# DmitryUlyanov/deep-image-prior

Measured on AMD Instinct MI355X. Metric: optimisation iters/sec per image (skip-net 512x512 denoising), higher is better.
Workload: dtype f32

## Files before the change

deep-image-prior_amd/csrc/bn_kernels.hip:

```cpp
#include "dip_common.h"
#include "bn_ticket.h"
#include "dip_group.h"
#include "dip_gradsrc.h"
#include <stdlib.h>

namespace {

template <bool GRP = false>
__global__ __launch_bounds__(256) void bn_finalize_kernel(const float* __restrict__ partials_, int ntiles,
                                                          int Cstride, int C, const float* __restrict__ gamma_,
                                                          const float* __restrict__ beta_, float eps, float momentum,
                                                          float* state_, int Cs, float* running_mean_,
                                                          float* running_var_, const DipGrpArg<GRP> grp) {
    DIP_GRP_PTR(const float*, partials);
    DIP_GRP_PTR(const float*, gamma);
    DIP_GRP_PTR(const float*, beta);
    DIP_GRP_PTR(float*, state);
    DIP_GRP_PTR(float*, running_mean);
    DIP_GRP_PTR(float*, running_var);
    __shared__ double sh[256][12];
    const int row = threadIdx.x;
    const int c0 = blockIdx.x * 4;
    double acc[12];
#pragma unroll
// ... 82 lines not shown

__device__ __forceinline__ void block_reduce_2(const RowLayout& L, f32x4 s1, f32x4 s2, float* partials, int Cs,
                                               float* sh ) {
    dip_tree_sum8(sh, L.nc4, L.rpi, L.prow, L.cg, L.active, s1, s2);
    if (L.active && L.prow == 0) {
        float* o = partials + (size_t)blockIdx.x * 2 * Cs + L.cg * 4;
        st4(o, s1);
        st4(o + Cs, s2);
    }
}

template <bool GRP = false>
__global__ __launch_bounds__(256) void bn_bwd_stats_kernel(const DipGradSrc src_, const float* __restrict__ y_, int H,
                                                           int W, int Cy, int C, const float* __restrict__ state_,
                                                           int Cs, float slope, float* dz_, int Cdz, float* partials_,
                                                           int ppb , const DipBnbFin fin_, const DipGrpArg<GRP> grp) {
    DIP_GRP_DESC(DipGradSrc, src);
    DIP_GRP_PTR(const float*, y);
    DIP_GRP_PTR(const float*, state);
    DIP_GRP_PTR(float*, dz);
    DIP_GRP_PTR(float*, partials);
    DIP_GRP_DESC(DipBnbFin, fin);
    __shared__ __attribute__((aligned(16))) double shd[256 * 8];
    __shared__ unsigned flag;
    float* sh = reinterpret_cast<float*>(shd);
    const RowLayout L = row_layout(C);
    f32x4 s1 = f32x4{0.f, 0.f, 0.f, 0.f}, s2 = s1;
    if (L.active) {
        const int ch = L.cg * 4;
        const f32x4 mean = ld4(state + ch), rstd = ld4(state + Cs + ch), a = ld4(state + 2 * Cs + ch),
                    b = ld4(state + 3 * Cs + ch);
        const int npix = H * W;
        const int p0 = blockIdx.x * ppb;
        const int p1 = min(p0 + ppb, npix);
        const GradSrcThin tw = grad_src_thin(src, ch);
        auto one = [&](int p, const f32x4& du, const f32x4& yv) {
            f32x4 g;
#pragma unroll
            for (int e = 0; e < 4; ++e) {
                const float z = fmaf(a[e], yv[e], b[e]);
                g[e] = dip_mul_rn(du[e], dip_act_grad(z, slope));
                const float xh = (yv[e] - mean[e]) * rstd[e];
                s1[e] += g[e];
                s2[e] += g[e] * xh;
            }
            if (dz != nullptr) st4(dz + (size_t)p * Cdz + ch, g);
        };
        int p = p0 + L.prow;
        for (; p + L.rpi < p1; p += 2 * L.rpi) {
            const int q = p + L.rpi;
            const int r0 = p / W, c0 = p - r0 * W, r1 = q / W, c1 = q - r1 * W;
            const f32x4 du0 = grad_src4(src, tw, r0, c0, H, W, ch);
            const f32x4 du1 = grad_src4(src, tw, r1, c1, H, W, ch);
            const f32x4 y0 = ld4(y + (size_t)p * Cy + ch);
            const f32x4 y1 = ld4(y + (size_t)q * Cy + ch);
            one(p, du0, y0);
            one(q, du1, y1);
        }
        if (p < p1) {
            const int r = p / W, c = p - r * W;
            one(p, grad_src4(src, tw, r, c, H, W, ch), ld4(y + (size_t)p * Cy + ch));
        }
    }
    if (fin.coef == nullptr) {
        block_reduce_2(L, s1, s2, partials, Cs, sh);
        return;
    }
    dip_tree_sum8(sh, L.nc4, L.rpi, L.prow, L.cg, L.active, s1, s2);
    if (L.active && L.prow == 0) {
        float* o = partials + (size_t)blockIdx.x * 2 * Cs + L.cg * 4;
#pragma unroll
        for (int e = 0; e < 4; ++e) { dip_st_sc1(o + e, s1[e]); dip_st_sc1(o + Cs + e, s2[e]); }
    }
    if (dip_ticket_last(fin.ticket, gridDim.x, &flag)) {
        dip_bnb_fin_rows(partials, gridDim.x, Cs, 0, C, fin, shd);
        dip_ticket_reset(fin.ticket);
    }
}

template <bool GRP = false>
__global__ __launch_bounds__(256) void bn_bwd_finalize_kernel(const float* __restrict__ partials_, int nblk,
                                                              const float* __restrict__ partials_lo_, int nblk_lo,
                                                              int c_lo, int Cs, int C, int npix, float* dgamma_,
                                                              float* dbeta_, float* coef_, const DipGrpArg<GRP> grp) {
    DIP_GRP_PTR(const float*, partials);
    DIP_GRP_PTR(const float*, partials_lo);
    DIP_GRP_PTR(float*, dgamma);
    DIP_GRP_PTR(float*, dbeta);
    DIP_GRP_PTR(float*, coef);
    __shared__ double sh[256][8];
    const int row = threadIdx.x;
    const int c0 = blockIdx.x * 4;
    if (c0 < c_lo) { partials = partials_lo; nblk = nblk_lo; }
    double a1[4] = {0.0, 0.0, 0.0, 0.0}, a2[4] = {0.0, 0.0, 0.0, 0.0};
#pragma unroll 8
    for (int t = row; t < nblk; t += 256) {
        const float* p = partials + (size_t)t * 2 * Cs + c0;
        const f32x4 v1 = ld4(p), v2 = ld4(p + Cs);
#pragma unroll
        for (int e = 0; e < 4; ++e) { a1[e] += (double)v1[e]; a2[e] += (double)v2[e]; }
    }
#pragma unroll
    for (int e = 0; e < 4; ++e) { sh[row][e] = a1[e]; sh[row][4 + e] = a2[e]; }
    for (int s = 128; s >= 1; s >>= 1) {
        __syncthreads();
        if (row < s) {
#pragma unroll
            for (int k = 0; k < 8; ++k) sh[row][k] += sh[row + s][k];
        }
    }
    __syncthreads();
    if (row < 4 && c0 + row < C) {
        const int c = c0 + row;
        const double s1 = sh[0][row], s2 = sh[0][4 + row];
        if (dbeta != nullptr) dbeta[c] = (float)s1;
        if (dgamma != nullptr) dgamma[c] = (float)s2;
        coef[c] = (float)(s1 / npix);
        coef[Cs + c] = (float)(s2 / npix);
    }
}

__device__ __forceinline__ void bnb_fin_prologue(const RowLayout& L, const float* __restrict__ partials, int nrows, int Cs,
                                                 int C, int npix, double* shd, float* dgamma, float* dbeta, float* coef,
                                                 f32x4& k1, f32x4& k2) {
    double a[8];
#pragma unroll
    for (int k = 0; k < 8; ++k) a[k] = 0.0;
    if (L.active) {
        const int ch = L.cg * 4;
#pragma unroll 4
        for (int t = L.prow; t < nrows; t += L.rpi) {
            const float* p = partials + (size_t)t * 2 * Cs + ch;
            const f32x4 v1 = ld4(p), v2 = ld4(p + Cs);
#pragma unroll
            for (int e = 0; e < 4; ++e) { a[e] += (double)v1[e]; a[4 + e] += (double)v2[e]; }
        }
    }
    double* mine = shd + (size_t)threadIdx.x * 8;
#pragma unroll
    for (int k = 0; k < 8; ++k) mine[k] = a[k];
    for (int s = dip_pow2_ceil(L.rpi) >> 1; s >= 1; s >>= 1) {
        __syncthreads();
        if (L.active && L.prow < s && L.prow + s < L.rpi) {
            const double* q = shd + (size_t)((L.prow + s) * L.nc4 + L.cg) * 8;
#pragma unroll
            for (int k = 0; k < 8; ++k) mine[k] += q[k];
        }
    }
    __syncthreads();
    if (!L.active) return;
    const double* r0 = shd + (size_t)L.cg * 8;
#pragma unroll
    for (int e = 0; e < 4; ++e) {
        k1[e] = (float)(r0[e] / npix);
        k2[e] = (float)(r0[4 + e] / npix);
    }
    if (blockIdx.x == 0 && L.prow == 0) {
#pragma unroll
        for (int e = 0; e < 4; ++e) {
            const int c = L.cg * 4 + e;
            if (c < C) {
                if (dbeta != nullptr) dbeta[c] = (float)r0[e];
                if (dgamma != nullptr) dgamma[c] = (float)r0[4 + e];
                if (coef != nullptr) { coef[c] = k1[e]; coef[Cs + c] = k2[e]; }
            }
        }
    }
}

struct BnbFinArg {
    const float* partials;
    int nrows;
    float* dgamma;
    float* dbeta;
};
template <class F> __host__ __device__ inline void dip_ptrs(BnbFinArg& b, F& f) { f(b.partials); f(b.dgamma); f(b.dbeta); }

template <bool GRP = false, bool FIN = false>
__global__ __launch_bounds__(256) void bn_bwd_apply_kernel(float* dz_, int Cdz, const float* __restrict__ y_, int Cy,
                                                           int npix, int C, const float* __restrict__ state_, int Cs,
                                                           float* coef_, int ppb, const BnbFinArg fin_, const DipGrpArg<GRP> grp) {
    DIP_GRP_PTR(float*, dz);
    DIP_GRP_PTR(const float*, y);
    DIP_GRP_PTR(const float*, state);
    DIP_GRP_PTR(float*, coef);
    DIP_GRP_DESC(BnbFinArg, fin);
    __shared__ __attribute__((aligned(16))) double shd[FIN ? 256 * 8 : 1];
    const RowLayout L = row_layout(C);
    f32x4 k1 = f32x4{0.f, 0.f, 0.f, 0.f}, k2 = k1;
    if constexpr (FIN) bnb_fin_prologue(L, fin.partials, fin.nrows, Cs, C, npix, shd, fin.dgamma, fin.dbeta, coef, k1, k2);
    if (!L.active) return;
    const int ch = L.cg * 4;
    const f32x4 mean = ld4(state + ch), rstd = ld4(state + Cs + ch), a = ld4(state + 2 * Cs + ch);
    if constexpr (!FIN) { k1 = ld4(coef + ch); k2 = ld4(coef + Cs + ch); }
    const int p0 = blockIdx.x * ppb;
    const int p1 = min(p0 + ppb, npix);
    for (int p = p0 + L.prow; p < p1; p += L.rpi) {
// ... 60 lines not shown
        one(p, grad_src4(src, tw, r, c, H, W, ch), ld4(y + (size_t)p * Cy + ch));
    }
}

__global__ __launch_bounds__(256) void fold_to_nchw_kernel(const DipGradSrc src, int H, int W, int C, float* dst) {
    const int p = blockIdx.x * blockDim.x + threadIdx.x;
    if (p >= H * W) return;
    const int r = p / W, c = p - r * W;
    for (int ch = 0; ch < C; ch += 4) {
        const f32x4 g = grad_src4(src, r, c, H, W, ch);
#pragma unroll
        for (int e = 0; e < 4; ++e)
            if (ch + e < C) dst[(size_t)(ch + e) * H * W + p] = g[e];
    }
}

__global__ __launch_bounds__(256) void fold_to_nhwc_kernel(const DipGradSrc src, int H, int W, int C, float* dst, int Cd) {
    const int nc4 = (C + 3) >> 2;
    const long long i = (long long)blockIdx.x * 256 + threadIdx.x;
    if (i >= (long long)H * W * nc4) return;
    const int cg = (int)(i % nc4);
    const long long p = i / nc4;
    const int r = (int)(p / W), c = (int)(p - (long long)r * W);
    st4(dst + (size_t)p * Cd + cg * 4, grad_src4(src, r, c, H, W, cg * 4));
}

__host__ int bn_blocks(bool apply) { return apply ? 4096 : 1024; }

__host__ int pixels_per_block(int npix, int C, int* nblk, bool apply = false) {
    const int nc4 = (C + 3) / 4;
    int rpi = 256 / nc4;
    if (rpi < 1) rpi = 1;
    int ppb = dip_cdiv(npix, bn_blocks(apply));
    if (ppb < rpi * 2) ppb = rpi * 2;
    *nblk = dip_cdiv(npix, ppb);
    return ppb;
}

}

extern "C" int dip_bn_finalize(const float* partials, int ntiles, int Cstride, int C, const float* gamma,
                               const float* beta, float eps, float momentum, float* state, int Cs,
                               float* running_mean, float* running_var, void* stream) {
    dip_launch_pair<DIP_FAM_BN>(bn_finalize_kernel<false>, bn_finalize_kernel<true>, dim3(dip_cdiv(C, 4)), dim3(256), 0, (hipStream_t)stream, partials,
                                ntiles, Cstride, C, gamma, beta, eps, momentum, state, Cs, running_mean, running_var);
    DIP_CHECK_LAUNCH();
    return 0;
}

extern "C" int dip_bn_bwd_nblk(int H, int W, int C) {
    int nblk;
    pixels_per_block(H * W, C, &nblk);
    return nblk;
}

extern "C" int dip_bn_bwd_stats_fin(const DipGradSrc* src, const float* y, int H, int W, int Cy, int C,
                                    const float* state, int Cs, float slope, float* dz, int Cdz, float* partials,
                                    int nblk, const DipBnbFin* finp, void* stream) {
    if (C > 1024) DIP_FAIL("bn_bwd_stats: C > 1024 unsupported");
    int nb;
    const int ppb = pixels_per_block(H * W, C, &nb);
    if (nb != nblk) DIP_FAIL("bn_bwd_stats: nblk mismatch (use dip_bn_bwd_nblk)");
    DipBnbFin fin = {};
    if (finp != nullptr && finp->coef != nullptr) {
        fin = *finp;
        if (C > 256 || nb > 256 || fin.ticket == nullptr || fin.C != C)
            DIP_FAIL("bn_bwd_stats_fin: needs <= 256 channels and rows (dip_fin_rows_ok), a ticket, C");
    }
    dip_launch_pair<DIP_FAM_BN>(bn_bwd_stats_kernel<false>, bn_bwd_stats_kernel<true>, dim3(nb), dim3(256), 0, (hipStream_t)stream, *src, y, H, W, Cy,
                                C, state, Cs, slope, dz, Cdz, partials, ppb, fin);
    DIP_CHECK_LAUNCH();
    return 0;
}

extern "C" int dip_bn_bwd_stats(const DipGradSrc* src, const float* y, int H, int W, int Cy, int C,
                                const float* state, int Cs, float slope, float* dz, int Cdz, float* partials,
                                int nblk, void* stream) {
    return dip_bn_bwd_stats_fin(src, y, H, W, Cy, C, state, Cs, slope, dz, Cdz, partials, nblk, nullptr, stream);
}

extern "C" int dip_bn_bwd_finalize(const float* partials, int nblk, int Cs, int C, int npix, float* dgamma,
                                   float* dbeta, float* coef, void* stream) {
    dip_launch_pair<DIP_FAM_BN>(bn_bwd_finalize_kernel<false>, bn_bwd_finalize_kernel<true>, dim3(dip_cdiv(C, 4)), dim3(256), 0, (hipStream_t)stream,
                                partials, nblk, (const float*)nullptr, 0, 0, Cs, C, npix, dgamma, dbeta, coef);
    DIP_CHECK_LAUNCH();
    return 0;
}

extern "C" int dip_bn_bwd_finalize2(const float* partials, int nblk, const float* partials_lo, int nblk_lo, int c_lo,
                                    int Cs, int C, int npix, float* dgamma, float* dbeta, float* coef, void* stream) {
    if ((c_lo & 3) || (c_lo > 0 && partials_lo == nullptr)) DIP_FAIL("bn_bwd_finalize2: c_lo must be a multiple of 4");
    dip_launch_pair<DIP_FAM_BN>(bn_bwd_finalize_kernel<false>, bn_bwd_finalize_kernel<true>, dim3(dip_cdiv(C, 4)), dim3(256), 0, (hipStream_t)stream,
                                partials, nblk, partials_lo, nblk_lo, c_lo, Cs, C, npix, dgamma, dbeta, coef);
    DIP_CHECK_LAUNCH();
    return 0;
}

extern "C" int dip_bn_bwd_apply(float* dz, int Cdz, const float* y, int Cy, int npix, int C, const float* state,
                                int Cs, const float* coef, void* stream) {
    int nb;
    const int ppb = pixels_per_block(npix, C, &nb, true);
    dip_launch_pair<DIP_FAM_BN>(bn_bwd_apply_kernel<false>, bn_bwd_apply_kernel<true>, dim3(nb), dim3(256), 0, (hipStream_t)stream, dz, Cdz, y, Cy, npix,
                                C, state, Cs, const_cast<float*>(coef), ppb, BnbFinArg{});
    DIP_CHECK_LAUNCH();
    return 0;
}

extern "C" int dip_bn_bwd_apply_src(const DipGradSrc* src, const float* y, int H, int W, int Cy, int C,
                                    const float* state, int Cs, float slope, const float* coef, float* dy, int Cdy,
                                    void* stream) {
    if (C > 1024) DIP_FAIL("bn_bwd_apply_src: C > 1024 unsupported");
    int nb;
    const int ppb = pixels_per_block(H * W, C, &nb, true);
    dip_launch_pair<DIP_FAM_BN>(bn_bwd_apply_src_kernel<false>, bn_bwd_apply_src_kernel<true>, dim3(nb), dim3(256), 0, (hipStream_t)stream, *src, y, H,
                                W, Cy, C, state, Cs, slope, const_cast<float*>(coef), dy, Cdy, ppb, BnbFinArg{});
    DIP_CHECK_LAUNCH();
    return 0;
}

extern "C" int dip_bn_bwd_fin_rows_ok(int nrows, int C) {
    static const int maxrows = getenv("DIP_BNB_FIN_MAX_ROWS") ? atoi(getenv("DIP_BNB_FIN_MAX_ROWS")) : 320;
    return (nrows >= 1 && nrows <= maxrows && C >= 1 && C <= 1024) ? 1 : 0;
}

extern "C" int dip_bn_bwd_apply_fin(float* dz, int Cdz, const float* y, int Cy, int npix, int C, const float* state, int Cs,
                                    const float* partials, int nrows, float* dgamma, float* dbeta, float* coef, void* stream) {
    if (C > 1024 || (Cs & 3) || partials == nullptr || nrows < 1) DIP_FAIL("bn_bwd_apply_fin: C <= 1024, Cs % 4 == 0, partial rows");
    int nb;
    const int ppb = pixels_per_block(npix, C, &nb, true);
    dip_launch_pair<DIP_FAM_BN>(bn_bwd_apply_kernel<false, true>, bn_bwd_apply_kernel<true, true>, dim3(nb), dim3(256), 0, (hipStream_t)stream, dz, Cdz,
                                y, Cy, npix, C, state, Cs, coef, ppb, BnbFinArg{partials, nrows, dgamma, dbeta});
    DIP_CHECK_LAUNCH();
    return 0;
}

extern "C" int dip_bn_bwd_apply_src_fin(const DipGradSrc* src, const float* y, int H, int W, int Cy, int C, const float* state,
                                        int Cs, float slope, const float* partials, int nrows, float* dgamma, float* dbeta,
                                        float* coef, float* dy, int Cdy, void* stream) {
    if (C > 1024 || (Cs & 3) || partials == nullptr || nrows < 1) DIP_FAIL("bn_bwd_apply_src_fin: C <= 1024, Cs % 4 == 0, partial rows");
    int nb;
    const int ppb = pixels_per_block(H * W, C, &nb, true);
    dip_launch_pair<DIP_FAM_BN>(bn_bwd_apply_src_kernel<false, true>, bn_bwd_apply_src_kernel<true, true>, dim3(nb), dim3(256), 0, (hipStream_t)stream,
                                *src, y, H, W, Cy, C, state, Cs, slope, coef, dy, Cdy, ppb, BnbFinArg{partials, nrows, dgamma, dbeta});
    DIP_CHECK_LAUNCH();
    return 0;
}

extern "C" int dip_fold_to_nhwc(const DipGradSrc* src, int H, int W, int C, float* dst, int Cd, void* stream) {
    if ((Cd & 3) || (src->Cg & 3)) DIP_FAIL("fold_to_nhwc: channel strides must be multiples of 4");
    const long long n = (long long)H * W * ((C + 3) / 4);
    dip_launch(fold_to_nhwc_kernel, dim3((unsigned)((n + 255) / 256)), dim3(256), 0, (hipStream_t)stream, *src, H, W, C, dst, Cd);
    DIP_CHECK_LAUNCH();
    return 0;
}

extern "C" int dip_fold_to_nchw(const DipGradSrc* src, int H, int W, int C, float* dst, void* stream) {
    dip_launch(fold_to_nchw_kernel, dim3(dip_cdiv(H * W, 256)), dim3(256), 0, (hipStream_t)stream, *src, H, W, C, dst);
    DIP_CHECK_LAUNCH();
    return 0;
}
```

deep-image-prior_amd/csrc/dip_group.h:

```cpp
#pragma once
#include "dip_common.h"
#include <stdint.h>
#include <type_traits>

struct DipGroupCtx {
    int ninst;
    long long stride;
    const char* base;
    long long row;
    unsigned native;
};
extern "C" const DipGroupCtx* dip_group_ctx(void);
extern "C" void dip_group_fault(const char* what);

enum : unsigned {
    DIP_FAM_BN = 1u,
    DIP_FAM_CONV = 2u,
    DIP_FAM_DMA = 4u,
    DIP_FAM_SMALL = 8u,
    DIP_FAM_THIN = 16u,
    DIP_FAM_WGRAD = 32u,
    DIP_FAM_LOSS = 64u,
    DIP_FAM_MISC = 128u,
    DIP_FAM_UPCAT = 256u,
};

struct DipGrp {
    long long stride;
    int gz;
};
struct DipNoGrp {};
template <bool GRP> using DipGrpArg = std::conditional_t<GRP, DipGrp, DipNoGrp>;

template <class F> __host__ __device__ inline void dip_ptrs(DipNoGrp&, F&) {}
template <class F> __host__ __device__ inline void dip_ptrs(DipTransform& t, F& f) { f(t.a); f(t.b); }
template <class F> __host__ __device__ inline void dip_ptrs(DipConvDesc& d, F& f) {
    f(d.x); dip_ptrs(d.tr, f); f(d.wp); f(d.bias); f(d.y); f(d.stats); f(d.ws);
    f(d.bnb_y); f(d.bnb_state); f(d.bnb_partials); f(d.bnb_partials_thin); f(d.wp3);
}
template <class F> __host__ __device__ inline void dip_ptrs(DipWgradDesc& d, F& f) {
    f(d.x); dip_ptrs(d.tr, f); f(d.dy); f(d.partial); f(d.bias_partial);
}
template <class F> __host__ __device__ inline void dip_ptrs(DipGradSrc& s, F& f) { f(s.g); f(s.tw); }
template <class F> __host__ __device__ inline void dip_ptrs(DipBnFin& b, F& f) {
    f(b.gamma); f(b.beta); f(b.state); f(b.running_mean); f(b.running_var); f(b.ticket);
}
template <class F> __host__ __device__ inline void dip_ptrs(DipBnbFin& b, F& f) { f(b.dgamma); f(b.dbeta); f(b.coef); f(b.ticket); }
template <class F> __host__ __device__ inline void dip_ptrs(DipUpcatDesc& d, F& f) {
    f(d.s); dip_ptrs(d.ts, f); f(d.d); dip_ptrs(d.td, f); f(d.cat); f(d.stats);
}
template <class F> __host__ __device__ inline void dip_ptrs(DipLossHeadDesc& d, F& f) {
    f(d.u); dip_ptrs(d.tr, f); f(d.w); f(d.bias); f(d.target); f(d.mask); f(d.out); f(d.partials); f(d.loss);
}
template <class F> __host__ __device__ inline void dip_ptrs(DipSRLossDesc& d, F& f) {
    f(d.out); f(d.taps); f(d.target); f(d.y); f(d.partials); f(d.loss);
}
template <class F> __host__ __device__ inline void dip_ptrs(DipSRTVDesc& d, F& f) {
    dip_ptrs(d.sr, f); f(d.tv_weight); f(d.tv_partials);
}

struct DipShiftF {
    long long off;
    template <class T> __host__ __device__ void operator()(T*& p) const {
        if (p != nullptr) p = reinterpret_cast<T*>(reinterpret_cast<uintptr_t>(p) + (uintptr_t)off);
    }
};
struct DipRangeF {
    uintptr_t lo, hi;
    bool ok;
    template <class T> void operator()(T*& p) {
        if (p != nullptr) {
            const uintptr_t v = reinterpret_cast<uintptr_t>(p);
            if (v < lo || v >= hi) ok = false;
        }
    }
};

template <class T, class F>
__host__ __device__ inline void dip_visit(T& v, F& f) {
    using U = std::remove_cv_t<T>;
    if constexpr (std::is_pointer_v<U>) f(v);
    else if constexpr (std::is_arithmetic_v<U> || std::is_enum_v<U> || std::is_same_v<U, std::nullptr_t>) { (void)f; }
    else dip_ptrs(v, f);
}
template <class T>
__host__ __device__ inline T dip_gshift(T v, long long off) {
    DipShiftF f{off};
    dip_visit(v, f);
    return v;
}
template <class... A>
inline bool dip_group_in_range(const DipGroupCtx& g, A... a) {
    DipRangeF f{reinterpret_cast<uintptr_t>(g.base), reinterpret_cast<uintptr_t>(g.base) + (uintptr_t)g.row, true};
    (dip_visit(a, f), ...);
    if (!f.ok) dip_group_fault("a pointer of a grouped launch lies outside instance 0's slab");
    return f.ok;
}

template <bool GRP, class T>
__device__ __forceinline__ const T& dip_pick(const T& shifted, const T& solo) {
    if constexpr (GRP) return shifted;
    else return solo;
}
template <bool GRP>
__device__ __forceinline__ long long dip_grp_off(const DipGrpArg<GRP>& grp) {
    if constexpr (GRP) return (long long)(blockIdx.z / (unsigned)grp.gz) * grp.stride;
    else return 0;
}
template <bool GRP>
__device__ __forceinline__ unsigned dip_grp_z(const DipGrpArg<GRP>& grp) {
    if constexpr (GRP) return blockIdx.z % (unsigned)grp.gz;
    else return blockIdx.z;
}
#define DIP_GRP_DESC(T, d)                                                   \
    T d##sh_;                                                                \
    if constexpr (GRP) d##sh_ = dip_gshift(d##_, dip_grp_off<GRP>(grp));     \
    const T& d = dip_pick<GRP>(d##sh_, d##_)
#define DIP_GRP_PTR(T, p) T p = GRP ? dip_gshift(p##_, dip_grp_off<GRP>(grp)) : p##_

template <class K, class... A>
inline void dip_launch(K kern, dim3 grid, dim3 block, size_t lds, hipStream_t st, A... a) {
    const DipGroupCtx& g = *dip_group_ctx();
    if (g.ninst <= 1) { kern<<<grid, block, lds, st>>>(a...); return; }
    if (!dip_group_in_range(g, a...)) return;
    for (int b = 0; b < g.ninst; ++b) kern<<<grid, block, lds, st>>>(dip_gshift(a, (long long)b * g.stride)...);
}

template <unsigned FAM, class K, class KG, class... A>
inline void dip_launch_pair(K kern, KG kern_g, dim3 grid, dim3 block, size_t lds, hipStream_t st, A... a) {
    const DipGroupCtx& g = *dip_group_ctx();
    if (g.ninst <= 1) { kern<<<grid, block, lds, st>>>(a..., DipNoGrp{}); return; }
    if (!dip_group_in_range(g, a...)) return;
    if (g.native & FAM) {
        const int gz = (int)grid.z;
        grid.z = (unsigned)(gz * g.ninst);
// ... 13 lines not shown
```

deep-image-prior_amd/csrc/dip_list.hip:

```cpp
#include "dip_common.h"
#include <string.h>
#include <utility>

namespace {

template <class T>
inline T slot_as(const uint64_t* s) {
    T v;
    memcpy(&v, s, sizeof(T));
    return v;
}
template <class... A, size_t... I>
inline int call_slots(int (*fn)(A...), const uint64_t* s, std::index_sequence<I...>) {
    return fn(slot_as<A>(s + I)...);
}
template <auto Fn> struct Thunk;
template <class... A, int (*Fn)(A...)>
struct Thunk<Fn> {
    static constexpr int nargs = (int)sizeof...(A);
    static int call(const uint64_t* s) { return call_slots(Fn, s, std::index_sequence_for<A...>{}); }
};

struct Entry {
    const char* name;
    int (*call)(const uint64_t*);
    int nargs;
};
#define DIP_REG(f) {#f, &Thunk<&f>::call, Thunk<&f>::nargs}
const Entry g_fns[] = {
    DIP_REG(dip_nchw_to_nhwc), DIP_REG(dip_nhwc_to_nchw), DIP_REG(dip_head_fwd), DIP_REG(dip_head_bwd),
    DIP_REG(dip_pack_weights), DIP_REG(dip_pack_weights_bf3),
    DIP_REG(dip_conv_igemm), DIP_REG(dip_conv_thin4), DIP_REG(dip_conv_igemm_dma_cols), DIP_REG(dip_conv_small), DIP_REG(dip_conv_thin),
    DIP_REG(dip_conv_dgrad_ring), DIP_REG(dip_conv_bf3_cols), DIP_REG(dip_conv_splitk_finish),
    DIP_REG(dip_conv_wgrad), DIP_REG(dip_wgrad_bf3), DIP_REG(dip_wgrad_thin), DIP_REG(dip_conv_wgrad_tail), DIP_REG(dip_wgrad_tail_stream), DIP_REG(dip_wgrad_reduce),
    DIP_REG(dip_bn_finalize), DIP_REG(dip_bn_bwd_stats), DIP_REG(dip_bn_bwd_stats_fin), DIP_REG(dip_bn_bwd_finalize),
    DIP_REG(dip_bn_bwd_finalize2), DIP_REG(dip_bn_bwd_apply), DIP_REG(dip_bn_bwd_apply_src), DIP_REG(dip_bn_bwd_apply_fin),
    DIP_REG(dip_bn_bwd_apply_src_fin), DIP_REG(dip_bn_bwd_one), DIP_REG(dip_fold_to_nchw), DIP_REG(dip_fold_to_nhwc),
    DIP_REG(dip_upcat_fwd), DIP_REG(dip_upcat_fwd_fin), DIP_REG(dip_avgpool2_fwd), DIP_REG(dip_avgpool2_bwd),
    DIP_REG(dip_maxpool2_fwd), DIP_REG(dip_maxpool2_bwd), DIP_REG(dip_upsample_bwd_stats), DIP_REG(dip_upsample_bwd_stats_crop),
    DIP_REG(dip_upsample_bwd_stats_crop_fin), DIP_REG(dip_upsample_bwd_one),
    DIP_REG(dip_adam_step), DIP_REG(dip_noise_axpy), DIP_REG(dip_adam_tick), DIP_REG(dip_adam_step_dev),
    DIP_REG(dip_noise_axpy_dev), DIP_REG(dip_noise_axpy_dev2), DIP_REG(dip_counter_add), DIP_REG(dip_counter_add_n),
    DIP_REG(dip_adam_sgld_step), DIP_REG(dip_adam_sgld_step_dev), DIP_REG(dip_posterior_dev),
    DIP_REG(dip_loss_head_fwd), DIP_REG(dip_loss_head_bwd), DIP_REG(dip_sr_loss_fwd), DIP_REG(dip_sr_loss_bwd),
    DIP_REG(dip_sr_tv_loss_fwd), DIP_REG(dip_sr_tv_loss_bwd),
    DIP_REG(dip_fit_monitor), DIP_REG(dip_fit_monitor_dev), DIP_REG(dip_arena_backtrack),
    DIP_REG(dip_sr_monitor), DIP_REG(dip_sr_monitor_dev), DIP_REG(dip_restore_monitor), DIP_REG(dip_restore_monitor_dev),
    DIP_REG(dip_early_stop_dev), DIP_REG(dip_early_stop_keep), DIP_REG(dip_early_stop_emv_dev),
    DIP_REG(dip_ssim_dev),
    DIP_REG(dip_lanczos_down_fwd), DIP_REG(dip_lanczos_down_bwd), DIP_REG(dip_down_dense_fwd), DIP_REG(dip_down_dense_bwd_data),
    DIP_REG(dip_down_dense_bwd_weight), DIP_REG(dip_res_join_fwd), DIP_REG(dip_res_join_bwd),
};
constexpr int NFN = (int)(sizeof(g_fns) / sizeof(g_fns[0]));

}

extern "C" int dip_list_fn_id(const char* name) {
    if (name == nullptr) return -1;
    for (int i = 0; i < NFN; ++i)
        if (strcmp(g_fns[i].name, name) == 0) return i;
    return -1;
}

extern "C" int dip_list_fn_nargs(int fn) { return (fn >= 0 && fn < NFN) ? g_fns[fn].nargs : -1; }

extern "C" int dip_list_run(const DipCmd* cmds, int n, void* const* streams, int nstreams, void* const* events, int nevents,
                            int* failed_at) {
    if (failed_at != nullptr) *failed_at = -1;
    for (int i = 0; i < n; ++i) {
        const DipCmd& c = cmds[i];
        int rc = 0;
        if (c.stream < 0 || c.stream >= nstreams) rc = -1;
        else if (c.kind == DIP_CMD_LAUNCH) {
            if (c.fn < 0 || c.fn >= NFN || c.slots == nullptr || c.nslots != g_fns[c.fn].nargs) rc = -1;
            else {
                c.slots[c.nslots - 1] = (uint64_t)reinterpret_cast<uintptr_t>(streams[c.stream]);
                rc = g_fns[c.fn].call(c.slots);
            }
        } else if (c.event < 0 || c.event >= nevents) rc = -1;
        else if (c.kind == DIP_CMD_RECORD)
            rc = (int)hipEventRecord(reinterpret_cast<hipEvent_t>(events[c.event]), reinterpret_cast<hipStream_t>(streams[c.stream]));
        else if (c.kind == DIP_CMD_WAIT)
            rc = (int)hipStreamWaitEvent(reinterpret_cast<hipStream_t>(streams[c.stream]), reinterpret_cast<hipEvent_t>(events[c.event]), 0);
        else rc = -1;
        if (rc != 0) {
            if (failed_at != nullptr) *failed_at = i;
            if (rc == -1 && c.kind != DIP_CMD_LAUNCH) dip_set_error("list_run: malformed command (stream / event index, kind)");
            else if (rc == -1 && (c.fn < 0 || c.fn >= NFN || c.slots == nullptr || c.nslots != g_fns[c.fn < 0 || c.fn >= NFN ? 0 : c.fn].nargs))
                dip_set_error("list_run: malformed LAUNCH command (function id, slot count)");
            else if (c.kind != DIP_CMD_LAUNCH) dip_set_error(hipGetErrorString((hipError_t)rc));
            return rc;
        }
    }
    return 0;
}

extern "C" int dip_iter_run(const DipPhase* phases, int nphases, void* const* streams, int nstreams, int* failed_at) {
    if (failed_at != nullptr) failed_at[0] = failed_at[1] = -1;
    if (phases == nullptr || nphases < 0 || streams == nullptr || nstreams < 1) {
        dip_set_error("iter_run: needs a phase table and at least one stream");
        return -1;
    }
    for (int p = 0; p < nphases; ++p) {
        const DipPhase& ph = phases[p];
        int at = -1;
        int rc = -1;
        if (ph.n < 0 || (ph.n > 0 && ph.cmds == nullptr) || ph.nevents < 0 || (ph.nevents > 0 && ph.events == nullptr))
            dip_set_error("iter_run: malformed phase (command / event table)");
        else rc = dip_list_run(ph.cmds, ph.n, streams, nstreams, ph.events, ph.nevents, &at);
        if (rc != 0) {
            if (failed_at != nullptr) { failed_at[0] = p; failed_at[1] = at; }
            return rc;
        }
    }
    return 0;
}

extern "C" int dip_events_create(void** events, int n) {
    for (int i = 0; i < n; ++i) {
        hipEvent_t e;
        hipError_t rc = hipEventCreateWithFlags(&e, hipEventDisableTiming);
        if (rc != hipSuccess) {
            dip_set_error(hipGetErrorString(rc));
            for (int j = 0; j < i; ++j) (void)hipEventDestroy(reinterpret_cast<hipEvent_t>(events[j]));
            return (int)rc;
        }
        events[i] = reinterpret_cast<void*>(e);
    }
    return 0;
}

extern "C" int dip_events_destroy(void** events, int n) {
    int rc = 0;
    for (int i = 0; i < n; ++i)
// ... 8 lines not shown
```

deep-image-prior_amd/csrc/loss_kernels.hip:

```cpp
#include "dip_common.h"
#include "dip_group.h"
#include <stdlib.h>

namespace {

__device__ __forceinline__ float sigmoidf_(float v) { return 1.f / (1.f + expf(-v)); }

template <bool GRP = false>
__global__ __launch_bounds__(256) void loss_head_fwd_kernel(const DipLossHeadDesc d_, const int ppb, const DipGrpArg<GRP> grp) {
    DIP_GRP_DESC(DipLossHeadDesc, d);
    __shared__ float red[256];
    const int tid = threadIdx.x;
    const int oi = tid & 3;
    const int cin4 = (d.Cin + 3) >> 2;
    const bool has_tr = d.tr.a != nullptr;
    const float slope = d.tr.slope;
    float bias[4];
#pragma unroll
    for (int o = 0; o < 4; ++o) bias[o] = (d.bias != nullptr && o < d.Cout) ? d.bias[o] : 0.f;
    const float* wrow = d.w + (size_t)(oi < d.Cout ? oi : 0) * d.Cin;
    const bool wvalid = oi < d.Cout;

    const int p0 = blockIdx.x * ppb, p1 = min(p0 + ppb, d.HW);
    float lsum = 0.f;
    for (int pb = p0; pb < p1; pb += 256) {
        const int p = pb + tid;
        const bool pv = p < p1;
        const float* up = d.u + (size_t)(pv ? p : p0) * d.Cu;
        f32x4 ac4[4];
#pragma unroll
        for (int e = 0; e < 4; ++e) ac4[e] = f32x4{0.f, 0.f, 0.f, 0.f};
#pragma unroll 8
        for (int k4 = 0; k4 < cin4; ++k4) {
            f32x4 b = *reinterpret_cast<const f32x4*>(up + k4 * 4);
            f32x4 a;
#pragma unroll
            for (int e = 0; e < 4; ++e) {
                const int c = k4 * 4 + e;
                a[e] = (wvalid && c < d.Cin) ? wrow[c] : 0.f;
                if (has_tr) {
                    const float ta = c < d.Cin ? d.tr.a[c] : 0.f, tb = c < d.Cin ? d.tr.b[c] : 0.f;
                    b[e] = dip_act(fmaf(ta, b[e], tb), slope);
                }
            }
#pragma unroll
            for (int e = 0; e < 4; ++e) ac4[e] = __builtin_amdgcn_mfma_f32_4x4x1f32(a[e], b[e], ac4[e], 4, 0, 0);
        }
        const f32x4 acc = (ac4[0] + ac4[1]) + (ac4[2] + ac4[3]);
        if (pv) {
#pragma unroll
            for (int o = 0; o < 4; ++o) {
                if (o < d.Cout) {
                    float y = acc[o] + bias[o];
                    if (d.sigmoid) y = sigmoidf_(y);
                    d.out[(size_t)o * d.HW + p] = y;
                    const float t = d.target[(size_t)o * d.HW + p];
                    float a = y, b = t;
                    if (d.mask != nullptr) {
                        const float m = d.mask[(size_t)(d.mask_c == 1 ? 0 : o) * d.HW + p];
                        a = y * m;
                        b = t * m;
                    }
                    const float df = a - b;
                    lsum = fmaf(df, df, lsum);
                }
            }
        }
    }
    red[tid] = lsum;
    __syncthreads();
    for (int s = 128; s >= 1; s >>= 1) {
        if (tid < s) red[tid] += red[tid + s];
        __syncthreads();
    }
    if (tid == 0) d.partials[blockIdx.x] = red[0];
}

template <int NC4, bool GRP = false>
__global__ __launch_bounds__(256) void loss_head_fwd_coal_kernel(const DipLossHeadDesc d_, const int ppb, const DipGrpArg<GRP> grp) {
    DIP_GRP_DESC(DipLossHeadDesc, d);
    __shared__ float red[256];
    constexpr int PW = 64 / NC4;
    constexpr int PB = 4 * PW;
    const int tid = threadIdx.x, lane = tid & 63, wave = tid >> 6;
    const int cg = lane % NC4, psub = lane / NC4;
    const bool has_tr = d.tr.a != nullptr;
    const float slope = has_tr ? d.tr.slope : 1.f;
    const bool leaky = slope > 0.f;
    f32x4 ta = f32x4{1.f, 1.f, 1.f, 1.f}, tb = f32x4{0.f, 0.f, 0.f, 0.f};
    float w[4][4];
#pragma unroll
    for (int e = 0; e < 4; ++e) {
        const int c = cg * 4 + e;
        if (has_tr && c < d.Cin) { ta[e] = d.tr.a[c]; tb[e] = d.tr.b[c]; }
#pragma unroll
        for (int o = 0; o < 4; ++o) w[o][e] = (o < d.Cout && c < d.Cin) ? d.w[(size_t)o * d.Cin + c] : 0.f;
    }
    const bool bA = (cg & (NC4 / 2)) != 0, bB = (cg & (NC4 / 4)) != 0;
    const int myo = 2 * (bA ? 1 : 0) + (bB ? 1 : 0);
    const bool writer = (cg & (NC4 / 4 - 1)) == 0 && myo < d.Cout;
    const float mybias = (d.bias != nullptr && myo < d.Cout) ? d.bias[myo] : 0.f;
    const int p0 = blockIdx.x * ppb, p1 = min(p0 + ppb, d.HW);
    float lsum = 0.f;
    constexpr int UN = 4;
    for (int base = p0 + wave * PW; base < p1; base += UN * PB) {
        const int pb = base + psub;
        f32x4 u[UN];
#pragma unroll
        for (int q = 0; q < UN; ++q) {
            const int p = pb + q * PB;
            u[q] = *reinterpret_cast<const f32x4*>(d.u + (size_t)(p < p1 ? p : p0) * d.Cu + cg * 4);
        }
#pragma unroll
        for (int q = 0; q < UN; ++q) {
            const int p = pb + q * PB;
            f32x4 v = u[q];
            if (leaky) {
#pragma unroll
                for (int e = 0; e < 4; ++e) v[e] = dip_act_leaky(fmaf(ta[e], v[e], tb[e]), slope);
            } else {
#pragma unroll
                for (int e = 0; e < 4; ++e) v[e] = dip_act(fmaf(ta[e], v[e], tb[e]), slope);
            }
            float part[4];
#pragma unroll
            for (int o = 0; o < 4; ++o) part[o] = (w[o][0] * v[0] + w[o][1] * v[1]) + (w[o][2] * v[2] + w[o][3] * v[3]);
            const float k0 = (bA ? part[2] : part[0]) + __shfl_xor(bA ? part[0] : part[2], NC4 / 2);
            const float k1 = (bA ? part[3] : part[1]) + __shfl_xor(bA ? part[1] : part[3], NC4 / 2);
            float mine = (bB ? k1 : k0) + __shfl_xor(bB ? k0 : k1, NC4 / 4);
#pragma unroll
            for (int sft = NC4 / 8; sft >= 1; sft >>= 1) mine += __shfl_xor(mine, sft);
            if (p < p1 && writer) {
                float y = mine + mybias;
                if (d.sigmoid) y = sigmoidf_(y);
                d.out[(size_t)myo * d.HW + p] = y;
                const float t = d.target[(size_t)myo * d.HW + p];
                float a = y, b = t;
                if (d.mask != nullptr) {
                    const float m = d.mask[(size_t)(d.mask_c == 1 ? 0 : myo) * d.HW + p];
                    a = y * m;
                    b = t * m;
                }
                const float df = a - b;
                lsum = fmaf(df, df, lsum);
            }
        }
    }
    red[tid] = lsum;
    __syncthreads();
    for (int s2 = 128; s2 >= 1; s2 >>= 1) {
        if (tid < s2) red[tid] += red[tid + s2];
        __syncthreads();
    }
    if (tid == 0) d.partials[blockIdx.x] = red[0];
}

template <bool GRP = false>
__global__ __launch_bounds__(256) void loss_reduce_kernel(const float* __restrict__ partials_, int n, double scale,
                                                          float* __restrict__ loss_, const DipGrpArg<GRP> grp) {
    DIP_GRP_PTR(const float*, partials);
    DIP_GRP_PTR(float*, loss);
    __shared__ double dred[256];
    const int tid = threadIdx.x;
    double s = 0.0;
    for (int i = tid; i < n; i += 256) s += (double)partials[i];
    dred[tid] = s;
    __syncthreads();
    for (int st = 128; st >= 1; st >>= 1) {
        if (tid < st) dred[tid] += dred[tid + st];
        __syncthreads();
    }
    if (tid == 0) *loss = (float)(dred[0] * scale);
}

template <bool GRP = false>
__global__ __launch_bounds__(256) void loss_head_bwd_kernel(const DipLossHeadDesc d_, const float* __restrict__ gscale_,
                                                            float* __restrict__ dy_, const int Cy, const DipGrpArg<GRP> grp) {
    DIP_GRP_DESC(DipLossHeadDesc, d);
    DIP_GRP_PTR(const float*, gscale);
    DIP_GRP_PTR(float*, dy);
    const int p = blockIdx.x * 256 + threadIdx.x;
    if (p >= d.HW) return;
    const float gs = gscale != nullptr ? *gscale : 1.f;
    const float k = 2.f / ((float)d.Cout * (float)d.HW);
    for (int c0 = 0; c0 < Cy; c0 += 4) {
        f32x4 v = f32x4{0.f, 0.f, 0.f, 0.f};
#pragma unroll
        for (int e = 0; e < 4; ++e) {
            const int o = c0 + e;
            if (o < d.Cout) {
                const float y = d.out[(size_t)o * d.HW + p];
                const float t = d.target[(size_t)o * d.HW + p];
                float a = y, b = t, m = 1.f;
                if (d.mask != nullptr) {
                    m = d.mask[(size_t)(d.mask_c == 1 ? 0 : o) * d.HW + p];
                    a = y * m;
                    b = t * m;
                }
                float g = (a - b) * k * gs;
                if (d.mask != nullptr) g = g * m;
                if (d.sigmoid) g = g * ((1.f - y) * y);
                v[e] = g;
            }
        }
        *reinterpret_cast<f32x4*>(dy + (size_t)p * Cy + c0) = v;
    }
}

template <bool GRP = false>
__global__  void adam_tick_kernel(DipIterState* st_, double lr, double beta1, double beta2, const DipGrpArg<GRP> grp) {
    DIP_GRP_PTR(DipIterState*, st);
    if (threadIdx.x != 0 || blockIdx.x != 0) return;
    const unsigned long long step = st->step + 1ull;
    st->step = step;
    const double bc1 = 1.0 - pow(beta1, (double)step);
    const double bc2 = 1.0 - pow(beta2, (double)step);
    st->step_size = (float)(lr / bc1);
    st->bc2_sqrt = (float)sqrt(bc2);
}

template <bool GRP = false>
__global__  void counter_add_kernel(unsigned long long* c_, unsigned long long inc, const DipGrpArg<GRP> grp) {
    DIP_GRP_PTR(unsigned long long*, c);
    if (threadIdx.x == 0 && blockIdx.x == 0) *c += inc;
}

template <bool GRP = false>
__global__  void counter_add_n_kernel(unsigned long long* c_, int n, unsigned long long inc, const DipGrpArg<GRP> grp) {
    DIP_GRP_PTR(unsigned long long*, c);
    const int i = (int)(blockIdx.x * blockDim.x + threadIdx.x);
    if (i < n) c[i] += inc;
}

}

#define NC4_MIN_CHECK(cout, nc4) ((nc4) < 4 || (cout) > (nc4))
static int head_ppb(int HW) {
    int ppb = dip_round_up(dip_cdiv(HW, 1024), 256);
    return ppb < 256 ? 256 : ppb;
}

extern "C" int dip_loss_head_nblk(int HW, int Cin) {
    (void)Cin;
    return dip_cdiv(HW, head_ppb(HW));
}

extern "C" int dip_loss_head_fwd(const DipLossHeadDesc* dp, void* stream) {
    const DipLossHeadDesc& d = *dp;
    if (d.Cout < 1 || d.Cout > 4) DIP_FAIL("loss_head: 1..4 output channels");
    if (d.Cin < 1 || (d.Cu & 3) || dip_round_up(d.Cin, 4) > d.Cu) DIP_FAIL("loss_head: channel stride must be a multiple of 4 covering Cin");
    if (d.mask != nullptr && d.mask_c != 1 && d.mask_c != d.Cout) DIP_FAIL("loss_head: mask must have 1 or Cout channels");
    const int ppb = head_ppb(d.HW);
    const int nblk = dip_cdiv(d.HW, ppb);
    if (nblk != d.nblk) DIP_FAIL("loss_head: nblk must come from dip_loss_head_nblk");
    const int nc4 = (d.Cin + 3) / 4;
    static const bool no_coal = getenv("DIP_LOSS_HEAD_NO_COAL") != nullptr;
    hipStream_t st = (hipStream_t)stream;
    if (no_coal || nc4 > 32 || (nc4 & (nc4 - 1)) != 0 || (NC4_MIN_CHECK(d.Cout, nc4))) {
        dip_launch_pair<DIP_FAM_LOSS>(loss_head_fwd_kernel<false>, loss_head_fwd_kernel<true>, dim3(nblk), dim3(256), 0, st, d, ppb);
    } else {
        switch (nc4) {
            case 32: dip_launch_pair<DIP_FAM_LOSS>(loss_head_fwd_coal_kernel<32>, loss_head_fwd_coal_kernel<32, true>, dim3(nblk), dim3(256), 0, st, d, ppb); break;
            case 16: dip_launch_pair<DIP_FAM_LOSS>(loss_head_fwd_coal_kernel<16>, loss_head_fwd_coal_kernel<16, true>, dim3(nblk), dim3(256), 0, st, d, ppb); break;
            case 8: dip_launch_pair<DIP_FAM_LOSS>(loss_head_fwd_coal_kernel<8>, loss_head_fwd_coal_kernel<8, true>, dim3(nblk), dim3(256), 0, st, d, ppb); break;
            default: dip_launch_pair<DIP_FAM_LOSS>(loss_head_fwd_coal_kernel<4>, loss_head_fwd_coal_kernel<4, true>, dim3(nblk), dim3(256), 0, st, d, ppb); break;
        }
    }
    DIP_CHECK_LAUNCH();
    dip_launch_pair<DIP_FAM_LOSS>(loss_reduce_kernel<false>, loss_reduce_kernel<true>, dim3(1), dim3(256), 0, (hipStream_t)stream,
                                  (const float*)d.partials, nblk, 1.0 / ((double)d.Cout * (double)d.HW), d.loss);
    DIP_CHECK_LAUNCH();
    return 0;
}

extern "C" int dip_loss_head_bwd(const DipLossHeadDesc* dp, const float* gscale, float* dy, int Cy, void* stream) {
    const DipLossHeadDesc& d = *dp;
    if (d.Cout < 1 || d.Cout > 4 || (Cy & 3) || Cy < d.Cout) DIP_FAIL("loss_head_bwd: bad channel counts");
    dip_launch_pair<DIP_FAM_LOSS>(loss_head_bwd_kernel<false>, loss_head_bwd_kernel<true>, dim3(dip_cdiv(d.HW, 256)), dim3(256), 0, (hipStream_t)stream,
                                  d, gscale, dy, Cy);
    DIP_CHECK_LAUNCH();
    return 0;
}

extern "C" int dip_adam_tick(DipIterState* st, double lr, double beta1, double beta2, void* stream) {
    dip_launch_pair<DIP_FAM_LOSS>(adam_tick_kernel<false>, adam_tick_kernel<true>, dim3(1), dim3(1), 0, (hipStream_t)stream, st, lr, beta1, beta2);
    DIP_CHECK_LAUNCH();
    return 0;
}

extern "C" int dip_counter_add(uint64_t* counter, uint64_t inc, void* stream) {
    dip_launch_pair<DIP_FAM_LOSS>(counter_add_kernel<false>, counter_add_kernel<true>, dim3(1), dim3(1), 0, (hipStream_t)stream,
                                  reinterpret_cast<unsigned long long*>(counter), (unsigned long long)inc);
    DIP_CHECK_LAUNCH();
    return 0;
}

extern "C" int dip_counter_add_n(uint64_t* counters, int n, uint64_t inc, void* stream) {
    if (counters == nullptr || n < 1) DIP_FAIL("counter_add_n: needs n >= 1 counters");
    dip_launch_pair<DIP_FAM_LOSS>(counter_add_n_kernel<false>, counter_add_n_kernel<true>, dim3(dip_cdiv(n, 64)), dim3(64), 0,
                                  (hipStream_t)stream, reinterpret_cast<unsigned long long*>(counters), n, (unsigned long long)inc);
    DIP_CHECK_LAUNCH();
    return 0;
}

namespace {

constexpr int SR_T = 16;
constexpr int SR_LDS_BYTES = 48 * 1024;
constexpr int SR_UN = 8;

template <int K, int F, bool GRP = false>
__global__ __launch_bounds__(256) void sr_loss_fwd_kernel(const DipSRLossDesc d_, const int qn, const int pitch, const int rp,
                                                          const DipGrpArg<GRP> grp) {
    DIP_GRP_DESC(DipSRLossDesc, d);
    extern __shared__ float sr_win[];
    __shared__ float red[256];
    const int k = K ? K : d.k, f = F ? F : d.f;
    const int tid = threadIdx.x, lx = tid & 15, ly = tid >> 4;
    const int ntx = (d.Wo + SR_T - 1) / SR_T, nty = (d.Ho + SR_T - 1) / SR_T;
    const int b = blockIdx.x;
    const int ox0 = (b % ntx) * SR_T, oy0 = ((b / ntx) % nty) * SR_T, c = b / (ntx * nty);
    const float* xc = d.out + (size_t)c * d.H * d.W;
    const int wc = (SR_T - 1) * f + k, wr = (rp - 1) * f + k, nwin = wr * wc;
    const int ox = ox0 + lx, oy = oy0 + ly;
    const bool inside = ox < d.Wo && oy < d.Ho;
    const int gx0 = ox0 * f - d.pad;
    float acc = 0.f;
    for (int ob = 0; ob < SR_T && oy0 + ob < d.Ho; ob += rp) {
        const int gy0 = (oy0 + ob) * f - d.pad;
        if (ob) __syncthreads();
        for (int i0 = tid; i0 < nwin; i0 += 256 * SR_UN) {
            float v[SR_UN];
#pragma unroll
            for (int u = 0; u < SR_UN; ++u) {
                const int idx = i0 + u * 256, wy = idx / wc, wx = idx - wy * wc;
                v[u] = idx < nwin ? xc[(size_t)min(max(gy0 + wy, 0), d.H - 1) * d.W + min(max(gx0 + wx, 0), d.W - 1)] : 0.f;
            }
#pragma unroll
            for (int u = 0; u < SR_UN; ++u) {
// ... 366 lines not shown
```

deep-image-prior_amd/dip_engine.py:

```python
from __future__ import annotations

import ctypes as C
import os
from typing import List, Optional

import torch

import dip_native as N
from dip_native import round_up


def _ptr(t: Optional[torch.Tensor], off_floats: int = 0) -> Optional[int]:
    if t is None:
        return None
    return t.data_ptr() + 4 * off_floats


class BNRec:

    def __init__(self, module: torch.nn.BatchNorm2d, name: str):
        self.module = module
        self.name = name
        self.C = module.num_features
        self.Cs = round_up(self.C, 4)
# ... 4 lines not shown


class ConvRec:
    def __init__(self, module: torch.nn.Conv2d, pad_mode: int, name: str):
        self.module = module
        self.name = name
        self.Cin, self.Cout = module.in_channels, module.out_channels
        self.ks = module.kernel_size[0]
        self.stride = module.stride[0]
        self.P = (self.ks - 1) // 2
        self.pad_mode = pad_mode if self.P > 0 else N.PAD_ZERO
        self.w_off = self.b_off = -1
        self.fwd_off = self.dgrad_off = -1
        self.need_dgrad = True

    @property
    def fwd_elems(self):
        return self.ks * self.ks * round_up(self.Cin, 4) * round_up(self.Cout, 32)

    @property
    def dgrad_elems(self):
        return self.ks * self.ks * round_up(self.Cout, 4) * round_up(self.Cin, 32)


class Act:

    def __init__(self, buf, H, W, Cch, bn: Optional[BNRec] = None, slope: float = 1.0):
        self.buf, self.H, self.W, self.C = buf, H, W, Cch
        self.Cs = round_up(Cch, 4)
        self.bn, self.slope = bn, slope

    def transform(self, shape_only=False) -> N.DipTransform:
        if self.bn is None:
            return N.DipTransform(None, None, 1.0)
        if shape_only:
            return N.DipTransform(1, 1, self.slope)
        assert self.bn.Cs == self.Cs
        return N.DipTransform(_ptr(self.bn.state, 2 * self.Cs), _ptr(self.bn.state, 3 * self.Cs), self.slope)


class ScalePlan:

    def __init__(self):
        self.skip_conv = self.skip_bn = None
        self.down_a = self.down_a_bn = self.down_b = self.down_b_bn = None
        self.cat_bn = self.up = self.up_bn = self.up1 = self.up1_bn = None
        self.ns = 0
        self.upsample_mode = "nearest"
        self.pool = None
        self.down_ds = None


class SkipEngine:
    kind = "skip"

    def __init__(self, net, scales: List[ScalePlan], out_conv: torch.nn.Conv2d, need_sigmoid: bool, pad: str,
                 act_slope: float = 0.2):
        self._init_common(net, need_sigmoid, pad, act_slope)
        self._collect_records(scales, out_conv)
        self.param_list = list(net.parameters())
        self._check_supported()

    def _init_common(self, net, need_sigmoid: bool, pad: str, act_slope: float):
        self.net = net
        self.need_sigmoid = need_sigmoid
        self.pad_mode = N.PAD_REFLECT if pad == "reflection" else N.PAD_ZERO
        self.slope = act_slope
        self.fwd_id = 0
        self._aux = {}
        self.two_streams = os.environ.get("DIP_TWO_STREAMS", "1") != "0"
        self.defer_scale = int(os.environ.get("DIP_DEFER_WGRAD", "2")) if self.two_streams else -1
        self.side_min_pixels = int(os.environ.get("DIP_SIDE_MIN_PIXELS", "0"))
        self._fwd_side, self._deferred, self._entered_defer_scale, self._fused_bnb = set(), [], False, {}
        self.use_clist = os.environ.get("DIP_NO_CLIST") is None
        import re
        ko = os.environ.get("DIP_KNOCKOUT")
        self._knockout = re.compile(ko) if ko else None
        self._ko_after, self._ko_seen = int(os.environ.get("DIP_KNOCKOUT_AFTER", "0")), {}
        self._clists = {}
        self._replicate_bufs = set()
        self.fuse_bnb = os.environ.get("DIP_BNB_FUSE", "0") == "1"
        self.fuse_bnb_1x1 = os.environ.get("DIP_BNB_FUSE", "0") == "2"
        self.thin_src = os.environ.get("DIP_NO_THIN_SRC") is None
        self.use_small = os.environ.get("DIP_CONV_NO_SMALL") is None
        self.ticket_fin = os.environ.get("DIP_TICKET_FIN") == "1"
        self.bnb_one = os.environ.get("DIP_BNB_NO_ONE") is None
        self.tail_inline = self.two_streams and os.environ.get("DIP_TAIL_INLINE", "1") != "0"
        self.bnb_fin_fuse = os.environ.get("DIP_BNB_FIN_FUSE") == "1"
        self.bulk2_max_pixels = 0
        if self.two_streams:
            env = os.environ.get("DIP_BULK2_MAX_PIXELS")
            self.bulk2_max_pixels = int(env) if env is not None else -1
        self._bulk2, self._bulk_flip = set(), False
        self.bf3 = False
        self.device = None
        self.shape_key = None
        self.lib = None
        self.slab = None

    def _collect_records(self, scales: List[ScalePlan], out_conv: torch.nn.Conv2d):
        self.nscales = len(scales)
        self.convs: List[ConvRec] = []
        self.bns: List[BNRec] = []
        self.sc = []
        for i, s in enumerate(scales):
            rec = ScalePlan()
            rec.ns, rec.upsample_mode = s.ns, s.upsample_mode
            rec.pool = getattr(s, 'pool', None)
            for attr in ("skip_conv", "down_a", "down_ds", "down_b", "up", "up1"):
                m = getattr(s, attr, None)
                if m is not None:
                    r = ConvRec(m, self.pad_mode, f"s{i}.{attr}")
                    if attr == "down_ds":
                        r.P = (r.ks - r.stride) // 2
                        r.pad_mode = N.PAD_REPLICATE
                    self.convs.append(r)
                    setattr(rec, attr, r)
            for attr in ("skip_bn", "down_a_bn", "down_b_bn", "cat_bn", "up_bn", "up1_bn"):
                m = getattr(s, attr)
                if m is not None:
                    r = BNRec(m, f"s{i}.{attr}")
                    self.bns.append(r)
                    setattr(rec, attr, r)
            self.sc.append(rec)
        self.out_conv = ConvRec(out_conv, self.pad_mode, "out")
        self.convs.append(self.out_conv)

    def _check_supported(self):
        for r in self.convs:
            lanczos_ds = r.name.endswith(".down_ds") and r.ks in (8, 12) and r.stride == 2
            if not lanczos_ds and (r.ks not in (1, 3, 5, 7) or r.stride not in (1, 2) or (r.ks == 1 and r.stride != 1)):
                raise NotImplementedError(f"dip-amd: conv {r.name} k={r.ks} s={r.stride} has no gfx950 kernel")
            m = r.module
            if m.dilation != (1, 1) or m.groups != 1 or m.kernel_size[0] != m.kernel_size[1]:
                raise NotImplementedError(f"dip-amd: conv {r.name}: dilation/groups/non-square unsupported")
        for b in self.bns:
            if b.module.momentum is None:
                raise NotImplementedError(f"dip-amd: BatchNorm {b.name}: momentum=None (cumulative moving average of "
                                          "the running statistics) is not implemented; the reference uses 0.1")
            if not b.module.affine:
                raise NotImplementedError(f"dip-amd: BatchNorm {b.name}: affine=False is not implemented")
        for i, s in enumerate(self.sc):
            if s.ns % 4 or s.down_b.Cout % 4 or s.up.Cout % 4 or (s.up.Cin % 4):
                raise NotImplementedError("dip-amd: internal channel counts must be multiples of 4")

    def _dalloc(self, n, dtype=torch.float32, zero=False):
        if self.slab is not None:
            return self.slab.alloc(int(n), dtype, zero)
        return (torch.zeros if zero else torch.empty)(int(n), dtype=dtype, device=self.device)

    def _dcopy(self, host_bytes):
        src = torch.frombuffer(bytearray(host_bytes), dtype=torch.uint8)
        t = self._dalloc(src.numel(), torch.uint8)
        t.copy_(src)
        return t

    def _build_arenas(self, device):
        self.lib = N.lib()
        self.device = device
        params = self.param_list
        off = 0
        slots = []
        for p in params:
            slots.append(off)
            off += round_up(p.numel(), 4)
        self.n_arena = off
# ... 30 lines not shown
                b.coef = self._dalloc(2 * b.Cs, zero=True)
        off = 0
        recs = (N.DipPackRec * len(self.convs))()
        max_elems = 0
        for k, r in enumerate(self.convs):
            r.fwd_off = off
            off += r.fwd_elems
            r.dgrad_off = off
            off += r.dgrad_elems
            recs[k] = N.DipPackRec(w_off=r.w_off, fwd_off=r.fwd_off, dgrad_off=r.dgrad_off, Cout=r.Cout, Cin=r.Cin, KS=r.ks,
                                   CinP4=round_up(r.Cin, 4), CoutP32=round_up(r.Cout, 32), CoutP4=round_up(r.Cout, 4),
                                   CinP32=round_up(r.Cin, 32))
            max_elems = max(max_elems, r.fwd_elems + r.dgrad_elems)
        self.packed = self._dalloc(off, zero=True)
        self.bf3 = bool(self.lib.dip_conv_bf3_terms())
        if self.bf3:
            off3, max3 = 0, 0
            recs3 = (N.DipPackRec3 * len(self.convs))()
            for k, r in enumerate(self.convs):
                r.fwd3_off = r.dgrad3_off = -1
                nchF, nchD = (round_up(r.Cin, 4) + 15) // 16, (round_up(r.Cout, 4) + 15) // 16
                CoutP, CinP = round_up(r.Cout, 32), round_up(r.Cin, 32)
                k1 = (os.environ.get("DIP_CONV_BF3_1X1") == "1" and r.ks == 1 and r.Cin % 16 == 0 and r.Cout % 16 == 0
                      and min(r.Cin, r.Cout) >= 128)
                if (r.ks == 3 or k1) and r.stride == 1 and not r.name.endswith(".down_ds"):
                    kk = r.ks * r.ks
                    r.fwd3_off = off3
                    off3 += kk * nchF * 3 * CoutP * 16
                    r.dgrad3_off = off3
                    off3 += kk * nchD * 3 * CinP * 16
                    max3 = max(max3, kk * 16 * (nchF * CoutP + nchD * CinP))
                recs3[k] = N.DipPackRec3(w_off=r.w_off, fwd_off=r.fwd3_off, dgrad_off=r.dgrad3_off, Cout=r.Cout, Cin=r.Cin,
                                         KS=r.ks, nchF=nchF, CoutP32=CoutP, nchD=nchD, CinP32=CinP)
            self.packed3 = self._dalloc(max(off3, 8), torch.int16, zero=True)
            self.pack_recs3 = self._dcopy(bytes(recs3))
            self.pack_max3 = max3
        self.pack_recs = self._dcopy(bytes(recs))
        self.pack_max = max_elems
        self.shape_key = None

    def _arena_ok(self) -> bool:
        if self.device is None:
            return False
        base = self.params.data_ptr()
        for p, o in zip(self.param_list, self.slots):
            if p.data_ptr() != base + 4 * o:
                return False
        return True

    def _new(self, n):
        t = self._dalloc(n)
        self._alloc.append(t)
        return t

    _SCRATCH = ("stats", "bwd", "wg", "wgb", "wg2", "wgb2", "ws", "stats2", "ws2", "bwd2", "bwd3")

    def _reset_sizing(self):
        self._need = dict.fromkeys(self._SCRATCH, 4)
        self._need["tickets"] = 8

    def _scratch(self, name, n):
        if self._sizing:
            self._need[name] = max(self._need[name], n)
            return None
        assert n <= self._need[name], (name, n, self._need[name])
        return self._pool[name]

    def _has_big_layer(self, H, W) -> bool:
        h, w = H, W
        for sc in self.sc:
            hl, wl = ((h + 1) // 2, (w + 1) // 2) if sc.pool is None else (h // 2, w // 2)
            for r, px in ((sc.down_a, hl * wl), (sc.down_b, hl * wl), (sc.up, h * w), (sc.up1, h * w)):
                if r is not None and r.ks >= 3 and r.Cin >= 96 and r.Cout >= 96 and px >= 65536:
                    return True
            h, w = hl, wl
        return False

    def _begin_plan(self, H, W, Cin_img):
        self.H, self.W, self.Cimg = H, W, Cin_img
        self._clists = {}
        self._reset_sizing()
        self._alloc = []
        self.n_out = self.out_conv.Cout
        if getattr(self, "_bulk2_auto", self.bulk2_max_pixels < 0):
            self._bulk2_auto = True
            self.bulk2_max_pixels = 0 if self._has_big_layer(H, W) else 100000

    def _build_plan(self, H, W, Cin_img):
        if min(H, W) < 2 ** self.nscales:
            raise NotImplementedError(f"dip-amd: input {H}x{W} is too small for {self.nscales} scales")
        self._begin_plan(H, W, Cin_img)
        oc = self.out_conv
        for sizing in (True, False):
            self._begin_pass(sizing)
            self.x_nhwc = self._buf(H * W * round_up(Cin_img, 4))
            xin = Act(self.x_nhwc, H, W, Cin_img)
            last = self._plan_scale(0, xin, H, W)
            self.Hout, self.Wout = last.H, last.W
            self.y_out = self._buf(last.H * last.W * round_up(oc.Cout, 4))
            self._emit_conv_fwd(oc, last, self.y_out, None)
            self.dy_out = self._buf(last.H * last.W * round_up(oc.Cout, 4))
            pre = []
            self._emit_wgrad(oc, last, self.dy_out, pre, scale=0)
            if self._thin_src_ok(oc, last):
                du_last = (self.dy_out, 0, oc)
            else:
                du_last = self._emit_dgrad(oc, last, self.dy_out, pre, fuse_bn=True)
            dy_last = self._emit_bn_act_bwd(last, du_last, pre)
            self.dbg_top = {"du_last": du_last, "dy_last": dy_last, "last": last}
            self.last_act = last
            self.bwd_ops = pre + self._bwd_scale_ops(0, dy_last)
            self.bwd_ops += self._flush_deferred_wgrads()
        self.shape_key = (H, W, Cin_img)

    def _begin_pass(self, sizing: bool):
        self._sizing = sizing
        self.fwd_ops, self.bwd_ops, self.bwd_input_ops, self.keep = [], [], [], []
        if not sizing:
            self._pool = {name: self._new(self._need[name]) for name in self._SCRATCH}
            self._pool["tickets"] = self._dalloc(self._need["tickets"], torch.int32, zero=True)
            self._alloc.append(self._pool["tickets"])
        self._ticket_off = 0
        self._fused_bnb = {}
        self._deferred = []
        self._replicate_bufs = set()
        self._fwd_side = set()
        self._bulk2, self._bulk_flip = set(), False
        self._entered_defer_scale = False

    def _plan_scale(self, i, xin: Act, H, W):
        s = self.sc[i]
        st = {}
        Hl, Wl = ((H + 1) // 2, (W + 1) // 2) if s.pool is None else (H // 2, W // 2)
        if s.ns:
            st["s_y"] = self._buf(H * W * round_up(s.ns, 4))
            self._emit_conv_fwd(s.skip_conv, xin, st["s_y"], s.skip_bn)
            st["s_act"] = Act(st["s_y"], H, W, s.ns, s.skip_bn, self.slope)
        st["d1_y"] = self._buf(Hl * Wl * round_up(s.down_a.Cout, 4))
        if s.pool in ('avg', 'max'):
            st["d1_full"] = self._buf(H * W * round_up(s.down_a.Cout, 4))
            self._emit_conv_fwd(s.down_a, xin, st["d1_full"], None)
            self._emit_avgpool(st["d1_full"], H, W, s.down_a.Cout, st["d1_y"], s.down_a_bn, s.pool)
        elif s.pool == 'lanczos':
            st["d1_full"] = self._buf(H * W * round_up(s.down_a.Cout, 4))
            self._emit_conv_fwd(s.down_a, xin, st["d1_full"], None)
            st["d1_raw"] = Act(st["d1_full"], H, W, s.down_a.Cout)
            self._emit_conv_fwd(s.down_ds, st["d1_raw"], st["d1_y"], s.down_a_bn)
        else:
            self._emit_conv_fwd(s.down_a, xin, st["d1_y"], s.down_a_bn)
        d1 = Act(st["d1_y"], Hl, Wl, s.down_a.Cout, s.down_a_bn, self.slope)
        st["d2_y"] = self._buf(Hl * Wl * round_up(s.down_b.Cout, 4))
        self._emit_conv_fwd(s.down_b, d1, st["d2_y"], s.down_b_bn)
        d2 = Act(st["d2_y"], Hl, Wl, s.down_b.Cout, s.down_b_bn, self.slope)
        st["d1"], st["d2"] = d1, d2
        deep = d2
        if i < self.nscales - 1:
            deep = self._plan_scale(i + 1, d2, Hl, Wl)
        st["deep"] = deep
        ccat = s.ns + deep.C
        assert ccat == s.cat_bn.C == s.up.Cin, (ccat, s.cat_bn.C, s.up.Cin)
        Hu, Wu = 2 * deep.H, 2 * deep.W
        if s.ns:
            Ho, Wo = min(H, Hu), min(W, Wu)
        else:
            Ho, Wo = Hu, Wu
        geom = dict(Hs=H, Ws=W, os_y=(H - Ho) // 2 if s.ns else 0, os_x=(W - Wo) // 2 if s.ns else 0,
                    Hd=deep.H, Wd=deep.W, od_y=(Hu - Ho) // 2, od_x=(Wu - Wo) // 2)
        default = (not s.ns or (Ho, Wo) == (H, W)) and deep.H == (Ho + 1) // 2 and deep.W == (Wo + 1) // 2 \
            and geom["od_y"] == 0 and geom["od_x"] == 0
        st["geom"] = None if default else geom
        st["cat"] = self._buf(Ho * Wo * round_up(ccat, 4))
        self._emit_upcat(s, st.get("s_act"), deep, st["cat"], Ho, Wo, st["geom"])
        cat = Act(st["cat"], Ho, Wo, ccat, s.cat_bn, 1.0)
        st["cat_act"] = cat
        st["u_y"] = self._buf(Ho * Wo * round_up(s.up.Cout, 4))
        self._emit_conv_fwd(s.up, cat, st["u_y"], s.up_bn)
        u = Act(st["u_y"], Ho, Wo, s.up.Cout, s.up_bn, self.slope)
        st["u"] = u
        res = u
        if s.up1 is not None:
            st["u1_y"] = self._buf(Ho * Wo * round_up(s.up1.Cout, 4))
            self._emit_conv_fwd(s.up1, u, st["u1_y"], s.up1_bn)
            res = Act(st["u1_y"], Ho, Wo, s.up1.Cout, s.up1_bn, self.slope)
            st["u1"] = res
        st["xin"], st["H"], st["W"], st["Ho"], st["Wo"] = xin, H, W, Ho, Wo
        s.st = st
        return res

    def _buf(self, n):
        return None if self._sizing else self._new(n)

    def _ticket(self, n=8):
        if self._sizing:
            self._need["tickets"] += n
            return None
        off = self._ticket_off
# ... 182 lines not shown
                self.keep.append(d)
                ops.append((self.lib.dip_conv_small, (C.byref(d),), "dgrad:" + r.name))
            return (gbuf, pad)
        ws = self._scratch("ws", wsf)
        d.ws = _ptr(ws) if ksplit > 1 else None
        variant = self.lib.dip_conv_variant(C.byref(d))
        if fuse_here and self.lib.dip_conv_bnb_fusable(C.byref(d)):
            c_lo = (r.Cin - 128) if variant == 3 else 0
            if c_lo % 4 == 0:
                self._fuse_bnb_into(d, x, gbuf, pad, self.lib.dip_conv_ntiles(Hg, Wg),
                                    self.lib.dip_conv_thin4_ntiles(Hg, Wg) if c_lo else 0, c_lo)
        if sizing:
            return (gbuf, pad)
        self.keep.append(d)
        if variant == 3 and self.two_streams:
            ncols = r.Cin - 128
            ops.append((self.lib.dip_conv_thin4, (C.byref(d), ncols), "dgthin:" + r.name))
            ops.append((self.lib.dip_conv_igemm_dma_cols, (C.byref(d), ncols), "dgrad:" + r.name))
        else:
            ops.append((self.lib.dip_conv_igemm, (C.byref(d),), "dgrad:" + r.name))
        if ring:
            dr = N.DipConvDesc.from_buffer_copy(d)
            dr.ksplit, dr.ws = 1, None
            self.keep.append(dr)
            ops.append((self.lib.dip_conv_dgrad_ring, (C.byref(dr),), "dgring:" + r.name))
        return (gbuf, pad)

    def _fuse_bnb_into(self, d: N.DipConvDesc, x: Act, gbuf, pad, rows, rows_lo=0, c_lo=0):
        bn = x.bn
        partials = self._scratch("bwd", rows * 2 * bn.Cs)
        thin = self._scratch("bwd3", rows_lo * 2 * bn.Cs)
        if self._sizing:
            return
        d.bnb_y, d.bnb_state = _ptr(x.buf), _ptr(bn.state)
        d.bnb_partials, d.bnb_partials_thin = _ptr(partials), _ptr(thin) if c_lo else None
        d.bnb_Cy, d.bnb_Cs, d.bnb_pad, d.bnb_slope = x.Cs, bn.Cs, pad, float(x.slope)
        self._fused_bnb[gbuf.data_ptr()] = (rows, rows_lo, c_lo)

    def _thin_src_ok(self, oc: ConvRec, last: Act) -> bool:
        return (self.thin_src and oc.ks == 1 and oc.stride == 1 and oc.Cout <= 4 and oc.Cin % 4 == 0 and last.bn is not None
                and not self.fuse_bnb and not self._bnb_one_ok(last))

    def _gradsrc(self, g, Cg, choff=0, window=None):
        if len(g) == 3:
            buf, _, oc = g
            d = N.DipGradSrc(g=_ptr(buf), Cg=round_up(oc.Cout, 4), tw=_ptr(self.params, oc.w_off), tn=oc.Cout, tcw=oc.Cin)
            self.keep.append(d)
            return d
        buf, pad = g
        fold = 0 if pad == 0 else (2 if buf.data_ptr() in self._replicate_bufs else 1)
        d = N.DipGradSrc(g=_ptr(buf), pad=pad, fold=fold, Cg=Cg, choff=choff)
        if window is not None:
            d.win_y, d.win_x, d.win_h, d.win_w = window
        self.keep.append(d)
        return d

    def _act_args(self, a: Act):
        return (_ptr(a.buf), a.H, a.W, a.Cs, a.C, _ptr(a.bn.state), a.bn.Cs, float(a.slope))

    def _dparams(self, bn: BNRec):
        return (_ptr(self.grads, bn.gamma_off), _ptr(self.grads, bn.beta_off), _ptr(bn.coef))

    def _emit_bnb_apply(self, a: Act, dz, ops, src=None, partials=None):
        bn, lib = a.bn, self.lib
        if partials is None:
            fns, fin = (lib.dip_bn_bwd_apply, lib.dip_bn_bwd_apply_src), (_ptr(bn.coef),)
        else:
            fns = (lib.dip_bn_bwd_apply_fin, lib.dip_bn_bwd_apply_src_fin)
            fin = (_ptr(partials[0]), partials[1], *self._dparams(bn))
        if src is None:
            args = (_ptr(dz), a.Cs, _ptr(a.buf), a.Cs, a.H * a.W, a.C, _ptr(bn.state), bn.Cs, *fin)
        else:
            args = (C.byref(src), *self._act_args(a), *fin, _ptr(dz), a.Cs)
        ops.append((fns[src is not None], args, "bnb_apply:" + bn.name))

    def _emit_bnb_fin_apply(self, a: Act, scratch, rows, dz, ops, src=None):
        bn = a.bn
        if self._fin_rows_ok(rows, a.C):
            return self._emit_bnb_apply(a, dz, ops, src, (scratch, rows))
        ops.append((self.lib.dip_bn_bwd_finalize, (_ptr(scratch), rows, bn.Cs, bn.C, a.H * a.W, *self._dparams(bn)),
                    "bnb_fin:" + bn.name))
        self._emit_bnb_apply(a, dz, ops, src)

    def _emit_bn_act_bwd(self, a: Act, g, ops, choff=0, Cg=None, side=False, window=None):
        bn = a.bn
        nblk = self.lib.dip_bn_bwd_nblk(a.H, a.W, a.C)
        fin_ok = self.ticket_fin and bool(self.lib.dip_fin_rows_ok(nblk, a.C))
        ticket = self._ticket() if fin_ok else None
        scratch = self._scratch("bwd2" if side else "bwd", nblk * 2 * a.Cs)
        if self._sizing:
            return None
        dz = self._new(a.H * a.W * a.Cs)
        src = self._gradsrc(g, Cg if Cg is not None else a.Cs, choff, window)
        lib = self.lib
        if self._bnb_one_ok(a) and self._fused_bnb.get(g[0].data_ptr()) is None:
            ops.append((lib.dip_bn_bwd_one, (C.byref(src), *self._act_args(a), _ptr(dz), a.Cs, *self._dparams(bn)),
                        "bnb_one:" + bn.name))
            return dz
        stats = (C.byref(src), *self._act_args(a), None, a.Cs, _ptr(scratch), nblk)
        fused = self._fused_bnb.get(g[0].data_ptr()) if (choff == 0 and not side) else None
        if fused is None and fin_ok:
            fin = self._bnb_fin(bn, a.H * a.W, ticket)
            self.keep.append(fin)
            ops.append((lib.dip_bn_bwd_stats_fin, (*stats, C.byref(fin)), "bnb_stats:" + bn.name))
            self._emit_bnb_apply(a, dz, ops, src)
        elif fused is None:
            ops.append((lib.dip_bn_bwd_stats, stats, "bnb_stats:" + bn.name))
            self._emit_bnb_fin_apply(a, scratch, nblk, dz, ops, src)
        else:
            rows, rows_lo, c_lo = fused
            if c_lo == 0 and self._fin_rows_ok(rows, a.C):
                self._emit_bnb_apply(a, dz, ops, src, (scratch, rows))
                return dz
            thin = self._scratch("bwd3", rows_lo * 2 * bn.Cs) if c_lo else None
            ops.append((lib.dip_bn_bwd_finalize2, (_ptr(scratch), rows, _ptr(thin), rows_lo, c_lo, bn.Cs, bn.C, a.H * a.W,
                                                   *self._dparams(bn)), "bnb_fin:" + bn.name))
            self._emit_bnb_apply(a, dz, ops, src)
        return dz

    def _fin_rows_ok(self, rows, Cc) -> bool:
        return self.bnb_fin_fuse and bool(self.lib.dip_bn_bwd_fin_rows_ok(rows, Cc))

    def _bnb_one_ok(self, a: Act) -> bool:
        return self.bnb_one and a.bn is not None and bool(self.lib.dip_bn_bwd_one_ok(a.H * a.W, a.C))

    def _emit_up_bwd(self, deep: Act, dcat, Cs_cat, choff, H, W, mode, ops, geom=None):
        bn = deep.bn
        nblk = self.lib.dip_bn_bwd_nblk(deep.H, deep.W, deep.C)
        fin_ok = self.ticket_fin and bool(self.lib.dip_fin_rows_ok(nblk, deep.C))
        ticket = self._ticket() if fin_ok else None
        scratch = self._scratch("bwd", nblk * 2 * deep.Cs)
        if self._sizing:
            return None
        dz = self._new(deep.H * deep.W * deep.Cs)
        lib = self.lib
        m = N.UP_BILINEAR if mode == "bilinear" else N.UP_NEAREST
        gm = geom if geom is not None else dict(Hd=(H + 1) // 2, Wd=(W + 1) // 2, od_y=0, od_x=0)
        crop = (_ptr(dcat), Cs_cat, choff, H, W, gm["Hd"], gm["Wd"], gm["od_y"], gm["od_x"], m)
        act = (_ptr(deep.buf), deep.Cs, deep.C, _ptr(bn.state), bn.Cs, float(deep.slope), _ptr(dz), deep.Cs)
        if self._bnb_one_ok(deep):
            ops.append((lib.dip_upsample_bwd_one, (*crop, *act, *self._dparams(bn)), "upb_one:" + bn.name))
        elif fin_ok:
            fin = self._bnb_fin(bn, deep.H * deep.W, ticket)
            self.keep.append(fin)
            ops.append((lib.dip_upsample_bwd_stats_crop_fin, (*crop, *act, _ptr(scratch), nblk, C.byref(fin)),
                        "upb_stats:" + bn.name))
            self._emit_bnb_apply(deep, dz, ops)
        else:
            if geom is None:
                ops.append((lib.dip_upsample_bwd_stats, (_ptr(dcat), Cs_cat, choff, H, W, m, *act, _ptr(scratch), nblk),
                            "upb_stats:" + bn.name))
            else:
                ops.append((lib.dip_upsample_bwd_stats_crop, (*crop, *act, _ptr(scratch), nblk), "upb_stats:" + bn.name))
            self._emit_bnb_fin_apply(deep, scratch, nblk, dz, ops)
        return dz

    def _bwd_scale_ops(self, i, dy_last):
        s = self.sc[i]
        st = s.st
        ops = []
        if i == self.defer_scale:
            self._entered_defer_scale = True
            ops += self._flush_deferred_wgrads()
        H, W, xin = st["H"], st["W"], st["xin"]
        Ho, Wo, geom = st["Ho"], st["Wo"], st["geom"]
        if s.up1 is not None:
            self._emit_wgrad(s.up1, st["u"], dy_last, ops, scale=i)
            g = self._emit_dgrad(s.up1, st["u"], dy_last, ops, fuse_bn=True)
            dy_u = self._emit_bn_act_bwd(st["u"], g, ops)
        else:
            dy_u = dy_last
        cat = st["cat_act"]
        self._emit_wgrad(s.up, cat, dy_u, ops, scale=i)
        g = self._emit_dgrad(s.up, cat, dy_u, ops, fuse_bn=True)
        dcat = self._emit_bn_act_bwd(cat, g, ops)
        dy_s = None
        if s.ns:
            win = (geom["os_y"], geom["os_x"], Ho, Wo) if (geom is not None and (Ho, Wo) != (H, W)) else None
            dy_s = self._emit_bn_act_bwd(st["s_act"], (dcat, 0), ops, choff=0, Cg=cat.Cs, side=True, window=win)
            self._emit_wgrad(s.skip_conv, xin, dy_s, ops, scale=i)
        deep = st["deep"]
        dy_deep = self._emit_up_bwd(deep, dcat, cat.Cs, s.ns, Ho, Wo, s.upsample_mode, ops, geom)
        if self._entered_defer_scale:
# ... 53 lines not shown
        producers = {p for ps in deps.values() for p in ps}
        main_seq = 0
        forked = [0, -1, -1, -1]
        pending = [False, False, False, False]
        for k, (fn, args, name) in enumerate(ops):
            c = cls_fn(name)
            if c and forked[c] != main_seq:
                sched += [("record", ("fork", k), 0), ("wait", c, ("fork", k))]
                forked[c] = main_seq
            if c == 0 and pending[1] and join_before_fn(name):
                sched += [("record", ("join", k), 1), ("wait", 0, ("join", k))]
                pending[1] = False
            for prod in deps.get(name, ()):
                sched.append(("wait", c, ("dep", prod)))
            sched.append(("launch", k, c))
            if name in producers:
                sched.append(("record", ("dep", name), c))
            if c:
                pending[c] = True
            else:
                main_seq += 1
        for c in (1, 2, 3):
            if pending[c]:
                sched += [("record", ("join", -c), c), ("wait", 0, ("join", -c))]
        return sched

    def _aux_streams(self):
        slot = "cap" if torch.cuda.is_current_stream_capturing() else "eager"
        st_ = self._aux.get((slot, self.device))
        if st_ is None:
            st_ = self._aux[(slot, self.device)] = ([torch.cuda.Stream(self.device) for _ in range(3)], {})
        return slot, st_[0], st_[1]

    def _issue(self, ops, main, key, cls_fn=None, join_before_fn=None, deps=None, compile_only=False, drop_last=False):
        multi = cls_fn is not None
        slot, aux, events = self._aux_streams() if multi else ("one", [], None)
        ko = False
        if self._knockout is not None:
            n = self._ko_seen[key] = self._ko_seen.get(key, 0) + 1
            ko = n > self._ko_after
        ck = (key, drop_last, multi, ko)
        ent = self._clists.get(ck)
        if ent is None or ent[0] is not ops:
            sched = self._schedule(ops[:-1] if drop_last else ops, cls_fn, join_before_fn, deps)
            if ko:
                sched = [c for c in sched if not (c[0] == "launch" and self._knockout.search(ops[c[1]][2]))]
            cl = None
            if self.use_clist:
                evidx = {}
                cmds = []
                for c in sched:
                    if c[0] == "launch":
                        fn, args, name = ops[c[1]]
                        cmds.append(("launch", fn, args, c[2], name))
                    elif c[0] == "record":
                        cmds.append(("record", evidx.setdefault(c[1], len(evidx)), c[2]))
                    else:
                        cmds.append(("wait", c[1], evidx.setdefault(c[2], len(evidx))))
                cl = N.CmdList(cmds)
            ent = self._clists[ck] = (ops, sched, cl)
        _, sched, cl = ent
        if compile_only:
            return cl
        if cl is not None:
            cl.run([main.cuda_stream] + [s_.cuda_stream for s_ in aux], slot)
            return
        streams = [main] + aux
        ptrs = [s_.cuda_stream for s_ in streams]
        check = N.check
        for c in sched:
            if c[0] == "launch":
                fn, args, name = ops[c[1]]
                rc = fn(*args, ptrs[c[2]])
                if rc:
                    check(rc, name)
            elif c[0] == "record":
                ev = events.get((key, c[1]))
                if ev is None:
                    ev = events[(key, c[1])] = torch.cuda.Event()
                ev.record(streams[c[2]])
            else:
                streams[c[1]].wait_event(events[(key, c[2])])

    _BWD_SIDE = staticmethod(lambda n: 2 if n.startswith(("wgrad:", "wgred:")) else
                             (1 if (n.startswith("dgthin:") or n.endswith(".skip_bn")) else 0))

    def _backward_deps(self, ops):
        names = [name for _, _, name in ops]
        present = set(names)
        deps = {}
        for i, sc in enumerate(self.sc):
            c, p = f"dgrad+:s{i}.skip_conv", f"bnb_apply:s{i}.skip_bn"
            if p not in present:
                p = f"bnb_one:s{i}.skip_bn"
            if sc.ns and c in present and p in present:
                deps.setdefault(c, []).append(p)
            c = f"wgrad:s{i}.skip_conv"
            if sc.ns and c in present and p in present:
                deps.setdefault(c, []).append(p)
        for k, name in enumerate(names):
            if not name.startswith("dgthin:"):
                continue
            main_part = "dgrad:" + name[len("dgthin:"):]
            j = names.index(main_part, k)
            consumer = next((n for n in names[j + 1:] if not self._BWD_SIDE(n)), None)
            if consumer is not None:
                deps.setdefault(consumer, []).append(name)
        return deps

    def _run_backward_two_streams(self, ops, main, compile_only=False):
        deps = self._bwd_deps if getattr(self, "_bwd_deps_for", None) is ops else None
        if deps is None:
            deps = self._bwd_deps = self._backward_deps(ops)
            self._bwd_deps_for = ops
        capturing = torch.cuda.is_current_stream_capturing()
        bulk2 = self._bulk2 if not capturing else ()
        cls = self._BWD_SIDE if not bulk2 else (lambda n: 3 if n in bulk2 else self._BWD_SIDE(n))
        return self._issue(ops, main, "bwd_cap" if capturing else "bwd", cls, lambda n: False, deps, compile_only)

    def _run_forward_two_streams(self, ops, main, compile_only=False, drop_last=False):
        side = self._fwd_side
        return self._issue(ops, main, "fwd", lambda n: 1 if n in side else 0, lambda n: n.startswith("upcat:"),
                           compile_only=compile_only, drop_last=drop_last)

    def _forward_prologue(self, x_ptr):
        lib = self.lib
        ops = [(lib.dip_pack_weights, (_ptr(self.params), _ptr(self.packed), self.pack_recs.data_ptr(),
                                       len(self.convs), self.pack_max), "pack_weights")]
        if self.bf3:
            ops.append((lib.dip_pack_weights_bf3, (_ptr(self.params), self.packed3.data_ptr(), self.pack_recs3.data_ptr(),
                                                   len(self.convs), self.pack_max3), "pack_weights_bf3"))
        ops.append((lib.dip_nchw_to_nhwc, (x_ptr, _ptr(self.x_nhwc), self.Cimg, self.H * self.W, round_up(self.Cimg, 4)),
                    "nchw_to_nhwc"))
        return ops

    def _launch_forward(self, x_ptr, main, with_out_conv=True, compile_only=False):
        if not compile_only:
            stream = main.cuda_stream
            for fn, args, name in self._forward_prologue(x_ptr):
                N.check(fn(*args, stream), name)
        drop_last = not with_out_conv
        if self.two_streams:
            return self._run_forward_two_streams(self.fwd_ops, main, compile_only, drop_last)
        return self._issue(self.fwd_ops, main, "fwd1", compile_only=compile_only, drop_last=drop_last)

    def _launch_backward(self, main, compile_only=False):
        if self.two_streams:
            return self._run_backward_two_streams(self.bwd_ops, main, compile_only)
        return self._issue(self.bwd_ops, main, "bwd1", compile_only=compile_only)

    def iteration_lists(self, with_out_conv=False):
        if not self.use_clist:
            raise RuntimeError("dip-amd: the native iteration chains compiled command lists; DIP_NO_CLIST=1 switches them off")
        if self._knockout is not None:
            raise RuntimeError("dip-amd: DIP_KNOCKOUT is a timing experiment of the eager path; the native iteration refuses it")
        if torch.cuda.is_current_stream_capturing():
            raise RuntimeError("dip-amd: the native iteration is an eager form; hipGraph capture goes through GraphedIteration")
        return self._launch_forward(None, None, with_out_conv, compile_only=True), self._launch_backward(None, compile_only=True)

    def _net_cin(self) -> int:
        return self.sc[0].down_a.Cin

    def _input_gin(self):
        return self.sc[0].gin

    def _prepare(self, dev, H, W, Cimg):
        if self.device != dev or not self._arena_ok():
            self._build_arenas(dev)
        if self.shape_key != (H, W, Cimg):
            if Cimg != self._net_cin():
                raise RuntimeError(f"dip-amd: input has {Cimg} channels, net expects {self._net_cin()}")
            self._build_plan(H, W, Cimg)

    def forward(self, x: torch.Tensor, head=None):
        if x.dim() != 4 or x.shape[0] != 1:
            raise NotImplementedError("dip-amd: input must be [1,C,H,W] (train-mode BatchNorm couples a batch; "
                                      "independent images run as independent nets)")
        if not self.net.training:
            raise NotImplementedError("dip-amd: eval-mode BatchNorm is not implemented (the reference never "
                                      "calls .eval() on the skip path)")
        dev = x.device
        _, Cimg, H, W = x.shape
        self._prepare(dev, H, W, Cimg)
        lib = self.lib
        with torch.cuda.device(dev):
            main = torch.cuda.current_stream(dev)
            stream = main.cuda_stream
            xs = x.detach()
            if xs.dtype != torch.float32:
                xs = xs.float()
            xs = xs.contiguous()
            self.fwd_id += 1
            self._launch_forward(xs.data_ptr(), main, head is None or head.with_out_conv)
            Ho_, Wo_ = self.Hout, self.Wout
            out = torch.empty((1, self.n_out, Ho_, Wo_), dtype=torch.float32, device=dev)
            loss = None
            if head is None:
                N.check(lib.dip_head_fwd(_ptr(self.y_out), out.data_ptr(), self.n_out, Ho_ * Wo_, round_up(self.n_out, 4),
                                         1 if self.need_sigmoid else 0, stream), "head_fwd")
            else:
                loss = torch.empty((), dtype=torch.float32, device=dev)
                self._head_desc = head._descriptor(self, out, loss)
                for fn, args, name in head.fwd_launches(self, self._head_desc):
                    N.check(fn(*args, stream), name)
            if len(self.bns):
                self.nbt.add_(1)
        self.last_out = out.detach()
        self.last_head = head
        return out if head is None else (loss, out)

    def _detach_stale_grads(self):
        base = self.grads.data_ptr()
        stale = [k for k, (p, o) in enumerate(zip(self.param_list, self.slots))
                 if p.grad is not None and p.grad.data_ptr() == base + 4 * o]
        if not stale:
            return
        if getattr(self, "grads_alt", None) is None or self.grads_alt.numel() != self.grads.numel() \
                or self.grads_alt.device != self.grads.device:
            self.grads_alt = torch.empty_like(self.grads)
        self.grads_alt.copy_(self.grads)
        for k in stale:
            p, o = self.param_list[k], self.slots[k]
            p.grad = self.grads_alt[o:o + p.numel()].view(p.shape)

    def backward(self, gout, fwd_id: int, need_input_grad: bool, gloss=None):
        if fwd_id != self.fwd_id:
            raise RuntimeError("dip-amd: backward() of a stale forward: the engine keeps the activations of the "
                               "most recent net(x) only (one forward, one backward per closure call)")
        dev = self.device
        lib = self.lib
        H, W = self.H, self.W
        grads = self.grads
        with torch.cuda.device(dev):
            main = torch.cuda.current_stream(dev)
            stream = main.cuda_stream
            self._detach_stale_grads()
            if self.last_head is None:
                g = gout.detach()
                if g.dtype != torch.float32:
                    g = g.float()
                g = g.contiguous()
                N.check(lib.dip_head_bwd(g.data_ptr(), self.last_out.data_ptr(), _ptr(self.dy_out), self.n_out,
                                         self.Hout * self.Wout,
                                         round_up(self.n_out, 4), 1 if self.need_sigmoid else 0, stream), "head_bwd")
            else:
                gl = gloss.detach().reshape(1)
                if gl.dtype != torch.float32:
                    gl = gl.float()
                self._gloss_keep = gl
                for fn, args, name in self.last_head.bwd_launches(self, self._head_desc, gl.data_ptr()):
                    N.check(fn(*args, stream), name)
            self._launch_backward(main)
            gx = None
            if need_input_grad:
                self._issue(self.bwd_input_ops, main, "bwdin")
                gbuf, pad = self._input_gin()
                src = N.DipGradSrc(g=_ptr(gbuf), pad=pad, fold=1 if pad > 0 else 0, Cg=round_up(self.Cimg, 4))
                gx = torch.empty((1, self.Cimg, H, W), dtype=torch.float32, device=dev)
                N.check(lib.dip_fold_to_nchw(C.byref(src), H, W, self.Cimg, gx.data_ptr(), stream), "fold_to_nchw")
        views = [grads[o:o + p.numel()].view(p.shape) for p, o in zip(self.param_list, self.slots)]
        return gx, views


class TableAct(Act):

    def __init__(self, buf, H, W, Cch, table, slope):
        super().__init__(buf, H, W, Cch, None, slope)
        self.table = table

    def transform(self, shape_only=False) -> N.DipTransform:
        if self.slope == 1.0:
            return N.DipTransform(None, None, 1.0)
        if shape_only:
            return N.DipTransform(1, 1, self.slope)
        return N.DipTransform(_ptr(self.table), _ptr(self.table, self.Cs), self.slope)


class ResBlockRec:

    def __init__(self, conv1, bn1, conv2, bn2):
        self.conv1, self.bn1, self.conv2, self.bn2 = conv1, bn1, conv2, bn2
        self.st = None


class ResNetEngine(SkipEngine):
    kind = "resnet"

    def __init__(self, net, first_conv, blocks, tail_conv, tail_bn, out_conv, need_residual: bool, pad: str,
                 act_slope: float = 0.2):
        self._init_common(net, True, pad, act_slope)
        self.defer_scale = -1
        self.nscales, self.sc = 0, []
        self.need_residual = bool(need_residual)
        self.first = ConvRec(first_conv, self.pad_mode, "first")
        self.blocks = []
        self.bns = []
        for k, (c1, b1, c2, b2) in enumerate(blocks):
            blk = ResBlockRec(ConvRec(c1, N.PAD_ZERO, f"b{k}.conv1"), BNRec(b1, f"b{k}.bn1"),
                              ConvRec(c2, N.PAD_ZERO, f"b{k}.conv2"), BNRec(b2, f"b{k}.bn2"))
            self.blocks.append(blk)
            self.bns += [blk.bn1, blk.bn2]
        self.tail = ConvRec(tail_conv, N.PAD_ZERO, "tail")
        self.tail_bn = BNRec(tail_bn, "tail_bn")
        self.bns.append(self.tail_bn)
        self.out_conv = ConvRec(out_conv, self.pad_mode, "out")
        self.convs = [self.first] + [c for b in self.blocks for c in (b.conv1, b.conv2)] + [self.tail, self.out_conv]
        self.param_list = list(net.parameters())
        self.gin = None
        self._check_supported()

    def _check_supported(self):
        super()._check_supported()
        if self.first.Cout % 4:
            raise NotImplementedError("dip-amd: internal channel counts must be multiples of 4")
        for r in self.convs:
            if r.ks != 3 or r.stride != 1:
                raise NotImplementedError(f"dip-amd: ResNet conv {r.name}: only 3x3 stride-1 convs are planned")
            if r is not self.first and r is not self.out_conv and tuple(r.module.padding) != (1, 1):
                raise NotImplementedError(f"dip-amd: ResNet conv {r.name}: padding {r.module.padding} (the join needs equal sizes)")

    def _net_cin(self) -> int:
        return self.first.Cin

    def _input_gin(self):
        return self.gin

    def _has_big_layer(self, H, W) -> bool:
        return any(r.Cin >= 96 and r.Cout >= 96 and H * W >= 65536 for r in self.convs)

    def _emit_join_fwd(self, xa: Act, xb: Act, out, name):
        if self._sizing:
            return
        ta, tb = xa.transform(), xb.transform()
        self.keep += [ta, tb]
        self.fwd_ops.append((self.lib.dip_res_join_fwd, (_ptr(xa.buf), xa.Cs, C.byref(ta), _ptr(xb.buf), xb.Cs, C.byref(tb),
# ... 148 lines not shown
```

deep-image-prior_amd/dip_group.py:

```python
from __future__ import annotations

import contextlib
import ctypes as C

import torch

import dip_native as N
from dip_native import round_up

_ALIGN = 256


class Slab:

    def __init__(self, device):
        self.device = device
        self.buf = None
        self.off = 0
        self.sizes = []

    def bind(self, row0: torch.Tensor):
        self.buf, self.measured, self.off, self.replay = row0, self.off, 0, 0

    def alloc(self, n, dtype=torch.float32, zero=False):
# ... 240 lines not shown
        stds = list(param_noise_std) if isinstance(param_noise_std, (list, tuple)) or hasattr(param_noise_std, "__len__") \
            else [param_noise_std] * B
        if len(stds) != B:
            raise ValueError(f"GroupedFits: param_noise_std is one float or one per instance: got {len(stds)} for {B} nets")
        if any(not float(s) >= 0.0 for s in stds):
            raise ValueError(f"dip-amd: GroupedFits: param_noise_std must be >= 0, got {stds}")
        sd = list(seeds) if param_noise_seeds is None else [int(s) for s in param_noise_seeds]
        if len(sd) != B:
            raise ValueError(f"GroupedFits: param_noise_seeds holds one seed per instance: got {len(sd)} for {B} nets")
        return float(weight_decay), [float(s) for s in stds], [s & 0xFFFFFFFFFFFFFFFF for s in sd]

    def _sgld_state(self, b):
        s = N.DipSgldState(0, self.param_noise_seeds[b], self.param_noise_std[b], 0.0)
        return torch.frombuffer(bytearray(bytes(s)), dtype=torch.int64)

    def set_param_noise_std(self, std):
        if not self.sgld:
            raise ValueError("dip-amd: GroupedFits.set_param_noise_std on a group without SGLD: construct it with "
                             "param_noise_std= / weight_decay=")
        _, stds, _ = self._check_sgld(self.weight_decay, std, self.param_noise_seeds, self.B, self.seeds)
        for b, s in enumerate(stds):
            self._inst(self._row0_extra["sgld"], b).view(torch.float32)[4:5].fill_(s)
        self.param_noise_std = stds

    def param_noise_offsets(self):
        return [int(self._inst(self._row0_extra["sgld"], b)[0].item()) & 0xFFFFFFFFFFFFFFFF for b in range(self.B)]

    def set_tv_weights(self, tv_weights):
        if self.tv_weights is None:
            raise ValueError("dip-amd: GroupedFits.set_tv_weights on a group without a TV term: construct a new group")
        ws, _ = self._check_tv(tv_weights, self.tv_beta, self.B, self.downsamplers)
        if ws is None:
            raise ValueError("dip-amd: GroupedFits.set_tv_weights: switching the TV term off changes the launch list; construct "
                             "a new group")
        for b, w in enumerate(ws):
            self._inst(self._row0_extra["tv_weight"], b).fill_(w)
        self.tv_weights = ws

    @staticmethod
    def _check_downsamplers(downsamplers, B, masks):
        from models.downsampler import Downsampler
        from utils.loss_head import sr_check_fixed_taps, sr_support
        downs = list(downsamplers)
        if len(downs) != B:
            raise ValueError(f"GroupedFits: one Downsampler per instance: got {len(downs)} for {B} nets")
        if masks is not None:
            raise ValueError("GroupedFits: masks and downsamplers exclude each other (the super-resolution loss has no mask)")
        for b, d in enumerate(downs):
            if not isinstance(d, Downsampler):
                raise TypeError(f"dip-amd: GroupedFits needs models.downsampler.Downsampler objects, instance {b} is a "
                                f"{type(d).__name__}")
            sr_check_fixed_taps(d, who="GroupedFits")
            if sr_support(d) != sr_support(downs[0]):
                raise ValueError(f"GroupedFits: the Downsampler of instance {b} has (k, factor, pad) = {sr_support(d)}, "
                                 f"instance 0 has {sr_support(downs[0])}: one launch list serves one filter support")
            if d.downsampler_.weight.shape[0] != downs[0].downsampler_.weight.shape[0]:
                raise ValueError(f"GroupedFits: the Downsampler of instance {b} differs from instance 0 in planes")
        return downs

    def pointers_outside_row0(self):
        lo, hi = self.mem.data_ptr(), self.mem.data_ptr() + self.stride
        bad = []

        def visit(name, field, v):
            if isinstance(v, C.Structure):
                for f, _ in v._fields_:
                    visit(name, field + "." + f, getattr(v, f))
            elif isinstance(v, int) and v >= (1 << 32) and not (lo <= v < hi):
                bad.append((name, field))

        eng = self.eng
        for ops in (eng.fwd_ops, eng.bwd_ops):
            for fn, args, name in ops:
                for k, a in enumerate(args):
                    visit(name, f"arg{k}", a._obj if hasattr(a, "_obj") else a)

        def pointer_args(ops):
            for fn, args, name in ops:
                for k, a in enumerate(args):
                    if not hasattr(a, "_obj"):
                        visit(name, f"arg{k}", a)

        visit("sr_loss" if self.downsamplers is not None else "loss_head", "desc", self._head)
        pointer_args(self._head_fwd + self._head_bwd)
        for _, prefix, desc, ops in self._monitors():
            visit({"mon_": "fit_monitor", "es_": "early_stop"}.get(prefix, prefix[:-1]), "desc", getattr(self, desc))
            pointer_args(getattr(self, ops))
        for k, t in self._row0_extra.items():
            if t is not None:
                visit("extra", k, t.data_ptr())
        for k in ("params", "grads", "packed", "pack_recs", "x_nhwc", "dy_out", "bnbuf", "nbt"):
            visit("engine", k, getattr(eng, k).data_ptr())
        if eng.bf3:
            visit("engine", "packed3", eng.packed3.data_ptr())
            visit("engine", "pack_recs3", eng.pack_recs3.data_ptr())
        return bad

    @staticmethod
    def _mask4(m):
        m = m.detach().float()
        while m.dim() < 4:
            m = m[None]
        return m.contiguous()

    def _build_row0(self, slab, Cimg, H, W, t0, m0):
        from utils import loss_head as LH
        eng, lib, sr, tv = self.eng, self.lib, self.downsamplers is not None, self.tv_weights is not None
        eng.slab = slab
        eng._build_arenas(self.device)
        if Cimg != eng.sc[0].down_a.Cin:
            raise RuntimeError(f"dip-amd: input has {Cimg} channels, net expects {eng.sc[0].down_a.Cin}")
        eng._build_plan(H, W, Cimg)
        Cn, Hn, Wn = eng.n_out, eng.Hout, eng.Wout
        if sr:
            geom = k, f, pad, Ho, Wo = LH.sr_geometry(self.downsamplers[0], Hn, Wn, who="GroupedFits")
            if (Ho, Wo) != tuple(t0.shape[2:]):
                raise ValueError(f"GroupedFits: targets (the LR images) are {tuple(t0.shape[2:])}, the down-sampled net output is "
                                 f"{(Ho, Wo)} (net output {(Hn, Wn)}, k {k}, factor {f}, pad {pad})")
        elif (Hn, Wn) != tuple(t0.shape[2:]):
            raise ValueError(f"GroupedFits: targets are {tuple(t0.shape[2:])}, the net output is {(Hn, Wn)}")
        nin, nout = Cimg * H * W, Cn * Hn * Wn
        ex = {}
        ex["saved"] = slab.alloc(nin)
        ex["noisy"] = slab.alloc(nin) if self.std > 0 else None
        ex["rng"] = slab.alloc(2, torch.int64, zero=True)
        if sr:
            ex["taps"] = slab.alloc(k * k)
            ex["target"] = slab.alloc(Cn * Ho * Wo)
            ex["mask"] = None
            ex["out"] = slab.alloc(nout)
            ex["y"] = slab.alloc(Cn * Ho * Wo)
            self.nblk = lib.dip_sr_loss_nblk(Cn, Ho, Wo)
            ex["partials"] = slab.alloc(self.nblk)
            if tv:
                self.tv_nblk = lib.dip_sr_tv_nblk(Cn, Hn, Wn)
                ex["tv_weight"] = slab.alloc(1)
                ex["tv_partials"] = slab.alloc(self.tv_nblk)
        else:
            ex["target"] = slab.alloc(nout)
            ex["mask"] = slab.alloc(self.mask_c * Hn * Wn) if m0 is not None else None
            ex["out"] = slab.alloc(nout)
            self.nblk = lib.dip_loss_head_nblk(Hn * Wn, eng.out_conv.Cin)
            ex["partials"] = slab.alloc(self.nblk)
        ex["loss"] = slab.alloc(1, zero=True)
        ex["gl"] = slab.alloc(1)
        ex["gl"].fill_(1.0)
        ex["m"] = slab.alloc(eng.n_arena, zero=True)
        ex["v"] = slab.alloc(eng.n_arena, zero=True)
        ex["iter"] = slab.alloc(16, torch.uint8, zero=True)
        self._row0_extra = ex
        self._x = ex["noisy"] if self.std > 0 else ex["saved"]
        at = lambda k: None if ex[k] is None else ex[k].data_ptr()
        if sr:
            self._head = LH.sr_descriptor(eng, geom, at("out"), at("taps"), at("target"), at("y"), at("partials"), self.nblk,
                                          at("loss"))
            if tv:
                self._head = LH.sr_tv_descriptor(self._head, at("tv_weight"), at("tv_partials"), self.tv_nblk, self.tv_beta)
            fwd, bwd = LH.sr_fwd_launches, LH.sr_bwd_launches
        else:
            self._head, self._tr = LH.mse_descriptor(eng, at("target"), at("mask"), self.mask_c, at("out"), at("partials"),
                                                     self.nblk, at("loss"))
            fwd, bwd = LH.mse_fwd_launches, LH.mse_bwd_launches
        self._with_out_conv = sr
        self._head_fwd, self._head_bwd = fwd(eng, self._head), bwd(eng, self._head, at("gl"))
        for m, prefix, desc, ops in self._monitors():
            d, launches = self._carve_monitor(slab, m, prefix)
            setattr(self, desc, d)
            setattr(self, ops, launches)
        if self.sgld:
            import dip_optim
            plist = eng.param_list
            self._sgld_ranges = dip_optim.noise_ranges(plist, eng.slots, [p for p in plist if p.dim() == 4])
            if len(self._sgld_ranges) > dip_optim.SGLD_MAX_RANGES:
                raise RuntimeError(f"dip-amd: GroupedFits: {len(self._sgld_ranges)} noised ranges; dip_adam_sgld_step_dev takes at "
                                   f"most {dip_optim.SGLD_MAX_RANGES}")
            self._sgld_n = eng.slots[-1] + plist[-1].numel()
            ex["sgld"] = slab.alloc(3, torch.int64, zero=True)
            ex["sgld_ranges"] = slab.alloc(max(2 * len(self._sgld_ranges), 1), torch.int64, zero=True)
            ex["sgld"].copy_(self._sgld_state(0))
            if self._sgld_ranges:
                ex["sgld_ranges"][:2 * len(self._sgld_ranges)].copy_(
                    torch.tensor(self._sgld_ranges, dtype=torch.int64).reshape(-1))

    def _monitor_sizes(self, m):
        from utils.fit_monitor import monitor_sizes
        eng, ex = self.eng, self._row0_extra
        return monitor_sizes(m, self.lib.dip_fit_monitor_nblk, ex["out"].numel(), (eng.n_out, eng.Hout, eng.Wout), (),
                             n_lr=None if ex.get("y") is None else ex["y"].numel(), n_arena=eng.n_arena)

    def _carve_monitor(self, slab, m, prefix):
        from utils import fit_monitor as FM
        eng, ex = self.eng, self._row0_extra
        if self.downsamplers is not None and prefix == "mon_":
            m._check_hr(self.B, (1, eng.n_out, eng.Hout, eng.Wout))
        if prefix == "ssim_":
            m._check_out(self.B, (1, eng.n_out, eng.Hout, eng.Wout))
        z = self._monitor_sizes(m)
        t = dict(out=ex["out"], out_LR=ex.get("y"), noisy=ex["target"], img=ex["target"], img_LR=ex["target"], mask=ex["mask"],
                 mask_c=self.mask_c, hw=eng.Hout * eng.Wout, loss=ex["loss"], avg=ex.get("mon_avg"))
        for b in m.BUFFERS:
            buf = None
            if b.when(m):
                buf = slab.alloc(b.count(z), b.dtype, zero=b.init == "zero")
                if b.init == "early_stop":
                    FM.early_stop_state_fill(buf)
            t[b.name] = ex[prefix + (b.key or b.name)] = buf
        desc = m._descriptor(t)
        arena = t[m.ARENA[0]] if m.ARENA else None
        return desc, FM.monitor_launches(self.lib, desc, eng.params.data_ptr(), eng.n_arena,
                                         None if arena is None else arena.data_ptr())

    def _off(self, t0):
        o = t0.data_ptr() - self.mem.data_ptr()
        assert 0 <= o and o + t0.numel() * t0.element_size() <= self.stride, "tensor is not in row 0 of the slab"
        return o

    def _inst(self, t0, b):
        o = self._off(t0) + b * self.stride
        return self.mem[o:o + t0.numel() * t0.element_size()].view(t0.dtype)

    def _strided(self, t0, *shape):
        if t0 is None:
            return None
        es = t0.element_size()
        assert self.stride % es == 0
        flat = self.mem.view(t0.dtype)
        inner = [1] * len(shape)
        for d in range(len(shape) - 2, -1, -1):
            inner[d] = inner[d + 1] * shape[d + 1]
        return torch.as_strided(flat, (self.B,) + tuple(shape), [self.stride // es] + inner,
                                flat.storage_offset() + self._off(t0) // es)

    def _adopt_net(self, b):
        eng = self.eng
        net = self.nets[b]
        prow = self._inst(eng.params, b)
        for p, o in zip(net.parameters(), eng.slots):
            n = p.numel()
            prow[o:o + n].copy_(p.detach().reshape(-1).to(device=self.device, dtype=torch.float32))
            p.data = prow[o:o + n].view(p.shape)
            p.grad = None
        bnrow, nbtrow = self._inst(eng.bnbuf, b), self._inst(eng.nbt, b)
        bn_mods = [m for m in net.modules() if isinstance(m, torch.nn.BatchNorm2d)]
        by_name = dict(net.named_modules())
        names0 = {id(m): k for k, m in self.nets[0].named_modules()}
        for k, rec in enumerate(eng.bns):
            m = by_name[names0[id(rec.module)]]
            if rec.rm_off >= 0:
                bnrow[rec.rm_off:rec.rm_off + rec.C].copy_(m.running_mean.to(self.device))
                bnrow[rec.rv_off:rec.rv_off + rec.C].copy_(m.running_var.to(self.device))
                nbtrow[k] = m.num_batches_tracked.to(self.device)
                m._buffers["running_mean"] = bnrow[rec.rm_off:rec.rm_off + rec.C]
                m._buffers["running_var"] = bnrow[rec.rv_off:rec.rv_off + rec.C]
                m._buffers["num_batches_tracked"] = nbtrow[k]
        assert len(bn_mods) == len(eng.bns)

    def _iteration(self):
        eng, lib, ex = self.eng, self.lib, self._row0_extra
        dev = self.device
        main = torch.cuda.current_stream(dev)
        st = main.cuda_stream
        N.check(lib.dip_group_begin(self.B, self.stride, self.mem.data_ptr(), self.stride), "group_begin")
        try:
            if self.std > 0:
                N.check(lib.dip_noise_axpy_dev2(ex["saved"].data_ptr(), ex["noisy"].data_ptr(), ex["saved"].numel(), self.std,
                                                ex["rng"].data_ptr(), st), "noise_axpy_dev2")
            eng._launch_forward(self._x.data_ptr(), main, with_out_conv=self._with_out_conv)
            for fn, args, name in self._head_fwd:
                N.check(fn(*args, st), name)
            for fn, args, name in self._head_bwd:
                N.check(fn(*args, st), name)
            eng._launch_backward(main)
            for _, _, _, ops in self._monitors():
                for fn, args, name in getattr(self, ops):
                    N.check(fn(*args, st), name)
            N.check(lib.dip_adam_tick(ex["iter"].data_ptr(), self.lr, self.ADAM_BETAS[0], self.ADAM_BETAS[1], st), "adam_tick")
            if self.sgld:
                N.check(lib.dip_adam_sgld_step_dev(eng.params.data_ptr(), eng.grads.data_ptr(), ex["m"].data_ptr(),
                                                   ex["v"].data_ptr(), self._sgld_n, self.ADAM_BETAS[0], self.ADAM_BETAS[1],
                                                   self.ADAM_EPS, self.weight_decay, ex["iter"].data_ptr(),
                                                   ex["sgld"].data_ptr(), ex["sgld_ranges"].data_ptr(),
                                                   len(self._sgld_ranges), st), "adam_sgld_step_dev")
            else:
                N.check(lib.dip_adam_step_dev(eng.params.data_ptr(), eng.grads.data_ptr(), ex["m"].data_ptr(),
                                              ex["v"].data_ptr(), eng.n_arena, self.ADAM_BETAS[0], self.ADAM_BETAS[1],
                                              self.ADAM_EPS, ex["iter"].data_ptr(), st), "adam_step_dev")
        finally:
            lib.dip_group_end()
        if len(eng.bns):
            self._nbt_all.add_(1)
        if self.out_avg is not None and self.monitor is None:
            if self.iterations == 0 and self.ema_first and not torch.cuda.is_current_stream_capturing():
                self.out_avg.copy_(self.out)
            else:
                self.out_avg.mul_(self.exp_weight).add_(self.out, alpha=1 - self.exp_weight)

    def _check_room(self, n):
        for m, *_ in self._monitors():
            m._check_room(n)

    def _issued(self, n):
        self.iterations += n
        for m, *_ in self._monitors():
            m.i += n

    def step(self, n=1):
        self._check_room(n)
        if self._dry:
            raise RuntimeError("dip-amd: a dry (host-memory) GroupedFits cannot launch anything")
        with torch.cuda.device(self.device):
            for _ in range(int(n)):
                self._iteration()
                self._issued(1)

    def capture(self, warmup=3):
        dev = self.device
        with torch.cuda.device(dev):
            cur = torch.cuda.current_stream(dev)
            self.capture_stream = torch.cuda.Stream(dev)
            self.capture_stream.wait_stream(cur)
            with torch.cuda.stream(self.capture_stream):
                self.step(max(int(warmup), 1))
            cur.wait_stream(self.capture_stream)
            torch.cuda.synchronize(dev)
            self.graph = torch.cuda.CUDAGraph()
            with torch.cuda.graph(self.graph, stream=self.capture_stream):
                self._iteration()
        return self

    def run(self, n=1):
        if self.graph is None:
            return self.step(n)
        self._check_room(n)
        for _ in range(int(n)):
            self.graph.replay()
        self._issued(int(n))

    def run_until(self, max_iter, check_every=50):
        es = self.early_stop
        if es is None:
            raise RuntimeError("dip-amd: GroupedFits.run_until needs early_stop=GroupedEarlyStopMonitor(...)")
        max_iter, check_every = max(int(max_iter), 0), int(check_every)
        if check_every < 1:
            raise ValueError(f"dip-amd: run_until: check_every must be >= 1, got {check_every}")
        self._check_room(max_iter)
        issued = 0
        while issued < max_iter:
            n = min(check_every, max_iter - issued)
            self.run(n)
            issued += n
            if all(es.stopped):
                break
        return issued

    def step_counts(self):
# ... 2 lines not shown
```

deep-image-prior_amd/dip_native.py:

```python
from __future__ import annotations

import ctypes as C
import os

_HERE = os.path.dirname(os.path.abspath(__file__))
LIB_PATH = os.path.join(_HERE, "lib", "libdip_hip.so")
ABI_VERSION = 8

PAD_ZERO, PAD_REFLECT, PAD_REPLICATE = 0, 1, 2
UP_NEAREST, UP_BILINEAR = 0, 1

c_float_p = C.c_void_p


class DipTransform(C.Structure):
    _fields_ = [("a", C.c_void_p), ("b", C.c_void_p), ("slope", C.c_float)]


class DipPackRec(C.Structure):
    _fields_ = [("w_off", C.c_int64), ("fwd_off", C.c_int64), ("dgrad_off", C.c_int64),
                ("Cout", C.c_int32), ("Cin", C.c_int32), ("KS", C.c_int32),
                ("CinP4", C.c_int32), ("CoutP32", C.c_int32), ("CoutP4", C.c_int32), ("CinP32", C.c_int32)]


class DipPackRec3(C.Structure):
    _fields_ = [("w_off", C.c_int64), ("fwd_off", C.c_int64), ("dgrad_off", C.c_int64),
                ("Cout", C.c_int32), ("Cin", C.c_int32), ("KS", C.c_int32),
                ("nchF", C.c_int32), ("CoutP32", C.c_int32), ("nchD", C.c_int32), ("CinP32", C.c_int32)]


class DipBnFin(C.Structure):
    _fields_ = [("gamma", C.c_void_p), ("beta", C.c_void_p), ("eps", C.c_float), ("momentum", C.c_float),
                ("state", C.c_void_p), ("Cs", C.c_int32), ("C", C.c_int32), ("running_mean", C.c_void_p),
                ("running_var", C.c_void_p), ("ticket", C.c_void_p)]


class DipBnbFin(C.Structure):
    _fields_ = [("dgamma", C.c_void_p), ("dbeta", C.c_void_p), ("coef", C.c_void_p), ("C", C.c_int32),
                ("npix", C.c_int32), ("ticket", C.c_void_p)]


class DipConvDesc(C.Structure):
    _fields_ = [("x", C.c_void_p), ("Hin", C.c_int32), ("Win", C.c_int32), ("Cx", C.c_int32), ("Cin", C.c_int32),
                ("tr", DipTransform), ("wp", C.c_void_p), ("bias", C.c_void_p), ("y", C.c_void_p),
                ("Hout", C.c_int32), ("Wout", C.c_int32), ("Cy", C.c_int32), ("Cout", C.c_int32),
                ("y_pitch", C.c_int32),
                ("ks", C.c_int32), ("stride", C.c_int32), ("pad_mode", C.c_int32), ("off", C.c_int32),
                ("dil", C.c_int32), ("accumulate", C.c_int32), ("stats", C.c_void_p),
                ("ksplit", C.c_int32), ("ws", C.c_void_p),
                ("bnb_y", C.c_void_p), ("bnb_state", C.c_void_p), ("bnb_partials", C.c_void_p),
                ("bnb_partials_thin", C.c_void_p), ("bnb_Cy", C.c_int32), ("bnb_Cs", C.c_int32),
                ("bnb_pad", C.c_int32), ("bnb_slope", C.c_float),
                ("wp3", C.c_void_p)]


class DipWgradDesc(C.Structure):
    _fields_ = [("x", C.c_void_p), ("Hin", C.c_int32), ("Win", C.c_int32), ("Cx", C.c_int32), ("Cin", C.c_int32),
                ("tr", DipTransform), ("dy", C.c_void_p),
                ("Hout", C.c_int32), ("Wout", C.c_int32), ("Cdy", C.c_int32), ("Cout", C.c_int32),
                ("ks", C.c_int32), ("stride", C.c_int32), ("pad_mode", C.c_int32), ("off", C.c_int32),
                ("partial", C.c_void_p), ("bias_partial", C.c_void_p), ("nsplit", C.c_int32),
                ("tap_groups", C.c_int32), ("chan_block", C.c_int32)]


class DipGradSrc(C.Structure):
    _fields_ = [("g", C.c_void_p), ("pad", C.c_int32), ("fold", C.c_int32), ("Cg", C.c_int32), ("choff", C.c_int32),
                ("win_y", C.c_int32), ("win_x", C.c_int32), ("win_h", C.c_int32), ("win_w", C.c_int32),
                ("tw", C.c_void_p), ("tn", C.c_int32), ("tcw", C.c_int32)]


class DipUpcatDesc(C.Structure):
    _fields_ = [("s", C.c_void_p), ("Cs_s", C.c_int32), ("ns", C.c_int32), ("ts", DipTransform),
                ("d", C.c_void_p), ("Cs_d", C.c_int32), ("nd", C.c_int32), ("td", DipTransform),
                ("H", C.c_int32), ("W", C.c_int32), ("mode", C.c_int32),
                ("cat", C.c_void_p), ("Cs_cat", C.c_int32),
                ("stats", C.c_void_p), ("nblk", C.c_int32),
                ("Hs", C.c_int32), ("Ws", C.c_int32), ("os_y", C.c_int32), ("os_x", C.c_int32),
                ("Hd", C.c_int32), ("Wd", C.c_int32), ("od_y", C.c_int32), ("od_x", C.c_int32)]


class DipCmd(C.Structure):
    _fields_ = [("kind", C.c_int32), ("fn", C.c_int32), ("stream", C.c_int32), ("event", C.c_int32),
                ("slots", C.POINTER(C.c_uint64)), ("nslots", C.c_int32), ("reserved", C.c_int32)]


class DipPhase(C.Structure):
    _fields_ = [("cmds", C.POINTER(DipCmd)), ("events", C.POINTER(C.c_void_p)), ("n", C.c_int32), ("nevents", C.c_int32)]


class DipIterState(C.Structure):
    _fields_ = [("step", C.c_uint64), ("step_size", C.c_float), ("bc2_sqrt", C.c_float)]


class DipLossHeadDesc(C.Structure):
    _fields_ = [("u", C.c_void_p), ("Cu", C.c_int32), ("Cin", C.c_int32), ("tr", DipTransform),
                ("w", C.c_void_p), ("bias", C.c_void_p), ("Cout", C.c_int32), ("HW", C.c_int32),
                ("sigmoid", C.c_int32), ("target", C.c_void_p), ("mask", C.c_void_p), ("mask_c", C.c_int32),
                ("out", C.c_void_p), ("partials", C.c_void_p), ("nblk", C.c_int32), ("loss", C.c_void_p)]


class DipSRLossDesc(C.Structure):
    _fields_ = [("out", C.c_void_p), ("taps", C.c_void_p), ("target", C.c_void_p), ("y", C.c_void_p),
                ("partials", C.c_void_p), ("nblk", C.c_int32), ("loss", C.c_void_p),
                ("C", C.c_int32), ("H", C.c_int32), ("W", C.c_int32), ("k", C.c_int32), ("f", C.c_int32),
                ("pad", C.c_int32), ("Ho", C.c_int32), ("Wo", C.c_int32), ("sigmoid", C.c_int32)]


class DipSRTVDesc(C.Structure):
    _fields_ = [("sr", DipSRLossDesc), ("tv_weight", C.c_void_p), ("tv_partials", C.c_void_p), ("tv_nblk", C.c_int32),
                ("beta", C.c_float)]

    loss = property(lambda self: self.sr.loss, lambda self, v: setattr(self.sr, "loss", v))
    out = property(lambda self: self.sr.out)


class DipFitMonitorDesc(C.Structure):
    _fields_ = [("out", C.c_void_p), ("noisy", C.c_void_p), ("gt", C.c_void_p), ("out_avg", C.c_void_p), ("n", C.c_int64),
                ("exp_weight", C.c_float), ("backtrack_db", C.c_float), ("loss", C.c_void_p), ("partial", C.c_void_p),
                ("records", C.c_void_p), ("capacity", C.c_int32), ("show_every", C.c_int32), ("backtracking", C.c_int32),
                ("reserved", C.c_int32), ("counter", C.c_void_p), ("state", C.c_void_p)]


class DipSRMonitorDesc(C.Structure):
    _fields_ = [("out_HR", C.c_void_p), ("out_LR", C.c_void_p), ("img_HR", C.c_void_p), ("img_LR", C.c_void_p),
                ("n_hr", C.c_int64), ("n_lr", C.c_int64), ("loss", C.c_void_p), ("partial", C.c_void_p),
                ("records", C.c_void_p), ("capacity", C.c_int32), ("reserved", C.c_int32), ("counter", C.c_void_p)]


class DipRestoreMonitorDesc(C.Structure):
    _fields_ = [("out", C.c_void_p), ("img", C.c_void_p), ("mask", C.c_void_p), ("n", C.c_int64), ("hw", C.c_int64),
                ("mask_c", C.c_int32), ("backtrack_db", C.c_float), ("loss", C.c_void_p), ("partial", C.c_void_p),
                ("records", C.c_void_p), ("capacity", C.c_int32), ("show_every", C.c_int32), ("backtracking", C.c_int32),
                ("reserved", C.c_int32), ("counter", C.c_void_p), ("state", C.c_void_p)]


class DipEarlyStopDesc(C.Structure):
    _fields_ = [("out", C.c_void_p), ("ring", C.c_void_p), ("mean", C.c_void_p), ("partial", C.c_void_p),
                ("records", C.c_void_p), ("state", C.c_void_p), ("counter", C.c_void_p), ("best_out", C.c_void_p),
                ("n", C.c_int64), ("window", C.c_int32), ("patience", C.c_int32), ("capacity", C.c_int32),
                ("loss", C.c_void_p)]


class DipEarlyStopEmvDesc(C.Structure):
    _fields_ = [("out", C.c_void_p), ("mean", C.c_void_p), ("partial", C.c_void_p), ("records", C.c_void_p),
                ("state", C.c_void_p), ("counter", C.c_void_p), ("best_out", C.c_void_p), ("n", C.c_int64),
                ("alpha", C.c_double), ("warmup", C.c_int32), ("patience", C.c_int32), ("capacity", C.c_int32),
                ("reserved", C.c_int32)]


class DipSgldState(C.Structure):
    _fields_ = [("offset", C.c_uint64), ("seed", C.c_uint64), ("std", C.c_float), ("pad_", C.c_float)]


class DipPosteriorDesc(C.Structure):
    _fields_ = [("out", C.c_void_p), ("mean", C.c_void_p), ("m2", C.c_void_p), ("count", C.c_void_p), ("counter", C.c_void_p),
                ("n", C.c_int64), ("burn_in", C.c_int32), ("every", C.c_int32)]


class DipSsimDesc(C.Structure):
    _fields_ = [("out", C.c_void_p), ("avg", C.c_void_p), ("gt", C.c_void_p), ("map", C.c_void_p), ("partial", C.c_void_p),
                ("records", C.c_void_p), ("counter", C.c_void_p), ("capacity", C.c_int32), ("C", C.c_int32), ("H", C.c_int32),
                ("W", C.c_int32), ("c1", C.c_float), ("c2", C.c_float), ("pivot", C.c_float), ("nblk", C.c_int32)]


assert C.sizeof(DipSgldState) == 24 and C.sizeof(DipPosteriorDesc) == 56
assert C.sizeof(DipSsimDesc) == 88
assert C.sizeof(DipEarlyStopDesc) == 96 and C.sizeof(DipEarlyStopEmvDesc) == 88

_SIGS = {
    "dip_abi_version": (C.c_int, []),
    "dip_build_id": (C.c_char_p, []),
    "dip_last_error": (C.c_char_p, []),
    "dip_device_pci_bus_id": (C.c_int, [C.c_int, C.c_char_p, C.c_int]),
    "dip_list_fn_id": (C.c_int, [C.c_char_p]),
    "dip_list_fn_nargs": (C.c_int, [C.c_int]),
    "dip_list_run": (C.c_int, [C.POINTER(DipCmd), C.c_int, C.POINTER(C.c_void_p), C.c_int, C.POINTER(C.c_void_p), C.c_int,
                               C.POINTER(C.c_int)]),
    "dip_iter_run": (C.c_int, [C.POINTER(DipPhase), C.c_int, C.POINTER(C.c_void_p), C.c_int, C.POINTER(C.c_int)]),
    "dip_events_create": (C.c_int, [C.POINTER(C.c_void_p), C.c_int]),
    "dip_events_destroy": (C.c_int, [C.POINTER(C.c_void_p), C.c_int]),
    "dip_nchw_to_nhwc": (C.c_int, [C.c_void_p, C.c_void_p, C.c_int, C.c_int, C.c_int, C.c_void_p]),
# ... 37 lines not shown
    "dip_conv_wgrad_ntiles": (C.c_int, [C.c_int, C.c_int]),
    "dip_wgrad_thin": (C.c_int, [C.POINTER(DipWgradDesc), C.c_void_p]),
    "dip_wgrad_thin_eligible": (C.c_int, [C.POINTER(DipWgradDesc)]),
    "dip_wgrad_thin_shape_ok": (C.c_int, [C.c_int, C.c_int, C.c_int, C.c_int, C.c_int, C.c_int]),
    "dip_wgrad_thin_nsplit": (C.c_int, [C.c_int, C.c_int, C.c_int, C.c_int, C.c_int, C.c_int]),
    "dip_wgrad_plan": (C.c_int, [C.c_int, C.c_int, C.c_int, C.c_int, C.c_int, C.c_int, C.POINTER(C.c_int)]),
    "dip_wgrad_plan2": (C.c_int, [C.c_int, C.c_int, C.c_int, C.c_int, C.c_int, C.c_int, C.POINTER(C.c_int),
                                  C.POINTER(C.c_int), C.POINTER(C.c_int)]),
    "dip_wgrad_reduce": (C.c_int, [C.c_void_p, C.c_void_p, C.c_int, C.c_int, C.c_int, C.c_int, C.c_void_p,
                                   C.c_void_p, C.c_void_p]),
    "dip_bn_finalize": (C.c_int, [C.c_void_p, C.c_int, C.c_int, C.c_int, C.c_void_p, C.c_void_p, C.c_float,
                                  C.c_float, C.c_void_p, C.c_int, C.c_void_p, C.c_void_p, C.c_void_p]),
    "dip_bn_bwd_stats": (C.c_int, [C.POINTER(DipGradSrc), C.c_void_p, C.c_int, C.c_int, C.c_int, C.c_int,
                                   C.c_void_p, C.c_int, C.c_float, C.c_void_p, C.c_int, C.c_void_p, C.c_int,
                                   C.c_void_p]),
    "dip_bn_bwd_nblk": (C.c_int, [C.c_int, C.c_int, C.c_int]),
    "dip_bn_bwd_finalize": (C.c_int, [C.c_void_p, C.c_int, C.c_int, C.c_int, C.c_int, C.c_void_p, C.c_void_p,
                                      C.c_void_p, C.c_void_p]),
    "dip_bn_bwd_finalize2": (C.c_int, [C.c_void_p, C.c_int, C.c_void_p, C.c_int, C.c_int, C.c_int, C.c_int, C.c_int,
                                       C.c_void_p, C.c_void_p, C.c_void_p, C.c_void_p]),
    "dip_bn_bwd_apply": (C.c_int, [C.c_void_p, C.c_int, C.c_void_p, C.c_int, C.c_int, C.c_int, C.c_void_p, C.c_int,
                                   C.c_void_p, C.c_void_p]),
    "dip_bn_bwd_apply_src": (C.c_int, [C.POINTER(DipGradSrc), C.c_void_p, C.c_int, C.c_int, C.c_int, C.c_int,
                                       C.c_void_p, C.c_int, C.c_float, C.c_void_p, C.c_void_p, C.c_int, C.c_void_p]),
    "dip_bn_bwd_fin_rows_ok": (C.c_int, [C.c_int, C.c_int]),
    "dip_bn_bwd_apply_fin": (C.c_int, [C.c_void_p, C.c_int, C.c_void_p, C.c_int, C.c_int, C.c_int, C.c_void_p, C.c_int,
                                       C.c_void_p, C.c_int, C.c_void_p, C.c_void_p, C.c_void_p, C.c_void_p]),
    "dip_bn_bwd_apply_src_fin": (C.c_int, [C.POINTER(DipGradSrc), C.c_void_p, C.c_int, C.c_int, C.c_int, C.c_int, C.c_void_p,
                                           C.c_int, C.c_float, C.c_void_p, C.c_int, C.c_void_p, C.c_void_p, C.c_void_p,
                                           C.c_void_p, C.c_int, C.c_void_p]),
    "dip_bn_bwd_one_ok": (C.c_int, [C.c_int, C.c_int]),
    "dip_bn_bwd_one": (C.c_int, [C.POINTER(DipGradSrc), C.c_void_p, C.c_int, C.c_int, C.c_int, C.c_int, C.c_void_p, C.c_int,
                                 C.c_float, C.c_void_p, C.c_int, C.c_void_p, C.c_void_p, C.c_void_p, C.c_void_p]),
    "dip_upsample_bwd_one": (C.c_int, [C.c_void_p, C.c_int, C.c_int, C.c_int, C.c_int, C.c_int, C.c_int, C.c_int, C.c_int,
                                       C.c_int, C.c_void_p, C.c_int, C.c_int, C.c_void_p, C.c_int, C.c_float, C.c_void_p,
                                       C.c_int, C.c_void_p, C.c_void_p, C.c_void_p, C.c_void_p]),
    "dip_fold_to_nchw": (C.c_int, [C.POINTER(DipGradSrc), C.c_int, C.c_int, C.c_int, C.c_void_p, C.c_void_p]),
    "dip_fold_to_nhwc": (C.c_int, [C.POINTER(DipGradSrc), C.c_int, C.c_int, C.c_int, C.c_void_p, C.c_int, C.c_void_p]),
    "dip_res_join_fwd": (C.c_int, [C.c_void_p, C.c_int, C.POINTER(DipTransform), C.c_void_p, C.c_int, C.POINTER(DipTransform),
                                   C.c_void_p, C.c_int, C.c_int, C.c_int, C.c_void_p]),
    "dip_res_join_bwd": (C.c_int, [C.c_void_p, C.c_int, C.POINTER(DipGradSrc), C.c_void_p, C.c_int, C.POINTER(DipTransform),
                                   C.c_void_p, C.c_int, C.c_int, C.c_int, C.c_int, C.c_void_p]),
    "dip_upcat_fwd": (C.c_int, [C.POINTER(DipUpcatDesc), C.c_void_p]),
    "dip_upcat_nblk": (C.c_int, [C.c_int, C.c_int, C.c_int]),
    "dip_upcat_fwd_fin": (C.c_int, [C.POINTER(DipUpcatDesc), C.POINTER(DipBnFin), C.c_void_p]),
    "dip_fin_rows_ok": (C.c_int, [C.c_int, C.c_int]),
    "dip_bn_bwd_stats_fin": (C.c_int, [C.POINTER(DipGradSrc), C.c_void_p, C.c_int, C.c_int, C.c_int, C.c_int,
                                       C.c_void_p, C.c_int, C.c_float, C.c_void_p, C.c_int, C.c_void_p, C.c_int,
                                       C.POINTER(DipBnbFin), C.c_void_p]),
    "dip_upsample_bwd_stats_crop_fin": (C.c_int, [C.c_void_p, C.c_int, C.c_int, C.c_int, C.c_int, C.c_int, C.c_int,
                                                  C.c_int, C.c_int, C.c_int, C.c_void_p, C.c_int, C.c_int, C.c_void_p,
                                                  C.c_int, C.c_float, C.c_void_p, C.c_int, C.c_void_p, C.c_int,
                                                  C.POINTER(DipBnbFin), C.c_void_p]),
    "dip_avgpool2_fwd": (C.c_int, [C.c_void_p, C.c_int, C.c_int, C.c_int, C.c_int, C.c_void_p, C.c_int, C.c_void_p,
                                   C.c_int, C.c_void_p]),
    "dip_avgpool2_bwd": (C.c_int, [C.c_void_p, C.c_int, C.c_int, C.c_int, C.c_int, C.c_void_p, C.c_int, C.c_void_p]),
    "dip_maxpool2_fwd": (C.c_int, [C.c_void_p, C.c_int, C.c_int, C.c_int, C.c_int, C.c_void_p, C.c_int, C.c_void_p,
                                   C.c_int, C.c_void_p]),
    "dip_maxpool2_bwd": (C.c_int, [C.c_void_p, C.c_void_p, C.c_int, C.c_int, C.c_int, C.c_int, C.c_int, C.c_void_p,
                                   C.c_int, C.c_void_p]),
    "dip_upsample_bwd_stats": (C.c_int, [C.c_void_p, C.c_int, C.c_int, C.c_int, C.c_int, C.c_int, C.c_void_p,
                                         C.c_int, C.c_int, C.c_void_p, C.c_int, C.c_float, C.c_void_p, C.c_int,
                                         C.c_void_p, C.c_int, C.c_void_p]),
    "dip_upsample_bwd_stats_crop": (C.c_int, [C.c_void_p, C.c_int, C.c_int, C.c_int, C.c_int, C.c_int, C.c_int, C.c_int,
                                              C.c_int, C.c_int, C.c_void_p, C.c_int, C.c_int, C.c_void_p, C.c_int,
                                              C.c_float, C.c_void_p, C.c_int, C.c_void_p, C.c_int, C.c_void_p]),
    "dip_adam_step": (C.c_int, [C.c_void_p, C.c_void_p, C.c_void_p, C.c_void_p, C.c_int64, C.c_double, C.c_double,
                                C.c_double, C.c_double, C.c_int, C.c_void_p]),
    "dip_noise_axpy": (C.c_int, [C.c_void_p, C.c_void_p, C.c_int64, C.c_float, C.c_uint64, C.c_uint64, C.c_void_p]),
    "dip_adam_tick": (C.c_int, [C.c_void_p, C.c_double, C.c_double, C.c_double, C.c_void_p]),
    "dip_adam_step_dev": (C.c_int, [C.c_void_p, C.c_void_p, C.c_void_p, C.c_void_p, C.c_int64, C.c_double, C.c_double,
                                    C.c_double, C.c_void_p, C.c_void_p]),
    "dip_noise_axpy_dev": (C.c_int, [C.c_void_p, C.c_void_p, C.c_int64, C.c_float, C.c_uint64, C.c_void_p, C.c_void_p]),
    "dip_noise_axpy_dev2": (C.c_int, [C.c_void_p, C.c_void_p, C.c_int64, C.c_float, C.c_void_p, C.c_void_p]),
    "dip_counter_add": (C.c_int, [C.c_void_p, C.c_uint64, C.c_void_p]),
    "dip_counter_add_n": (C.c_int, [C.c_void_p, C.c_int, C.c_uint64, C.c_void_p]),
    "dip_group_begin": (C.c_int, [C.c_int, C.c_longlong, C.c_void_p, C.c_longlong]),
    "dip_group_end": (C.c_int, []),
    "dip_group_size": (C.c_int, []),
    "dip_group_native": (C.c_int, [C.c_int]),
    "dip_loss_head_nblk": (C.c_int, [C.c_int, C.c_int]),
    "dip_loss_head_fwd": (C.c_int, [C.POINTER(DipLossHeadDesc), C.c_void_p]),
    "dip_loss_head_bwd": (C.c_int, [C.POINTER(DipLossHeadDesc), C.c_void_p, C.c_void_p, C.c_int, C.c_void_p]),
    "dip_sr_loss_nblk": (C.c_int, [C.c_int, C.c_int, C.c_int]),
    "dip_sr_loss_fwd": (C.c_int, [C.POINTER(DipSRLossDesc), C.c_void_p]),
    "dip_sr_loss_bwd": (C.c_int, [C.POINTER(DipSRLossDesc), C.c_void_p, C.c_void_p, C.c_int, C.c_void_p]),
    "dip_sr_tv_nblk": (C.c_int, [C.c_int, C.c_int, C.c_int]),
    "dip_sr_tv_loss_fwd": (C.c_int, [C.POINTER(DipSRTVDesc), C.c_void_p]),
    "dip_sr_tv_loss_bwd": (C.c_int, [C.POINTER(DipSRTVDesc), C.c_void_p, C.c_void_p, C.c_int, C.c_void_p]),
    "dip_fit_monitor_nblk": (C.c_int, [C.c_int64]),
    "dip_fit_monitor": (C.c_int, [C.c_void_p, C.c_void_p, C.c_void_p, C.c_void_p, C.c_int64, C.c_float, C.c_int,
                                  C.c_void_p, C.c_void_p, C.c_void_p, C.c_void_p, C.c_int, C.c_float, C.c_void_p]),
    "dip_fit_monitor_dev": (C.c_int, [C.POINTER(DipFitMonitorDesc), C.c_void_p]),
    "dip_arena_backtrack": (C.c_int, [C.c_void_p, C.c_void_p, C.c_int64, C.c_void_p, C.c_void_p]),
    "dip_sr_monitor": (C.c_int, [C.c_void_p, C.c_void_p, C.c_void_p, C.c_void_p, C.c_int64, C.c_int64, C.c_void_p, C.c_void_p,
                                 C.c_void_p, C.c_void_p]),
    "dip_sr_monitor_dev": (C.c_int, [C.POINTER(DipSRMonitorDesc), C.c_void_p]),
    "dip_restore_monitor": (C.c_int, [C.c_void_p, C.c_void_p, C.c_void_p, C.c_int, C.c_int64, C.c_int64, C.c_void_p, C.c_void_p,
                                      C.c_void_p, C.c_void_p, C.c_int, C.c_float, C.c_void_p]),
    "dip_restore_monitor_dev": (C.c_int, [C.POINTER(DipRestoreMonitorDesc), C.c_void_p]),
    "dip_early_stop_dev": (C.c_int, [C.POINTER(DipEarlyStopDesc), C.c_void_p]),
    "dip_early_stop_keep": (C.c_int, [C.c_void_p, C.c_void_p, C.c_int64, C.c_void_p, C.c_void_p]),
    "dip_early_stop_emv_dev": (C.c_int, [C.POINTER(DipEarlyStopEmvDesc), C.c_void_p]),
    "dip_adam_sgld_step": (C.c_int, [C.c_void_p, C.c_void_p, C.c_void_p, C.c_void_p, C.c_int64, C.c_double, C.c_double,
                                     C.c_double, C.c_double, C.c_double, C.c_int, C.c_float, C.c_uint64, C.c_uint64,
                                     C.c_void_p, C.c_int, C.c_void_p]),
    "dip_adam_sgld_step_dev": (C.c_int, [C.c_void_p, C.c_void_p, C.c_void_p, C.c_void_p, C.c_int64, C.c_double, C.c_double,
                                         C.c_double, C.c_double, C.c_void_p, C.c_void_p, C.c_void_p, C.c_int, C.c_void_p]),
    "dip_posterior_dev": (C.c_int, [C.POINTER(DipPosteriorDesc), C.c_void_p]),
    "dip_ssim_nblk": (C.c_int, [C.c_int, C.c_int, C.c_int]),
    "dip_ssim_dev": (C.c_int, [C.POINTER(DipSsimDesc), C.c_void_p]),
    "dip_lanczos_down_fwd": (C.c_int, [C.c_void_p, C.c_void_p, C.c_void_p, C.c_int, C.c_int, C.c_int, C.c_int,
                                       C.c_int, C.c_int, C.c_void_p]),
    "dip_lanczos_down_bwd": (C.c_int, [C.c_void_p, C.c_void_p, C.c_void_p, C.c_int, C.c_int, C.c_int, C.c_int,
                                       C.c_int, C.c_int, C.c_void_p]),
    "dip_down_dense_fwd": (C.c_int, [C.c_void_p, C.c_void_p, C.c_void_p, C.c_void_p, C.c_int, C.c_int, C.c_int, C.c_int,
                                     C.c_int, C.c_int, C.c_void_p]),
    "dip_down_dense_bwd_data": (C.c_int, [C.c_void_p, C.c_void_p, C.c_void_p, C.c_int, C.c_int, C.c_int, C.c_int,
                                          C.c_int, C.c_int, C.c_void_p]),
    "dip_down_dense_bwd_weight": (C.c_int, [C.c_void_p, C.c_void_p, C.c_void_p, C.c_void_p, C.c_int, C.c_int, C.c_int,
                                            C.c_int, C.c_int, C.c_int, C.c_void_p]),
}

EXPORTS = tuple(_SIGS.keys())
_lib = None


def lib():
    global _lib
    if _lib is None:
        if not os.path.exists(LIB_PATH):
            raise RuntimeError(
                f"{LIB_PATH} is missing: the deep-image-prior MI355X backend has no fallback path. "
                "Build it with `python __graft_entry__.py build` (needs hipcc, targets gfx950).")
        L = C.CDLL(LIB_PATH)
        for name, (res, args) in _SIGS.items():
            fn = getattr(L, name)
            fn.restype = res
            fn.argtypes = args
        if L.dip_abi_version() != ABI_VERSION:
            raise RuntimeError(f"libdip_hip.so ABI {L.dip_abi_version()} != binding ABI {ABI_VERSION}")
        _lib = L
    return _lib


def check(rc: int, what: str = ""):
    if rc != 0:
        msg = lib().dip_last_error()
        raise RuntimeError(f"libdip_hip {what} failed (rc={rc}): {msg.decode() if msg else ''}")


def round_up(x: int, m: int) -> int:
    return (x + m - 1) // m * m


def conv_plan(Hout, Wout, Cin, Cout, ks, stride):
    k, rows, wsf = C.c_int(), C.c_int(), C.c_int64()
    check(lib().dip_conv_plan(Hout, Wout, Cin, Cout, ks, stride, C.byref(k), C.byref(rows), C.byref(wsf)), "conv_plan")
    return k.value, rows.value, wsf.value


def conv_plan_fp32(Hout, Wout, Cin, Cout, ks, stride):
    k, rows, wsf = C.c_int(), C.c_int(), C.c_int64()
    check(lib().dip_conv_plan_fp32(Hout, Wout, Cin, Cout, ks, stride, C.byref(k), C.byref(rows), C.byref(wsf)), "conv_plan_fp32")
    return k.value, rows.value, wsf.value

# ... 134 lines not shown
```

deep-image-prior_amd/dip_optim.py:

```python
from __future__ import annotations

import os

import torch

import dip_native as N


class _Group:

    def __init__(self, params):
        self.params = params
        self.base = params[0].data_ptr()
        last = params[-1]
        self.numel = (last.data_ptr() - self.base) // 4 + last.numel()
        dev = params[0].device
        self.m = torch.zeros(self.numel, dtype=torch.float32, device=dev)
        self.v = torch.zeros(self.numel, dtype=torch.float32, device=dev)
        self.gbuf = None
        self.offsets = [(p.data_ptr() - self.base) // 4 for p in params]


def _split_contiguous(params, max_gap=4):
    groups, run = [], []
# ... 316 lines not shown
            raise RuntimeError("dip-amd: NativeIteration works on MI355X tensors only (net_input is on the CPU; no CPU "
                               "fallback)")
        if net_input.dim() != 4 or net_input.shape[0] != 1 or net_input.dtype != torch.float32 \
                or not net_input.is_contiguous():
            raise ValueError(f"dip-amd: net_input must be a contiguous fp32 [1,C,H,W] tensor, got {net_input.dtype} "
                             f"{tuple(net_input.shape)}")
        if net_input.requires_grad:
            raise ValueError("dip-amd: net_input requires grad (opt_over='net,input'): that goes through the eager closure")
        if not isinstance(head, (MSEHead, SRHead)):
            raise TypeError(f"dip-amd: NativeIteration needs a utils.loss_head.MSEHead or SRHead, got {type(head).__name__}")
        if head.net is not net:
            raise ValueError(f"dip-amd: the {type(head).__name__} was built for another net")
        head._check_state()
        if reg_noise is not None:
            if not isinstance(reg_noise, RegNoise):
                raise TypeError("dip-amd: reg_noise must be a utils.reg_noise.RegNoise or None, got "
                                f"{type(reg_noise).__name__}")
            if reg_noise.saved.shape != net_input.shape or reg_noise.saved.device != net_input.device:
                raise ValueError("dip-amd: the RegNoise was built for another net_input")
        self.head, self.opt = head, optimizer
        self._check_monitors()
        self.net_input, self.reg = net_input.detach(), reg_noise
        self.out = None
        self.iterations = 0
        self._key = None
        self._plan = None
        self._one = torch.ones(1, dtype=torch.float32, device=self.device)
        self._check_capture()

    def _check_capture(self):
        if torch.cuda.is_current_stream_capturing():
            raise RuntimeError("dip-amd: NativeIteration.step() cannot be captured into a hipGraph (its loss slot changes per "
                               "iteration); capture the eager closure with GraphedIteration instead")

    def _check_training(self):
        if not self.net.training:
            raise NotImplementedError("dip-amd: eval-mode BatchNorm is not implemented (NativeIteration needs net.train())")

    def _monitors(self):
        return [(slot, getattr(self, slot)) for slot in ("monitor", "early_stop", "posterior", "ssim")
                if getattr(self, slot) is not None]

    def _check_monitors(self):
        import utils.fit_monitor as FM
        takes = {"monitor": ((FM.FitMonitor, FM.SRFitMonitor, FM.RestorationFitMonitor), "dip-amd: monitor must be a "
                             "utils.fit_monitor.FitMonitor, an SRFitMonitor, a RestorationFitMonitor or None", "back-tracks"),
                 "early_stop": (FM.EarlyStopMonitor, "dip-amd: early_stop must be a utils.fit_monitor.EarlyStopMonitor or None",
                                "keeps the parameters of"),
                 "posterior": (FM.PosteriorMonitor, "dip-amd: posterior must be a utils.fit_monitor.PosteriorMonitor or None",
                               "samples"),
                 "ssim": (FM.SSIMMonitor, "dip-amd: ssim must be a utils.fit_monitor.SSIMMonitor or None", "records")}
        head = getattr(self, "head", None)
        for slot, m in self._monitors():
            types, refusal, copies = takes[slot]
            if not isinstance(m, types):
                raise TypeError(f"{refusal}, got {type(m).__name__}")
            if head is not None and m.head_kind not in (None, head.kind):
                raise TypeError(f"dip-amd: an SRFitMonitor records out_LR and out_HR of a utils.loss_head.SRHead, the head is a "
                                f"{type(head).__name__} (use a FitMonitor)")
            if m.dev != self.device:
                raise RuntimeError(f"dip-amd: the {type(m).__name__} lives on {m.dev}, the iteration runs on {self.device}")
            if m.engine is not None and m.engine is not self.engine:
                raise ValueError(f"dip-amd: the {type(m).__name__} {copies} another net (it was built for a different skip() net)")

    def _signature(self, sig):
        eng, head, opt, reg = self.engine, self.head, self.opt, self.reg
        return (id(eng._clists), eng.shape_key, id(getattr(eng, "fwd_ops", None)), id(getattr(eng, "bwd_ops", None)), sig,
                *opt._plan_key(),
                head._plan_key(),
                None if reg is None else (reg.std, reg.seed, id(reg.saved), id(reg.out), id(reg.offset))) \
            + tuple((slot, m._plan_key()) for slot, m in self._monitors())

    def _build(self):
        eng, head, opt, reg = self.engine, self.head, self.opt, self.reg
        lib = N.lib()
        dev = self.device
        self._check_monitors()
        noisy = reg is not None and reg.std > 0
        x = self.net_input if reg is None else (reg.out if noisy else reg.saved)
        _, Cimg, H, W = x.shape
        eng._prepare(dev, H, W, Cimg)
        if opt._sig != opt._signature():
            opt._prepare()
        fwd, bwd = eng.iteration_lists(with_out_conv=head.with_out_conv)
        out = self.out
        if out is None or tuple(out.shape) != (1, eng.n_out, eng.Hout, eng.Wout) or out.device != dev:
            out = torch.empty((1, eng.n_out, eng.Hout, eng.Wout), dtype=torch.float32, device=dev)
        loss0 = torch.zeros((), dtype=torch.float32, device=dev)
        desc = head._descriptor(eng, out, loss0)
        pre = []
        if noisy:
            pre.append((lib.dip_noise_axpy_dev, (reg.saved.data_ptr(), reg.out.data_ptr(), reg.saved.numel(), reg.std,
                                                 reg.seed, reg.offset.data_ptr()), "noise_axpy_dev"))
        pre += eng._forward_prologue(x.data_ptr())
        mid = head.fwd_launches(eng, desc)
        if len(eng.bns):
            mid.append((lib.dip_counter_add_n, (eng.nbt.data_ptr(), eng.nbt.numel(), 1), "num_batches_tracked"))
        mid += head.bwd_launches(eng, desc, self._one.data_ptr())
        st = opt._state(dev, opt.step_count)
        b1, b2 = float(opt.betas[0]), float(opt.betas[1])
        adam = [(lib.dip_adam_tick, (st.data_ptr(), float(opt.lr), b1, b2), "adam_tick")]
        pbase, gbase = eng.params.data_ptr(), eng.grads.data_ptr()
        for g in opt._groups:
            if g.params[0].device != dev or g.base < pbase or g.base + 4 * g.numel > pbase + 4 * eng.params.numel():
                raise RuntimeError("dip-amd: a FusedAdam group lies outside the net's parameter arena")
            adam.append(opt._step_launch(lib, g, gbase + (g.base - pbase), st))
        on_main = lambda ops: N.CmdList([("launch", fn, args, 0, name) for fn, args, name in ops])
        phases = [on_main(pre), fwd, on_main(mid), bwd, on_main(adam)]
        descs = {}
        for slot, m in self._monitors():
            descs[slot], ops = m._plan(eng, out, head)
            phases.insert(len(phases) - 1, on_main(ops))
        mdesc = descs.get("monitor")
        if mdesc is not None:
            mdesc.loss = loss0.data_ptr()
        lists = N.IterList(phases)
        views = [eng.grads[o:o + p.numel()].view(p.shape) for p, o in zip(eng.param_list, eng.slots)]
        self.out = out
        self._plan = dict(lists=lists, desc=desc, mdesc=mdesc, edesc=descs.get("early_stop"), views=views, x=x, state=st,
                          loss0=loss0,
                          keep=(head._plan_keep(), eng._clists, eng.fwd_ops, eng.bwd_ops, opt._groups,
                                eng.params, eng.grads, eng.nbt, eng.dy_out,
                                None if reg is None else (reg.saved, reg.out, reg.offset),
                                [m._plan_keep() for _, m in self._monitors()]))
        self._key = self._signature(opt._sig)

    def _begin(self, n=1):
        self._check_training()
        self._check_capture()
        self._check_monitors()
        self.head._check_state()
        for _, m in self._monitors():
            m._check_room(n)
        if self._signature(self.opt._signature()) != self._key:
            self._build()
        for _, m in self._monitors():
            m._sync_counter()
        eng = self.engine
        ptrs = [torch.cuda.current_stream(self.device).cuda_stream]
        if eng.two_streams:
            ptrs += [s_.cuda_stream for s_ in eng._aux_streams()[1]]
        return ptrs

    def _issue(self, loss_ptr, ptrs):
        self._plan["desc"].loss = loss_ptr
        if self._plan["mdesc"] is not None:
            self._plan["mdesc"].loss = loss_ptr
        self._plan["lists"].run(ptrs)

    def _finish(self, n):
        eng = self.engine
        for p, v in zip(eng.param_list, self._plan["views"]):
            if p.grad is not v:
                p.grad = v
        eng.fwd_id += n
        eng.last_out, eng.last_head = self.out, self.head
        self.opt.step_count += n
        self.iterations += n
        for _, m in self._monitors():
            m._advance(n)

    @torch.no_grad()
    def step(self):
        with torch.cuda.device(self.device):
            ptrs = self._begin()
            loss = torch.empty((), dtype=torch.float32, device=self.device)
            self._issue(loss.data_ptr(), ptrs)
            self._finish(1)
        return loss

    @torch.no_grad()
    def run(self, n):
        n = max(int(n), 0)
        with torch.cuda.device(self.device):
            losses = torch.empty(n, dtype=torch.float32, device=self.device)
            if n == 0:
                return losses
            ptrs = self._begin(n)
            base = losses.data_ptr()
            done = 0
            try:
                for i in range(n):
                    self._issue(base + 4 * i, ptrs)
                    done += 1
            finally:
                if done:
                    self._finish(done)
        return losses

    def run_until(self, max_iter, check_every=50):
        es = self.early_stop
        if es is None:
            raise RuntimeError("dip-amd: NativeIteration.run_until needs early_stop=EarlyStopMonitor(...)")
        max_iter, check_every = max(int(max_iter), 0), int(check_every)
        if check_every < 1:
            raise ValueError(f"dip-amd: run_until: check_every must be >= 1, got {check_every}")
        es._check_room(max_iter)
        parts, issued = [], 0
        while issued < max_iter:
            n = min(check_every, max_iter - issued)
            parts.append(self.run(n))
            issued += n
            if es.stopped:
                break
        with torch.cuda.device(self.device):
            losses = torch.cat(parts) if parts else torch.empty(0, dtype=torch.float32, device=self.device)
        return issued, losses


class ArenaLBFGS:

    def __init__(self, params, lr=1, max_iter=20, max_eval=None, tolerance_grad=1e-7, tolerance_change=1e-9,
                 history_size=100, _allow_cpu=False):
        self.params = list(params)
# ... 130 lines not shown
```

deep-image-prior_amd/utils/loss_head.py:

```python
import ctypes as C

import torch

import dip_native as N


def mse_descriptor(eng, target_ptr, mask_ptr, mask_c, out_ptr, partials_ptr, nblk, loss_ptr):
    a, oc = eng.last_act, eng.out_conv
    tr = a.transform()
    p = eng.params.data_ptr()
    return N.DipLossHeadDesc(a.buf.data_ptr(), a.Cs, oc.Cin, tr, p + 4 * oc.w_off, p + 4 * oc.b_off if oc.b_off >= 0 else None,
                             oc.Cout, eng.Hout * eng.Wout, 1 if eng.need_sigmoid else 0, target_ptr, mask_ptr, mask_c,
                             out_ptr, partials_ptr, nblk, loss_ptr), tr


def mse_fwd_launches(eng, desc):
    return [(eng.lib.dip_loss_head_fwd, (C.byref(desc),), "loss_head_fwd")]


def mse_bwd_launches(eng, desc, gscale_ptr):
    return [(eng.lib.dip_loss_head_bwd, (C.byref(desc), gscale_ptr, eng.dy_out.data_ptr(), N.round_up(eng.n_out, 4)),
             "loss_head_bwd")]


def sr_check_fixed_taps(d, who="SRHead"):
    if getattr(d, "_dense", False) or getattr(d, "_nondiag", False) or d.downsampler_.weight.requires_grad \
            or d.downsampler_.bias.requires_grad:
        raise NotImplementedError(f"dip-amd: {who} covers the fixed-taps Downsampler; a trainable one (opt_over='down', a "
                                  "loaded non-diagonal weight, or the down-sampler of a skip() net) goes through the "
                                  "spelled closure: out_LR = downsampler(net(x)); mse(out_LR, img_LR)")


def sr_support(d):
    return int(d.kernel.shape[0]), int(d.factor), int(d._pad)


def sr_geometry(d, H, W, who="SRHead"):
    k, f, pad = sr_support(d)
    if H + 2 * pad < k or W + 2 * pad < k:
        raise ValueError(f"{who}: the net output {(H, W)} is smaller than the {k}x{k} filter")
    return k, f, pad, (H + 2 * pad - k) // f + 1, (W + 2 * pad - k) // f + 1


def sr_descriptor(eng, geom, out_ptr, taps_ptr, target_ptr, y_ptr, partials_ptr, nblk, loss_ptr):
    k, f, pad, Ho, Wo = geom
    return N.DipSRLossDesc(out_ptr, taps_ptr, target_ptr, y_ptr, partials_ptr, nblk, loss_ptr, eng.n_out, eng.Hout, eng.Wout,
                           k, f, pad, Ho, Wo, 1 if eng.need_sigmoid else 0)


def sr_check_tv(tv_weight, tv_beta, who="SRHead"):
    import math
    try:
        w, beta = float(tv_weight), float(tv_beta)
    except (TypeError, ValueError):
        raise TypeError(f"dip-amd: {who}: tv_weight / tv_beta must be numbers, got {tv_weight!r} / {tv_beta!r}") from None
    if not math.isfinite(w) or w < 0:
        raise ValueError(f"dip-amd: {who}: tv_weight must be finite and >= 0, got {tv_weight!r}")
    if not math.isfinite(beta) or beta <= 0:
        raise ValueError(f"dip-amd: {who}: tv_beta must be finite and > 0, got {tv_beta!r}")
    return w, beta


def sr_tv_descriptor(sr_desc, tv_weight_ptr, tv_partials_ptr, tv_nblk, beta):
    return N.DipSRTVDesc(sr_desc, tv_weight_ptr, tv_partials_ptr, tv_nblk, beta)


def sr_fwd_launches(eng, desc):
    fn, name = (eng.lib.dip_sr_tv_loss_fwd, "sr_tv_loss_fwd") if isinstance(desc, N.DipSRTVDesc) else \
        (eng.lib.dip_sr_loss_fwd, "sr_loss_fwd")
    return [(eng.lib.dip_head_fwd, (eng.y_out.data_ptr(), desc.out, eng.n_out, eng.Hout * eng.Wout, N.round_up(eng.n_out, 4),
                                    1 if eng.need_sigmoid else 0), "head_fwd"),
            (fn, (C.byref(desc),), name)]


def sr_bwd_launches(eng, desc, gscale_ptr):
    fn, name = (eng.lib.dip_sr_tv_loss_bwd, "sr_tv_loss_bwd") if isinstance(desc, N.DipSRTVDesc) else \
        (eng.lib.dip_sr_loss_bwd, "sr_loss_bwd")
    return [(fn, (C.byref(desc), gscale_ptr, eng.dy_out.data_ptr(), N.round_up(eng.n_out, 4)), name)]


class MSEHead:
    kind = "mse"
    with_out_conv = False
    fwd_launches, bwd_launches = staticmethod(mse_fwd_launches), staticmethod(mse_bwd_launches)

    def __init__(self, net, target, mask=None):
        eng = getattr(net, "__dict__", {}).get("_dip_engine")
        if eng is None or isinstance(eng, Exception):
            raise RuntimeError("dip-amd: MSEHead needs a net built by models.skip.skip()")
        if not target.is_cuda:
            raise RuntimeError("dip-amd: MSEHead works on MI355X tensors only (no CPU fallback)")
        self.net, self.engine = net, eng
        oc = eng.out_conv
        if oc.ks != 1 or oc.Cout > 4:
            raise NotImplementedError("dip-amd: the fused loss head covers a 1x1 output conv with <= 4 channels "
                                      "(n_channels 1 or 3 in every reference notebook)")
        if target.dim() != 4 or target.shape[0] != 1 or target.shape[1] != oc.Cout:
            raise ValueError(f"MSEHead: target must be [1,{oc.Cout},H,W], got {tuple(target.shape)}")
        self.target = target.detach().contiguous().float()
# ... 138 lines not shown
```

include/dip_hip.h:

```cpp
#ifndef DIP_HIP_H
#define DIP_HIP_H

#include <stdint.h>

#ifdef __cplusplus
extern "C" {
#endif

#define DIP_ABI_VERSION 8

#define DIP_PAD_ZERO 0
#define DIP_PAD_REFLECT 1
#define DIP_PAD_REPLICATE 2

#define DIP_ACT_SWISH (-1.0f)
#define DIP_ACT_ELU (-2.0f)
#define DIP_ACT_RELU (-3.0f)

#define DIP_UP_NEAREST 0
#define DIP_UP_BILINEAR 1

int dip_abi_version(void);
const char* dip_build_id(void);
const char* dip_last_error(void);
// ... 95 lines not shown
    float* bnb_partials_thin;
    int32_t bnb_Cy, bnb_Cs, bnb_pad;
    float bnb_slope;
    const void* wp3;
} DipConvDesc;
int dip_conv_igemm(const DipConvDesc* d, void* stream);
int dip_conv_ntiles(int Hout, int Wout);
int dip_conv_thin4_ntiles(int Hout, int Wout);
int dip_conv_bnb_fusable(const DipConvDesc* d);
int dip_conv_plan(int Hout, int Wout, int Cin, int Cout, int ks, int stride, int* ksplit, int* stats_rows,
                  int64_t* ws_floats);
int dip_conv_plan_fp32(int Hout, int Wout, int Cin, int Cout, int ks, int stride, int* ksplit, int* stats_rows,
                       int64_t* ws_floats);
int dip_conv_plan_dil2(int Hout, int Wout, int Cin, int Cout, int ks, int* ksplit, int* stats_rows,
                       int64_t* ws_floats);
int dip_conv_variant(const DipConvDesc* d);
int dip_conv_thin4(const DipConvDesc* d, int ncols, void* stream);
int dip_conv_igemm_dma_cols(const DipConvDesc* d, int n_base, void* stream);
int dip_conv_thin(const DipConvDesc* d, void* stream);
int dip_conv_thin_eligible(const DipConvDesc* d);
int dip_conv_thin_shape_ok(int Hout, int Wout, int Cin, int Cout, int ks, int stride);
int dip_conv_small(const DipConvDesc* d, void* stream);
int dip_conv_small_eligible(const DipConvDesc* d);
int dip_conv_small_rows(const DipConvDesc* d);
int dip_conv_dgrad_ring(const DipConvDesc* d, void* stream);
int dip_conv_dgrad_ring_ok(const DipConvDesc* d);
int dip_conv_bf3_eligible(const DipConvDesc* d);
int dip_conv_bf3_cols(const DipConvDesc* d, int n_base, int ncols, void* stream);
int dip_conv_bf3_terms(void);
int dip_conv_bf3_set_terms(int terms);
int dip_conv_splitk_finish(const DipConvDesc* d, void* stream);

typedef struct DipWgradDesc {
    const float* x;
    int32_t Hin, Win, Cx, Cin;
    DipTransform tr;
    const float* dy;
    int32_t Hout, Wout, Cdy, Cout;
    int32_t ks, stride, pad_mode, off;
    float* partial;
    float* bias_partial;
    int32_t nsplit;
    int32_t tap_groups;
    int32_t chan_block;
} DipWgradDesc;
int dip_conv_wgrad(const DipWgradDesc* d, void* stream);
int dip_wgrad_bf3_eligible(const DipWgradDesc* d);
int dip_wgrad_bf3(const DipWgradDesc* d, void* stream);
int dip_conv_wgrad_tail(const DipWgradDesc* d, void* stream);
int dip_wgrad_tail_stream_ok(const DipWgradDesc* d);
int dip_wgrad_tail_stream(const DipWgradDesc* d, void* stream);
int dip_wgrad_thin(const DipWgradDesc* d, void* stream);
int dip_wgrad_thin_eligible(const DipWgradDesc* d);
int dip_wgrad_thin_shape_ok(int Hout, int Wout, int Cin, int Cout, int ks, int stride);
int dip_wgrad_thin_nsplit(int Hout, int Wout, int Cin, int Cout, int ks, int stride);
int dip_conv_wgrad_ntiles(int Hout, int Wout);
int dip_wgrad_plan(int Hout, int Wout, int Cin, int Cout, int ks, int stride, int* nsplit);
int dip_wgrad_plan2(int Hout, int Wout, int Cin, int Cout, int ks, int stride, int* nsplit, int* tap_groups,
                    int* chan_block);
int dip_wgrad_reduce(const float* partial, const float* bias_partial, int nsplit, int ks, int Cin,
                     int Cout, float* dw , float* dbias , void* stream);

int dip_bn_finalize(const float* partials, int ntiles, int Cstride, int C, const float* gamma,
                    const float* beta, float eps, float momentum, float* state, int Cs,
                    float* running_mean, float* running_var, void* stream);

typedef struct DipGradSrc {
    const float* g;
    int32_t pad, fold, Cg, choff;
    int32_t win_y, win_x, win_h, win_w;
    const float* tw;
    int32_t tn, tcw;
} DipGradSrc;

int dip_bn_bwd_stats(const DipGradSrc* src, const float* y, int H, int W, int Cy, int C,
                     const float* state, int Cs, float slope, float* dz, int Cdz,
                     float* partials , int nblk, void* stream);
int dip_bn_bwd_nblk(int H, int W, int C);
int dip_bn_bwd_stats_fin(const DipGradSrc* src, const float* y, int H, int W, int Cy, int C,
                         const float* state, int Cs, float slope, float* dz, int Cdz,
                         float* partials , int nblk, const DipBnbFin* fin, void* stream);
int dip_bn_bwd_finalize(const float* partials, int nblk, int Cs, int C, int npix, float* dgamma,
                        float* dbeta, float* coef, void* stream);
int dip_bn_bwd_finalize2(const float* partials, int nblk, const float* partials_lo, int nblk_lo, int c_lo, int Cs,
                         int C, int npix, float* dgamma, float* dbeta, float* coef, void* stream);
int dip_bn_bwd_apply(float* dz, int Cdz, const float* y, int Cy, int npix, int C, const float* state,
                     int Cs, const float* coef, void* stream);
int dip_bn_bwd_apply_src(const DipGradSrc* src, const float* y, int H, int W, int Cy, int C,
                         const float* state, int Cs, float slope, const float* coef, float* dy, int Cdy,
                         void* stream);
int dip_bn_bwd_fin_rows_ok(int nrows, int C);
int dip_bn_bwd_apply_fin(float* dz, int Cdz, const float* y, int Cy, int npix, int C, const float* state, int Cs,
                         const float* partials, int nrows, float* dgamma, float* dbeta, float* coef, void* stream);
int dip_bn_bwd_apply_src_fin(const DipGradSrc* src, const float* y, int H, int W, int Cy, int C, const float* state, int Cs,
                             float slope, const float* partials, int nrows, float* dgamma, float* dbeta, float* coef,
                             float* dy, int Cdy, void* stream);
int dip_bn_bwd_one_ok(int npix, int C);
int dip_bn_bwd_one(const DipGradSrc* src, const float* y, int H, int W, int Cy, int C, const float* state, int Cs,
                   float slope, float* dy, int Cdy, float* dgamma, float* dbeta, float* coef, void* stream);
int dip_fold_to_nchw(const DipGradSrc* src, int H, int W, int C, float* dst, void* stream);
int dip_fold_to_nhwc(const DipGradSrc* src, int H, int W, int C, float* dst, int Cd, void* stream);

int dip_res_join_fwd(const float* xa, int Cxa, const DipTransform* ta, const float* xb, int Cxb, const DipTransform* tb,
                     float* out, int Co, int npix, int C, void* stream);
int dip_res_join_bwd(const float* g, int Cg, const DipGradSrc* src, const float* y, int Cy, const DipTransform* ty,
                     float* gout, int Cgo, int H, int W, int C, void* stream);

typedef struct DipUpcatDesc {
    const float* s; int32_t Cs_s, ns; DipTransform ts;
    const float* d; int32_t Cs_d, nd; DipTransform td;
    int32_t H, W, mode;
    float* cat; int32_t Cs_cat;
    float* stats; int32_t nblk;
    int32_t Hs, Ws, os_y, os_x;
    int32_t Hd, Wd, od_y, od_x;
} DipUpcatDesc;
int dip_upcat_fwd(const DipUpcatDesc* d, void* stream);
int dip_upcat_fwd_fin(const DipUpcatDesc* d, const DipBnFin* fin, void* stream);
int dip_fin_rows_ok(int rows, int C);
int dip_upcat_nblk(int H, int W, int C);

int dip_avgpool2_fwd(const float* x, int H, int W, int Cx, int C, float* y, int Cy, float* stats, int nblk,
                     void* stream);
int dip_avgpool2_bwd(const float* dy, int H, int W, int Cdy, int C, float* dx, int Cdx, void* stream);
int dip_maxpool2_fwd(const float* x, int H, int W, int Cx, int C, float* y, int Cy, float* stats, int nblk,
                     void* stream);
int dip_maxpool2_bwd(const float* dy, const float* x, int H, int W, int Cdy, int Cx, int C, float* dx, int Cdx,
                     void* stream);

int dip_upsample_bwd_stats(const float* dcat, int Cs_cat, int choff, int H, int W, int mode,
                           const float* y, int Cy, int C, const float* state, int Cs, float slope,
                           float* dz, int Cdz, float* partials, int nblk, void* stream);
int dip_upsample_bwd_stats_crop(const float* dcat, int Cs_cat, int choff, int H, int W, int Hd, int Wd, int od_y,
                                int od_x, int mode, const float* y, int Cy, int C, const float* state, int Cs,
                                float slope, float* dz, int Cdz, float* partials, int nblk, void* stream);

int dip_upsample_bwd_stats_crop_fin(const float* dcat, int Cs_cat, int choff, int H, int W, int Hd, int Wd, int od_y,
                                    int od_x, int mode, const float* y, int Cy, int C, const float* state, int Cs,
                                    float slope, float* dz, int Cdz, float* partials, int nblk, const DipBnbFin* fin,
                                    void* stream);

int dip_upsample_bwd_one(const float* dcat, int Cs_cat, int choff, int H, int W, int Hd, int Wd, int od_y, int od_x,
                         int mode, const float* y, int Cy, int C, const float* state, int Cs, float slope, float* dy,
                         int Cdy, float* dgamma, float* dbeta, float* coef, void* stream);

int dip_adam_step(float* p, const float* g, float* m, float* v, int64_t n, double lr, double beta1,
                  double beta2, double eps, int step, void* stream);

int dip_noise_axpy(const float* z, float* out, int64_t n, float sigma, uint64_t seed, uint64_t offset,
                   void* stream);

typedef struct DipIterState {
    uint64_t step;
    float step_size;
    float bc2_sqrt;
} DipIterState;
int dip_adam_tick(DipIterState* st, double lr, double beta1, double beta2, void* stream);
int dip_adam_step_dev(float* p, const float* g, float* m, float* v, int64_t n, double beta1, double beta2,
                      double eps, const DipIterState* st, void* stream);
int dip_noise_axpy_dev(const float* z, float* out, int64_t n, float sigma, uint64_t seed, uint64_t* offset_dev,
                       void* stream);
int dip_noise_axpy_dev2(const float* z, float* out, int64_t n, float sigma, uint64_t* state_dev, void* stream);
int dip_counter_add(uint64_t* counter, uint64_t inc, void* stream);
int dip_counter_add_n(uint64_t* counters, int n, uint64_t inc, void* stream);

typedef struct DipSgldState {
    uint64_t offset;
    uint64_t seed;
    float std;
    float pad_;
} DipSgldState;
int dip_adam_sgld_step_dev(float* p, const float* g, float* m, float* v, int64_t n, double beta1, double beta2, double eps,
                           double weight_decay, const DipIterState* st, DipSgldState* noise, const int64_t* ranges,
                           int nranges, void* stream);
int dip_adam_sgld_step(float* p, const float* g, float* m, float* v, int64_t n, double lr, double beta1, double beta2,
                       double eps, double weight_decay, int step, float std, uint64_t seed, uint64_t offset,
                       const int64_t* ranges, int nranges, void* stream);

typedef struct DipLossHeadDesc {
    const float* u;
    int Cu, Cin;
    DipTransform tr;
    const float* w;
    const float* bias;
    int Cout, HW, sigmoid;
    const float* target;
    const float* mask;
    int mask_c;
    float* out;
    float* partials;
    int nblk;
    float* loss;
} DipLossHeadDesc;
int dip_loss_head_nblk(int HW, int Cin);
int dip_loss_head_fwd(const DipLossHeadDesc* d, void* stream);
int dip_loss_head_bwd(const DipLossHeadDesc* d, const float* gscale, float* dy, int Cy, void* stream);

typedef struct DipSRLossDesc {
    const float* out;
    const float* taps;
    const float* target;
    float* y;
    float* partials;
    int nblk;
    float* loss;
    int C, H, W, k, f, pad, Ho, Wo, sigmoid;
} DipSRLossDesc;
int dip_sr_loss_nblk(int C, int Ho, int Wo);
int dip_sr_loss_fwd(const DipSRLossDesc* d, void* stream);
int dip_sr_loss_bwd(const DipSRLossDesc* d, const float* gscale, float* dy, int Cy, void* stream);

typedef struct DipSRTVDesc {
    DipSRLossDesc sr;
    const float* tv_weight;
    float* tv_partials;
    int tv_nblk;
    float beta;
} DipSRTVDesc;
int dip_sr_tv_nblk(int C, int H, int W);
int dip_sr_tv_loss_fwd(const DipSRTVDesc* d, void* stream);
int dip_sr_tv_loss_bwd(const DipSRTVDesc* d, const float* gscale, float* dy, int Cy, void* stream);

int dip_fit_monitor_nblk(int64_t n);
int dip_fit_monitor(const float* out, const float* noisy, const float* gt, float* out_avg, int64_t n,
                    float exp_weight, int first, const float* loss, float* partial, float* record,
                    float* state, int check_backtrack, float backtrack_db, void* stream);
typedef struct DipFitMonitorDesc {
    const float* out;
    const float* noisy;
    const float* gt;
    float* out_avg;
    int64_t n;
    float exp_weight, backtrack_db;
    const float* loss;
    float* partial;
    float* records;
    int capacity, show_every;
    int backtracking;
    int reserved;
    int* counter;
    float* state;
} DipFitMonitorDesc;
int dip_fit_monitor_dev(const DipFitMonitorDesc* d, void* stream);
int dip_arena_backtrack(float* params, float* snapshot, int64_t n, const float* state, void* stream);

typedef struct DipSRMonitorDesc {
    const float* out_HR;
    const float* out_LR;
    const float* img_HR;
    const float* img_LR;
    int64_t n_hr, n_lr;
    const float* loss;
    float* partial;
    float* records;
    int capacity;
    int reserved;
    int* counter;
} DipSRMonitorDesc;
int dip_sr_monitor(const float* out_HR, const float* out_LR, const float* img_HR, const float* img_LR, int64_t n_hr,
                   int64_t n_lr, const float* loss, float* partial, float* record, void* stream);
int dip_sr_monitor_dev(const DipSRMonitorDesc* d, void* stream);

typedef struct DipRestoreMonitorDesc {
    const float* out;
    const float* img;
    const float* mask;
    int64_t n, hw;
    int mask_c;
    float backtrack_db;
    const float* loss;
    float* partial;
    float* records;
    int capacity, show_every;
    int backtracking;
    int reserved;
    int* counter;
    float* state;
} DipRestoreMonitorDesc;
int dip_restore_monitor(const float* out, const float* img, const float* mask, int mask_c, int64_t n, int64_t hw,
// ... 77 lines not shown
```

Before: 189.9.

## Fuse loss head backward and last BN backward stats into forward head kernel

Adds a fused loss-head forward kernel that, besides the output and loss, computes the upstream gradient per pixel and accumulates the final BN backward partial sums and the out-conv weight and bias gradient partials. It assumes unit loss gradient and applies the real gradient scale later in the finalize and reduce kernels. This removes a separate head backward pass and a BN stats pass over the last activation. The cost is a heavier forward kernel with more registers and extra reductions, plus new row buffers.

```diff
diff --git a/deep-image-prior_amd/csrc/bn_kernels.hip b/deep-image-prior_amd/csrc/bn_kernels.hip
--- a/deep-image-prior_amd/csrc/bn_kernels.hip
+++ b/deep-image-prior_amd/csrc/bn_kernels.hip
@@ -188,9 +188,11 @@
 __global__ __launch_bounds__(256) void bn_bwd_finalize_kernel(const float* __restrict__ partials_, int nblk,
                                                               const float* __restrict__ partials_lo_, int nblk_lo,
                                                               int c_lo, int Cs, int C, int npix, float* dgamma_,
-                                                              float* dbeta_, float* coef_, const DipGrpArg<GRP> grp) {
+                                                              float* dbeta_, float* coef_, const float* __restrict__ gscale_,
+                                                              const DipGrpArg<GRP> grp) {
     DIP_GRP_PTR(const float*, partials);
     DIP_GRP_PTR(const float*, partials_lo);
+    DIP_GRP_PTR(const float*, gscale);
     DIP_GRP_PTR(float*, dgamma);
     DIP_GRP_PTR(float*, dbeta);
     DIP_GRP_PTR(float*, coef);
@@ -218,7 +220,8 @@
     __syncthreads();
     if (row < 4 && c0 + row < C) {
         const int c = c0 + row;
-        const double s1 = sh[0][row], s2 = sh[0][4 + row];
+        const double gs = gscale != nullptr ? (double)*gscale : 1.0;
+        const double s1 = sh[0][row] * gs, s2 = sh[0][4 + row] * gs;
         if (dbeta != nullptr) dbeta[c] = (float)s1;
         if (dgamma != nullptr) dgamma[c] = (float)s2;
         coef[c] = (float)(s1 / npix);
@@ -445,7 +448,15 @@
 extern "C" int dip_bn_bwd_finalize(const float* partials, int nblk, int Cs, int C, int npix, float* dgamma,
                                    float* dbeta, float* coef, void* stream) {
     dip_launch_pair<DIP_FAM_BN>(bn_bwd_finalize_kernel<false>, bn_bwd_finalize_kernel<true>, dim3(dip_cdiv(C, 4)), dim3(256), 0, (hipStream_t)stream,
-                                partials, nblk, (const float*)nullptr, 0, 0, Cs, C, npix, dgamma, dbeta, coef);
+                                partials, nblk, (const float*)nullptr, 0, 0, Cs, C, npix, dgamma, dbeta, coef, (const float*)nullptr);
+    DIP_CHECK_LAUNCH();
+    return 0;
+}
+
+extern "C" int dip_bn_bwd_finalize_gs(const float* partials, int nblk, int Cs, int C, int npix, const float* gscale, float* dgamma,
+                                      float* dbeta, float* coef, void* stream) {
+    dip_launch_pair<DIP_FAM_BN>(bn_bwd_finalize_kernel<false>, bn_bwd_finalize_kernel<true>, dim3(dip_cdiv(C, 4)), dim3(256), 0, (hipStream_t)stream,
+                                partials, nblk, (const float*)nullptr, 0, 0, Cs, C, npix, dgamma, dbeta, coef, gscale);
     DIP_CHECK_LAUNCH();
     return 0;
 }
@@ -454,7 +465,7 @@
                                     int Cs, int C, int npix, float* dgamma, float* dbeta, float* coef, void* stream) {
     if ((c_lo & 3) || (c_lo > 0 && partials_lo == nullptr)) DIP_FAIL("bn_bwd_finalize2: c_lo must be a multiple of 4");
     dip_launch_pair<DIP_FAM_BN>(bn_bwd_finalize_kernel<false>, bn_bwd_finalize_kernel<true>, dim3(dip_cdiv(C, 4)), dim3(256), 0, (hipStream_t)stream,
-                                partials, nblk, partials_lo, nblk_lo, c_lo, Cs, C, npix, dgamma, dbeta, coef);
+                                partials, nblk, partials_lo, nblk_lo, c_lo, Cs, C, npix, dgamma, dbeta, coef, (const float*)nullptr);
     DIP_CHECK_LAUNCH();
     return 0;
 }
diff --git a/deep-image-prior_amd/csrc/dip_group.h b/deep-image-prior_amd/csrc/dip_group.h
--- a/deep-image-prior_amd/csrc/dip_group.h
+++ b/deep-image-prior_amd/csrc/dip_group.h
@@ -51,6 +51,9 @@
 }
 template <class F> __host__ __device__ inline void dip_ptrs(DipLossHeadDesc& d, F& f) {
     f(d.u); dip_ptrs(d.tr, f); f(d.w); f(d.bias); f(d.target); f(d.mask); f(d.out); f(d.partials); f(d.loss);
+}
+template <class F> __host__ __device__ inline void dip_ptrs(DipLossHeadFuse& d, F& f) {
+    f(d.bn_state); f(d.bn_rows); f(d.wg_rows);
 }
 template <class F> __host__ __device__ inline void dip_ptrs(DipSRLossDesc& d, F& f) {
     f(d.out); f(d.taps); f(d.target); f(d.y); f(d.partials); f(d.loss);
diff --git a/deep-image-prior_amd/csrc/dip_list.hip b/deep-image-prior_amd/csrc/dip_list.hip
--- a/deep-image-prior_amd/csrc/dip_list.hip
+++ b/deep-image-prior_amd/csrc/dip_list.hip
@@ -42,14 +42,14 @@
     DIP_REG(dip_adam_step), DIP_REG(dip_noise_axpy), DIP_REG(dip_adam_tick), DIP_REG(dip_adam_step_dev),
     DIP_REG(dip_noise_axpy_dev), DIP_REG(dip_noise_axpy_dev2), DIP_REG(dip_counter_add), DIP_REG(dip_counter_add_n),
     DIP_REG(dip_adam_sgld_step), DIP_REG(dip_adam_sgld_step_dev), DIP_REG(dip_posterior_dev),
-    DIP_REG(dip_loss_head_fwd), DIP_REG(dip_loss_head_bwd), DIP_REG(dip_sr_loss_fwd), DIP_REG(dip_sr_loss_bwd),
-    DIP_REG(dip_sr_tv_loss_fwd), DIP_REG(dip_sr_tv_loss_bwd),
+    DIP_REG(dip_loss_head_fwd), DIP_REG(dip_loss_head_bwd), DIP_REG(dip_sr_loss_fwd), DIP_REG(dip_sr_loss_bwd),    DIP_REG(dip_sr_tv_loss_fwd), DIP_REG(dip_sr_tv_loss_bwd),
     DIP_REG(dip_fit_monitor), DIP_REG(dip_fit_monitor_dev), DIP_REG(dip_arena_backtrack),
     DIP_REG(dip_sr_monitor), DIP_REG(dip_sr_monitor_dev), DIP_REG(dip_restore_monitor), DIP_REG(dip_restore_monitor_dev),
     DIP_REG(dip_early_stop_dev), DIP_REG(dip_early_stop_keep), DIP_REG(dip_early_stop_emv_dev),
     DIP_REG(dip_ssim_dev),
     DIP_REG(dip_lanczos_down_fwd), DIP_REG(dip_lanczos_down_bwd), DIP_REG(dip_down_dense_fwd), DIP_REG(dip_down_dense_bwd_data),
     DIP_REG(dip_down_dense_bwd_weight), DIP_REG(dip_res_join_fwd), DIP_REG(dip_res_join_bwd),
+    DIP_REG(dip_loss_head_fwd_fused), DIP_REG(dip_loss_head_wgrad_reduce), DIP_REG(dip_bn_bwd_finalize_gs),
 };
 constexpr int NFN = (int)(sizeof(g_fns) / sizeof(g_fns[0]));
 
diff --git a/deep-image-prior_amd/csrc/loss_kernels.hip b/deep-image-prior_amd/csrc/loss_kernels.hip
--- a/deep-image-prior_amd/csrc/loss_kernels.hip
+++ b/deep-image-prior_amd/csrc/loss_kernels.hip
@@ -76,6 +76,8 @@
     if (tid == 0) d.partials[blockIdx.x] = red[0];
 }
 
+__host__ __device__ inline int head_wg_stride(int Cin, int Cout) { return (Cout * Cin + Cout + 3) & ~3; }
+
 template <int NC4, bool GRP = false>
 __global__ __launch_bounds__(256) void loss_head_fwd_coal_kernel(const DipLossHeadDesc d_, const int ppb, const DipGrpArg<GRP> grp) {
     DIP_GRP_DESC(DipLossHeadDesc, d);
@@ -155,6 +157,204 @@
     if (tid == 0) d.partials[blockIdx.x] = red[0];
 }
 
+template <int NC4, bool GRP = false>
+__global__ __launch_bounds__(256) void loss_head_fwd_fused_kernel(const DipLossHeadDesc d_, const DipLossHeadFuse fu_, const int ppb,
+                                                                  const DipGrpArg<GRP> grp) {
+    DIP_GRP_DESC(DipLossHeadDesc, d);
+    DIP_GRP_DESC(DipLossHeadFuse, fu);
+    __shared__ float red[256];
+    constexpr int PW = 64 / NC4;
+    constexpr int PB = 4 * PW;
+    const int tid = threadIdx.x, lane = tid & 63, wave = tid >> 6;
+    const int cg = lane % NC4, psub = lane / NC4;
+    const bool has_tr = d.tr.a != nullptr;
+    const float slope = has_tr ? d.tr.slope : 1.f;
+    const bool leaky = slope > 0.f;
+    f32x4 ta = f32x4{1.f, 1.f, 1.f, 1.f}, tb = f32x4{0.f, 0.f, 0.f, 0.f};
+    float w[4][4];
+#pragma unroll
+    for (int e = 0; e < 4; ++e) {
+        const int c = cg * 4 + e;
+        if (has_tr && c < d.Cin) { ta[e] = d.tr.a[c]; tb[e] = d.tr.b[c]; }
+#pragma unroll
+        for (int o = 0; o < 4; ++o) w[o][e] = (o < d.Cout && c < d.Cin) ? d.w[(size_t)o * d.Cin + c] : 0.f;
+    }
+    const bool bA = (cg & (NC4 / 2)) != 0, bB = (cg & (NC4 / 4)) != 0;
+    const int myo = 2 * (bA ? 1 : 0) + (bB ? 1 : 0);
+    const bool writer = (cg & (NC4 / 4 - 1)) == 0 && myo < d.Cout;
+    const float mybias = (d.bias != nullptr && myo < d.Cout) ? d.bias[myo] : 0.f;
+    const int p0 = blockIdx.x * ppb, p1 = min(p0 + ppb, d.HW);
+    float lsum = 0.f;
+    const f32x4 bmean = *reinterpret_cast<const f32x4*>(fu.bn_state + cg * 4);
+    const f32x4 brstd = *reinterpret_cast<const f32x4*>(fu.bn_state + fu.bn_Cs + cg * 4);
+    const float kunit = 2.f / ((float)d.Cout * (float)d.HW);
+    f32x4 bs1 = f32x4{0.f, 0.f, 0.f, 0.f}, bs2 = bs1, dbs = bs1;
+    f32x4 dws[4] = {bs1, bs1, bs1, bs1};
+    constexpr int UN = 4;
+    for (int base = p0 + wave * PW; base < p1; base += UN * PB) {
+        const int pb = base + psub;
+        f32x4 u[UN];
+#pragma unroll
+        for (int q = 0; q < UN; ++q) {
+            const int p = pb + q * PB;
+            u[q] = *reinterpret_cast<const f32x4*>(d.u + (size_t)(p < p1 ? p : p0) * d.Cu + cg * 4);
+        }
+#pragma unroll
+        for (int q = 0; q < UN; ++q) {
+            const int p = pb + q * PB;
+            f32x4 v = u[q];
+            if (leaky) {
+#pragma unroll
+                for (int e = 0; e < 4; ++e) v[e] = dip_act_leaky(fmaf(ta[e], v[e], tb[e]), slope);
+            } else {
+#pragma unroll
+                for (int e = 0; e < 4; ++e) v[e] = dip_act(fmaf(ta[e], v[e], tb[e]), slope);
+            }
+            float part[4];
+#pragma unroll
+            for (int o = 0; o < 4; ++o) part[o] = (w[o][0] * v[0] + w[o][1] * v[1]) + (w[o][2] * v[2] + w[o][3] * v[3]);
+            const float k0 = (bA ? part[2] : part[0]) + __shfl_xor(bA ? part[0] : part[2], NC4 / 2);
+            const float k1 = (bA ? part[3] : part[1]) + __shfl_xor(bA ? part[1] : part[3], NC4 / 2);
+            float mine = (bB ? k1 : k0) + __shfl_xor(bB ? k0 : k1, NC4 / 4);
+#pragma unroll
+            for (int sft = NC4 / 8; sft >= 1; sft >>= 1) mine += __shfl_xor(mine, sft);
+            float gun = 0.f;
+            if (p < p1 && writer) {
+                float y = mine + mybias;
+                if (d.sigmoid) y = sigmoidf_(y);
+                d.out[(size_t)myo * d.HW + p] = y;
+                const float t = d.target[(size_t)myo * d.HW + p];
+                float a = y, b = t;
+                if (d.mask != nullptr) {
+                    const float m = d.mask[(size_t)(d.mask_c == 1 ? 0 : myo) * d.HW + p];
+                    a = y * m;
+                    b = t * m;
+                }
+                const float df = a - b;
+                lsum = fmaf(df, df, lsum);
+                {
+                    float g = (a - b) * kunit;
+                    if (d.mask != nullptr) g = g * d.mask[(size_t)(d.mask_c == 1 ? 0 : myo) * d.HW + p];
+                    if (d.sigmoid) g = g * ((1.f - y) * y);
+                    gun = g;
+                }
+            }
+            {
+                float g[4];
+#pragma unroll
+                for (int o = 0; o < 4; ++o) {
+                    const int src = (o >> 1) * (NC4 / 2) + (o & 1) * (NC4 / 4);
+                    float b;
+                    if constexpr (NC4 == 32) {
+                        const float lo = __builtin_bit_cast(float, __builtin_amdgcn_readlane(__builtin_bit_cast(int, gun), src));
+                        const float hi = __builtin_bit_cast(float, __builtin_amdgcn_readlane(__builtin_bit_cast(int, gun), 32 + src));
+                        b = psub ? hi : lo;
+                    } else {
+                        b = __shfl(gun, (lane & ~(NC4 - 1)) + src);
+                    }
+                    g[o] = o < d.Cout ? b : 0.f;
+                }
+                if (p < p1) {
+                    const f32x4 yq = u[q];
+#pragma unroll
+                    for (int e = 0; e < 4; ++e) {
+                        const float du = fmaf(g[3], w[3][e], fmaf(g[2], w[2][e], fmaf(g[1], w[1][e], g[0] * w[0][e])));
+                        const float z = fmaf(ta[e], yq[e], tb[e]);
+                        const float gm = dip_mul_rn(du, dip_act_grad(z, slope));
+                        const float xh = (yq[e] - bmean[e]) * brstd[e];
+                        bs1[e] += gm;
+                        bs2[e] += gm * xh;
+#pragma unroll
+                        for (int o = 0; o < 4; ++o) dws[o][e] = fmaf(g[o], v[e], dws[o][e]);
+                    }
+                    if (cg == 0) {
+#pragma unroll
+                        for (int o = 0; o < 4; ++o) dbs[o] += g[o];
+                    }
+                }
+            }
+        }
+    }
+    red[tid] = lsum;
+    __syncthreads();
+    for (int s2 = 128; s2 >= 1; s2 >>= 1) {
+        if (tid < s2) red[tid] += red[tid + s2];
+        __syncthreads();
+    }
+    if (tid == 0) d.partials[blockIdx.x] = red[0];
+    {
+        __shared__ __attribute__((aligned(16))) float sh[256 * 8];
+        constexpr int RPI = 256 / NC4;
+        const int prow = tid / NC4;
+        dip_tree_sum8(sh, NC4, RPI, prow, cg, true, bs1, bs2);
+        if (prow == 0) {
+            float* o = fu.bn_rows + (size_t)blockIdx.x * 2 * fu.bn_Cs + cg * 4;
+            *reinterpret_cast<f32x4*>(o) = bs1;
+            *reinterpret_cast<f32x4*>(o + fu.bn_Cs) = bs2;
+        }
+        float* wrow = fu.wg_rows + (size_t)blockIdx.x * head_wg_stride(d.Cin, d.Cout);
+        __syncthreads();
+        dip_tree_sum8(sh, NC4, RPI, prow, cg, true, dws[0], dws[1]);
+        if (prow == 0) {
+            *reinterpret_cast<f32x4*>(wrow + cg * 4) = dws[0];
+            if (d.Cout > 1) *reinterpret_cast<f32x4*>(wrow + d.Cin + cg * 4) = dws[1];
+        }
+        if (d.Cout > 2) {
+            __syncthreads();
+            dip_tree_sum8(sh, NC4, RPI, prow, cg, true, dws[2], dws[3]);
+            if (prow == 0) {
+                *reinterpret_cast<f32x4*>(wrow + 2 * d.Cin + cg * 4) = dws[2];
+                if (d.Cout > 3) *reinterpret_cast<f32x4*>(wrow + 3 * d.Cin + cg * 4) = dws[3];
+            }
+        }
+        __syncthreads();
+        f32x4 zero = f32x4{0.f, 0.f, 0.f, 0.f};
+        dip_tree_sum8(sh, NC4, RPI, prow, cg, true, dbs, zero);
+        if (tid == 0) {
+#pragma unroll
+            for (int o = 0; o < 4; ++o)
+                if (o < d.Cout) wrow[d.Cout * d.Cin + o] = dbs[o];
+        }
+    }
+}
+
+template <bool GRP = false>
+__global__ __launch_bounds__(256) void head_wgrad_reduce_kernel(const float* __restrict__ rows_, int nblk, int stride, int nw, int n,
+                                                                const float* __restrict__ gscale_, float* __restrict__ dw_,
+                                                                float* __restrict__ db_, const DipGrpArg<GRP> grp) {
+    DIP_GRP_PTR(const float*, rows);
+    DIP_GRP_PTR(const float*, gscale);
+    DIP_GRP_PTR(float*, dw);
+    DIP_GRP_PTR(float*, db);
+    __shared__ double sh[256][4];
+    const int row = threadIdx.x;
+    const int c0 = blockIdx.x * 4;
+    double a[4] = {0.0, 0.0, 0.0, 0.0};
+#pragma unroll 4
+    for (int t = row; t < nblk; t += 256) {
+        const f32x4 v = *reinterpret_cast<const f32x4*>(rows + (size_t)t * stride + c0);
+#pragma unroll
+        for (int e = 0; e < 4; ++e) a[e] += (double)v[e];
+    }
+#pragma unroll
+    for (int e = 0; e < 4; ++e) sh[row][e] = a[e];
+    for (int s = 128; s >= 1; s >>= 1) {
+        __syncthreads();
+        if (row < s) {
+#pragma unroll
+            for (int e = 0; e < 4; ++e) sh[row][e] += sh[row + s][e];
+        }
+    }
+    __syncthreads();
+    const int c = c0 + row;
+    if (row < 4 && c < n) {
+        const double gs = gscale != nullptr ? (double)*gscale : 1.0;
+        const float r = (float)(sh[0][row] * gs);
+        if (c < nw) dw[c] = r;
+        else if (db != nullptr) db[c - nw] = r;
+    }
+}
+
 template <bool GRP = false>
 __global__ __launch_bounds__(256) void loss_reduce_kernel(const float* __restrict__ partials_, int n, double scale,
                                                           float* __restrict__ loss_, const DipGrpArg<GRP> grp) {
@@ -245,6 +445,60 @@
     return dip_cdiv(HW, head_ppb(HW));
 }
 
+static bool head_no_coal() {
+    static const bool no_coal = getenv("DIP_LOSS_HEAD_NO_COAL") != nullptr;
+    return no_coal;
+}
+
+extern "C" int dip_loss_head_fuse_ok(int Cin, int Cout) {
+    const int nc4 = Cin / 4;
+    return (!head_no_coal() && Cin >= 4 && (Cin & 3) == 0 && nc4 <= 32 && (nc4 & (nc4 - 1)) == 0 && Cout >= 1 && Cout <= 4 &&
+            !(NC4_MIN_CHECK(Cout, nc4))) ? 1 : 0;
+}
+
+extern "C" int dip_loss_head_wg_stride(int Cin, int Cout) { return head_wg_stride(Cin, Cout); }
+
+static int head_reduce_launch(const DipLossHeadDesc& d, int nblk, hipStream_t st) {
+    dip_launch_pair<DIP_FAM_LOSS>(loss_reduce_kernel<false>, loss_reduce_kernel<true>, dim3(1), dim3(256), 0, st,
+                                  (const float*)d.partials, nblk, 1.0 / ((double)d.Cout * (double)d.HW), d.loss);
+    DIP_CHECK_LAUNCH();
+    return 0;
+}
+
+extern "C" int dip_loss_head_fwd_fused(const DipLossHeadDesc* dp, const DipLossHeadFuse* fp, void* stream) {
+    if (dp == nullptr || fp == nullptr) DIP_FAIL("loss_head_fused: NULL descriptor");
+    const DipLossHeadDesc& d = *dp;
+    const DipLossHeadFuse& f = *fp;
+    if (!dip_loss_head_fuse_ok(d.Cin, d.Cout)) DIP_FAIL("loss_head_fused: this head does not take the coalesced kernel (dip_loss_head_fuse_ok)");
+    if ((d.Cu & 3) || d.Cin > d.Cu) DIP_FAIL("loss_head_fused: channel stride must be a multiple of 4 covering Cin");
+    if (d.mask != nullptr && d.mask_c != 1 && d.mask_c != d.Cout) DIP_FAIL("loss_head_fused: mask must have 1 or Cout channels");
+    if (d.tr.a == nullptr || d.tr.b == nullptr || f.bn_state == nullptr || f.bn_rows == nullptr || f.wg_rows == nullptr ||
+        (f.bn_Cs & 3) || f.bn_Cs < d.Cin)
+        DIP_FAIL("loss_head_fused: needs the producer's BatchNorm (transform and state, Cs % 4 == 0 covering Cin) and both row buffers");
+    const int ppb = head_ppb(d.HW);
+    const int nblk = dip_cdiv(d.HW, ppb);
+    if (nblk != d.nblk) DIP_FAIL("loss_head_fused: nblk must come from dip_loss_head_nblk");
+    hipStream_t st = (hipStream_t)stream;
+    switch (d.Cin / 4) {
+        case 32: dip_launch_pair<DIP_FAM_LOSS>(loss_head_fwd_fused_kernel<32>, loss_head_fwd_fused_kernel<32, true>, dim3(nblk), dim3(256), 0, st, d, f, ppb); break;
+        case 16: dip_launch_pair<DIP_FAM_LOSS>(loss_head_fwd_fused_kernel<16>, loss_head_fwd_fused_kernel<16, true>, dim3(nblk), dim3(256), 0, st, d, f, ppb); break;
+        case 8: dip_launch_pair<DIP_FAM_LOSS>(loss_head_fwd_fused_kernel<8>, loss_head_fwd_fused_kernel<8, true>, dim3(nblk), dim3(256), 0, st, d, f, ppb); break;
+        default: dip_launch_pair<DIP_FAM_LOSS>(loss_head_fwd_fused_kernel<4>, loss_head_fwd_fused_kernel<4, true>, dim3(nblk), dim3(256), 0, st, d, f, ppb); break;
+    }
+    DIP_CHECK_LAUNCH();
+    return head_reduce_launch(d, nblk, st);
+}
+
+extern "C" int dip_loss_head_wgrad_reduce(const float* wg_rows, int nblk, int Cin, int Cout, const float* gscale, float* dw, float* db,
+                                          void* stream) {
+    if (wg_rows == nullptr || dw == nullptr || nblk < 1 || Cin < 1 || Cout < 1 || Cout > 4) DIP_FAIL("loss_head_wgrad_reduce: bad arguments");
+    const int stride = head_wg_stride(Cin, Cout);
+    dip_launch_pair<DIP_FAM_LOSS>(head_wgrad_reduce_kernel<false>, head_wgrad_reduce_kernel<true>, dim3(stride / 4), dim3(256), 0,
+                                  (hipStream_t)stream, wg_rows, nblk, stride, Cout * Cin, Cout * Cin + Cout, gscale, dw, db);
+    DIP_CHECK_LAUNCH();
+    return 0;
+}
+
 extern "C" int dip_loss_head_fwd(const DipLossHeadDesc* dp, void* stream) {
     const DipLossHeadDesc& d = *dp;
     if (d.Cout < 1 || d.Cout > 4) DIP_FAIL("loss_head: 1..4 output channels");
@@ -254,7 +508,7 @@
     const int nblk = dip_cdiv(d.HW, ppb);
     if (nblk != d.nblk) DIP_FAIL("loss_head: nblk must come from dip_loss_head_nblk");
     const int nc4 = (d.Cin + 3) / 4;
-    static const bool no_coal = getenv("DIP_LOSS_HEAD_NO_COAL") != nullptr;
+    const bool no_coal = head_no_coal();
     hipStream_t st = (hipStream_t)stream;
     if (no_coal || nc4 > 32 || (nc4 & (nc4 - 1)) != 0 || (NC4_MIN_CHECK(d.Cout, nc4))) {
         dip_launch_pair<DIP_FAM_LOSS>(loss_head_fwd_kernel<false>, loss_head_fwd_kernel<true>, dim3(nblk), dim3(256), 0, st, d, ppb);
diff --git a/deep-image-prior_amd/dip_engine.py b/deep-image-prior_amd/dip_engine.py
--- a/deep-image-prior_amd/dip_engine.py
+++ b/deep-image-prior_amd/dip_engine.py
@@ -110,6 +110,8 @@
         self.fuse_bnb = os.environ.get("DIP_BNB_FUSE", "0") == "1"
         self.fuse_bnb_1x1 = os.environ.get("DIP_BNB_FUSE", "0") == "2"
         self.thin_src = os.environ.get("DIP_NO_THIN_SRC") is None
+        self.head_fuse_on = os.environ.get("DIP_HEAD_FUSE", "0") == "1"
+        self.head_fuse, self.bwd_ops_head, self._head_alloc = False, None, None
         self.use_small = os.environ.get("DIP_CONV_NO_SMALL") is None
         self.ticket_fin = os.environ.get("DIP_TICKET_FIN") == "1"
         self.bnb_one = os.environ.get("DIP_BNB_NO_ONE") is None
@@ -306,6 +308,7 @@
         self._reset_sizing()
         self._alloc = []
         self.n_out = self.out_conv.Cout
+        self.head_fuse, self.bwd_ops_head, self._head_alloc = False, None, None
         if getattr(self, "_bulk2_auto", self.bulk2_max_pixels < 0):
             self._bulk2_auto = True
             self.bulk2_max_pixels = 0 if self._has_big_layer(H, W) else 100000
@@ -330,12 +333,38 @@
                 du_last = (self.dy_out, 0, oc)
             else:
                 du_last = self._emit_dgrad(oc, last, self.dy_out, pre, fuse_bn=True)
-            dy_last = self._emit_bn_act_bwd(last, du_last, pre)
+            head_alt = []
+            dy_last = self._emit_bn_act_bwd(last, du_last, pre, head_alt=head_alt)
             self.dbg_top = {"du_last": du_last, "dy_last": dy_last, "last": last}
             self.last_act = last
             self.bwd_ops = pre + self._bwd_scale_ops(0, dy_last)
             self.bwd_ops += self._flush_deferred_wgrads()
+        self._plan_head_fuse(oc, last, head_alt)
         self.shape_key = (H, W, Cin_img)
+
+    def _plan_head_fuse(self, oc: ConvRec, last: Act, head_alt):
+        if not (self.head_fuse_on and head_alt and self._thin_src_ok(oc, last)
+                and bool(self.lib.dip_loss_head_fuse_ok(oc.Cin, oc.Cout))):
+            return
+        bn, lib = last.bn, self.lib
+        stats, fin, apply, wgrad, wgred = ("bnb_stats:" + bn.name, "bnb_fin:" + bn.name, "bnb_apply:" + bn.name,
+                                           "wgrad:" + oc.name, "wgred:" + oc.name)
+        if not ({stats, apply, wgrad, wgred} <= {name for _, _, name in self.bwd_ops}):
+            return
+        nblk = lib.dip_loss_head_nblk(last.H * last.W, oc.Cin)
+        rows_bn = self._pool["head_bn"] = self._dalloc(nblk * 2 * bn.Cs)
+        rows_wg = self._pool["head_wg"] = self._dalloc(nblk * lib.dip_loss_head_wg_stride(oc.Cin, oc.Cout))
+        gs = self._pool["head_gs"] = self._dalloc(1)
+        gs.fill_(1.0)
+        self._head_alloc = (rows_bn, rows_wg, gs)
+        swap = {stats: (lib.dip_bn_bwd_finalize_gs, (_ptr(rows_bn), nblk, bn.Cs, bn.C, last.H * last.W, _ptr(gs),
+                                                     *self._dparams(bn)), fin),
+                apply: head_alt[0],
+                wgrad: (lib.dip_loss_head_wgrad_reduce, (_ptr(rows_wg), nblk, oc.Cin, oc.Cout, _ptr(gs), _ptr(self.grads, oc.w_off),
+                                                         _ptr(self.grads, oc.b_off) if oc.b_off >= 0 else None),
+                        "wghead:" + oc.name)}
+        self.bwd_ops_head = [swap.get(op[2], op) for op in self.bwd_ops if op[2] not in (fin, wgred)]
+        self.head_fuse, self._head_gs_one = True, True
 
     def _begin_pass(self, sizing: bool):
         self._sizing = sizing
@@ -684,7 +713,7 @@
                     "bnb_fin:" + bn.name))
         self._emit_bnb_apply(a, dz, ops, src)
 
-    def _emit_bn_act_bwd(self, a: Act, g, ops, choff=0, Cg=None, side=False, window=None):
+    def _emit_bn_act_bwd(self, a: Act, g, ops, choff=0, Cg=None, side=False, window=None, head_alt=None):
         bn = a.bn
         nblk = self.lib.dip_bn_bwd_nblk(a.H, a.W, a.C)
         fin_ok = self.ticket_fin and bool(self.lib.dip_fin_rows_ok(nblk, a.C))
@@ -701,6 +730,8 @@
             return dz
         stats = (C.byref(src), *self._act_args(a), None, a.Cs, _ptr(scratch), nblk)
         fused = self._fused_bnb.get(g[0].data_ptr()) if (choff == 0 and not side) else None
+        if fused is None and head_alt is not None:
+            self._emit_bnb_apply(a, dz, head_alt, src)
         if fused is None and fin_ok:
             fin = self._bnb_fin(bn, a.H * a.W, ticket)
             self.keep.append(fin)
@@ -920,7 +951,7 @@
             else:
                 streams[c[1]].wait_event(events[(key, c[2])])
 
-    _BWD_SIDE = staticmethod(lambda n: 2 if n.startswith(("wgrad:", "wgred:")) else
+    _BWD_SIDE = staticmethod(lambda n: 2 if n.startswith(("wgrad:", "wgred:", "wghead:")) else
                              (1 if (n.startswith("dgthin:") or n.endswith(".skip_bn")) else 0))
 
     def _backward_deps(self, ops):
@@ -946,15 +977,16 @@
                 deps.setdefault(consumer, []).append(name)
         return deps
 
-    def _run_backward_two_streams(self, ops, main, compile_only=False):
-        deps = self._bwd_deps if getattr(self, "_bwd_deps_for", None) is ops else None
+    def _run_backward_two_streams(self, ops, main, compile_only=False, key="bwd"):
+        ent = getattr(self, "_bwd_deps_by_key", {}).get(key)
+        deps = ent[1] if ent is not None and ent[0] is ops else None
         if deps is None:
-            deps = self._bwd_deps = self._backward_deps(ops)
-            self._bwd_deps_for = ops
+            deps = self._backward_deps(ops)
+            self._bwd_deps_by_key = dict(getattr(self, "_bwd_deps_by_key", {}), **{key: (ops, deps)})
         capturing = torch.cuda.is_current_stream_capturing()
         bulk2 = self._bulk2 if not capturing else ()
         cls = self._BWD_SIDE if not bulk2 else (lambda n: 3 if n in bulk2 else self._BWD_SIDE(n))
-        return self._issue(ops, main, "bwd_cap" if capturing else "bwd", cls, lambda n: False, deps, compile_only)
+        return self._issue(ops, main, key + "_cap" if capturing else key, cls, lambda n: False, deps, compile_only)
 
     def _run_forward_two_streams(self, ops, main, compile_only=False, drop_last=False):
         side = self._fwd_side
@@ -982,19 +1014,29 @@
             return self._run_forward_two_streams(self.fwd_ops, main, compile_only, drop_last)
         return self._issue(self.fwd_ops, main, "fwd1", compile_only=compile_only, drop_last=drop_last)
 
-    def _launch_backward(self, main, compile_only=False):
+    def head_fused(self, head) -> bool:
+        return bool(self.head_fuse and head is not None and getattr(head, "kind", None) == "mse")
+
+    def head_gs_one(self):
+        if self.head_fuse and not getattr(self, "_head_gs_one", True):
+            self._pool["head_gs"].fill_(1.0)
+            self._head_gs_one = True
+
+    def _launch_backward(self, main, compile_only=False, head_fused=False):
+        ops, sfx = (self.bwd_ops_head, "h") if head_fused else (self.bwd_ops, "")
         if self.two_streams:
-            return self._run_backward_two_streams(self.bwd_ops, main, compile_only)
-        return self._issue(self.bwd_ops, main, "bwd1", compile_only=compile_only)
-
-    def iteration_lists(self, with_out_conv=False):
+            return self._run_backward_two_streams(ops, main, compile_only, "bwd" + sfx)
+        return self._issue(ops, main, "bwd1" + sfx, compile_only=compile_only)
+
+    def iteration_lists(self, with_out_conv=False, head_fused=False):
         if not self.use_clist:
             raise RuntimeError("dip-amd: the native iteration chains compiled command lists; DIP_NO_CLIST=1 switches them off")
         if self._knockout is not None:
             raise RuntimeError("dip-amd: DIP_KNOCKOUT is a timing experiment of the eager path; the native iteration refuses it")
         if torch.cuda.is_current_stream_capturing():
             raise RuntimeError("dip-amd: the native iteration is an eager form; hipGraph capture goes through GraphedIteration")
-        return self._launch_forward(None, None, with_out_conv, compile_only=True), self._launch_backward(None, compile_only=True)
+        return (self._launch_forward(None, None, with_out_conv, compile_only=True),
+                self._launch_backward(None, compile_only=True, head_fused=head_fused))
 
     def _net_cin(self) -> int:
         return self.sc[0].down_a.Cin
@@ -1088,7 +1130,11 @@
                 self._gloss_keep = gl
                 for fn, args, name in self.last_head.bwd_launches(self, self._head_desc, gl.data_ptr()):
                     N.check(fn(*args, stream), name)
-            self._launch_backward(main)
+            head_fused = self.head_fused(self.last_head)
+            if head_fused:
+                self._pool["head_gs"].copy_(gl)
+                self._head_gs_one = False
+            self._launch_backward(main, head_fused=head_fused)
             gx = None
             if need_input_grad:
                 self._issue(self.bwd_input_ops, main, "bwdin")
diff --git a/deep-image-prior_amd/dip_group.py b/deep-image-prior_amd/dip_group.py
--- a/deep-image-prior_amd/dip_group.py
+++ b/deep-image-prior_amd/dip_group.py
@@ -346,6 +346,8 @@
                         visit(name, f"arg{k}", a)
 
         visit("sr_loss" if self.downsamplers is not None else "loss_head", "desc", self._head)
+        if getattr(self._head, "fuse", None) is not None:
+            visit("loss_head", "fuse", self._head.fuse)
         pointer_args(self._head_fwd + self._head_bwd)
         for _, prefix, desc, ops in self._monitors():
             visit({"mon_": "fit_monitor", "es_": "early_stop"}.get(prefix, prefix[:-1]), "desc", getattr(self, desc))
@@ -426,6 +428,7 @@
                                                      self.nblk, at("loss"))
             fwd, bwd = LH.mse_fwd_launches, LH.mse_bwd_launches
         self._with_out_conv = sr
+        self._head_fused = (not sr) and eng.head_fuse
         self._head_fwd, self._head_bwd = fwd(eng, self._head), bwd(eng, self._head, at("gl"))
         for m, prefix, desc, ops in self._monitors():
             d, launches = self._carve_monitor(slab, m, prefix)
@@ -534,7 +537,7 @@
                 N.check(fn(*args, st), name)
             for fn, args, name in self._head_bwd:
                 N.check(fn(*args, st), name)
-            eng._launch_backward(main)
+            eng._launch_backward(main, head_fused=self._head_fused)
             for _, _, _, ops in self._monitors():
                 for fn, args, name in getattr(self, ops):
                     N.check(fn(*args, st), name)
diff --git a/deep-image-prior_amd/dip_native.py b/deep-image-prior_amd/dip_native.py
--- a/deep-image-prior_amd/dip_native.py
+++ b/deep-image-prior_amd/dip_native.py
@@ -97,6 +97,10 @@
                 ("w", C.c_void_p), ("bias", C.c_void_p), ("Cout", C.c_int32), ("HW", C.c_int32),
                 ("sigmoid", C.c_int32), ("target", C.c_void_p), ("mask", C.c_void_p), ("mask_c", C.c_int32),
                 ("out", C.c_void_p), ("partials", C.c_void_p), ("nblk", C.c_int32), ("loss", C.c_void_p)]
+
+
+class DipLossHeadFuse(C.Structure):
+    _fields_ = [("bn_state", C.c_void_p), ("bn_Cs", C.c_int32), ("bn_rows", C.c_void_p), ("wg_rows", C.c_void_p)]
 
 
 class DipSRLossDesc(C.Structure):
@@ -300,6 +304,13 @@
     "dip_loss_head_nblk": (C.c_int, [C.c_int, C.c_int]),
     "dip_loss_head_fwd": (C.c_int, [C.POINTER(DipLossHeadDesc), C.c_void_p]),
     "dip_loss_head_bwd": (C.c_int, [C.POINTER(DipLossHeadDesc), C.c_void_p, C.c_void_p, C.c_int, C.c_void_p]),
+    "dip_loss_head_fwd_fused": (C.c_int, [C.POINTER(DipLossHeadDesc), C.POINTER(DipLossHeadFuse), C.c_void_p]),
+    "dip_loss_head_fuse_ok": (C.c_int, [C.c_int, C.c_int]),
+    "dip_loss_head_wg_stride": (C.c_int, [C.c_int, C.c_int]),
+    "dip_loss_head_wgrad_reduce": (C.c_int, [C.c_void_p, C.c_int, C.c_int, C.c_int, C.c_void_p, C.c_void_p, C.c_void_p,
+                                             C.c_void_p]),
+    "dip_bn_bwd_finalize_gs": (C.c_int, [C.c_void_p, C.c_int, C.c_int, C.c_int, C.c_int, C.c_void_p, C.c_void_p,
+                                         C.c_void_p, C.c_void_p, C.c_void_p]),
     "dip_sr_loss_nblk": (C.c_int, [C.c_int, C.c_int, C.c_int]),
     "dip_sr_loss_fwd": (C.c_int, [C.POINTER(DipSRLossDesc), C.c_void_p]),
     "dip_sr_loss_bwd": (C.c_int, [C.POINTER(DipSRLossDesc), C.c_void_p, C.c_void_p, C.c_int, C.c_void_p]),
diff --git a/deep-image-prior_amd/dip_optim.py b/deep-image-prior_amd/dip_optim.py
--- a/deep-image-prior_amd/dip_optim.py
+++ b/deep-image-prior_amd/dip_optim.py
@@ -422,7 +422,7 @@
         eng._prepare(dev, H, W, Cimg)
         if opt._sig != opt._signature():
             opt._prepare()
-        fwd, bwd = eng.iteration_lists(with_out_conv=head.with_out_conv)
+        fwd, bwd = eng.iteration_lists(with_out_conv=head.with_out_conv, head_fused=eng.head_fused(head))
         out = self.out
         if out is None or tuple(out.shape) != (1, eng.n_out, eng.Hout, eng.Wout) or out.device != dev:
             out = torch.empty((1, eng.n_out, eng.Hout, eng.Wout), dtype=torch.float32, device=dev)
@@ -459,7 +459,7 @@
         self.out = out
         self._plan = dict(lists=lists, desc=desc, mdesc=mdesc, edesc=descs.get("early_stop"), views=views, x=x, state=st,
                           loss0=loss0,
-                          keep=(head._plan_keep(), eng._clists, eng.fwd_ops, eng.bwd_ops, opt._groups,
+                          keep=(head._plan_keep(), eng._clists, eng.fwd_ops, eng.bwd_ops, eng.bwd_ops_head, eng._head_alloc, opt._groups,
                                 eng.params, eng.grads, eng.nbt, eng.dy_out,
                                 None if reg is None else (reg.saved, reg.out, reg.offset),
                                 [m._plan_keep() for _, m in self._monitors()]))
@@ -470,6 +470,7 @@
         self._check_capture()
         self._check_monitors()
         self.head._check_state()
+        self.engine.head_gs_one()
         for _, m in self._monitors():
             m._check_room(n)
         if self._signature(self.opt._signature()) != self._key:
diff --git a/deep-image-prior_amd/utils/loss_head.py b/deep-image-prior_amd/utils/loss_head.py
--- a/deep-image-prior_amd/utils/loss_head.py
+++ b/deep-image-prior_amd/utils/loss_head.py
@@ -9,12 +9,19 @@
     a, oc = eng.last_act, eng.out_conv
     tr = a.transform()
     p = eng.params.data_ptr()
-    return N.DipLossHeadDesc(a.buf.data_ptr(), a.Cs, oc.Cin, tr, p + 4 * oc.w_off, p + 4 * oc.b_off if oc.b_off >= 0 else None,
+    desc = N.DipLossHeadDesc(a.buf.data_ptr(), a.Cs, oc.Cin, tr, p + 4 * oc.w_off, p + 4 * oc.b_off if oc.b_off >= 0 else None,
                              oc.Cout, eng.Hout * eng.Wout, 1 if eng.need_sigmoid else 0, target_ptr, mask_ptr, mask_c,
-                             out_ptr, partials_ptr, nblk, loss_ptr), tr
+                             out_ptr, partials_ptr, nblk, loss_ptr)
+    desc.fuse = None
+    if eng.head_fuse:
+        desc.fuse = N.DipLossHeadFuse(a.bn.state.data_ptr(), a.bn.Cs, eng._pool["head_bn"].data_ptr(),
+                                      eng._pool["head_wg"].data_ptr())
+    return desc, tr
 
 
 def mse_fwd_launches(eng, desc):
+    if desc.fuse is not None:
+        return [(eng.lib.dip_loss_head_fwd_fused, (C.byref(desc), C.byref(desc.fuse)), "loss_head_fwd")]
     return [(eng.lib.dip_loss_head_fwd, (C.byref(desc),), "loss_head_fwd")]
 
 
diff --git a/include/dip_hip.h b/include/dip_hip.h
--- a/include/dip_hip.h
+++ b/include/dip_hip.h
@@ -201,6 +201,8 @@
                          float* partials , int nblk, const DipBnbFin* fin, void* stream);
 int dip_bn_bwd_finalize(const float* partials, int nblk, int Cs, int C, int npix, float* dgamma,
                         float* dbeta, float* coef, void* stream);
+int dip_bn_bwd_finalize_gs(const float* partials, int nblk, int Cs, int C, int npix, const float* gscale, float* dgamma,
+                           float* dbeta, float* coef, void* stream);
 int dip_bn_bwd_finalize2(const float* partials, int nblk, const float* partials_lo, int nblk_lo, int c_lo, int Cs,
                          int C, int npix, float* dgamma, float* dbeta, float* coef, void* stream);
 int dip_bn_bwd_apply(float* dz, int Cdz, const float* y, int Cy, int npix, int C, const float* state,
@@ -314,6 +316,17 @@
 int dip_loss_head_nblk(int HW, int Cin);
 int dip_loss_head_fwd(const DipLossHeadDesc* d, void* stream);
 int dip_loss_head_bwd(const DipLossHeadDesc* d, const float* gscale, float* dy, int Cy, void* stream);
+typedef struct DipLossHeadFuse {
+    const float* bn_state;
+    int bn_Cs;
+    float* bn_rows;
+    float* wg_rows;
+} DipLossHeadFuse;
+int dip_loss_head_fwd_fused(const DipLossHeadDesc* d, const DipLossHeadFuse* f, void* stream);
+int dip_loss_head_fuse_ok(int Cin, int Cout);
+int dip_loss_head_wg_stride(int Cin, int Cout);
+int dip_loss_head_wgrad_reduce(const float* wg_rows, int nblk, int Cin, int Cout, const float* gscale, float* dw, float* db,
+                               void* stream);
 
 typedef struct DipSRLossDesc {
     const float* out;
```

Result: no change. 189.6 (-0.1%).
